# martinruenz/co-fusion

Measured on AMD Instinct MI355X. Metric: frames/sec at 640x480 (N active models) + ICP-reduce achieved HBM GB/s vs peak, higher is better.
Workload: dtype f32

## Files before the change

co_fusion_amd/csrc/cabi_model.hip:

```cpp
#include <math.h>
#include <string.h>

#include <string>
#include <vector>

#include "cf_host.h"

using namespace cf;

struct cf_model {
    cf_ctx* ctx = nullptr;
    uint32_t max_surfels = 0;
    uint32_t count_host = 0;
    bool count_pending = false;
    hipEvent_t count_event = nullptr;
    hipEvent_t count_wait = nullptr;
    bool ratio_valid = false;
    hipEvent_t ratio_event = nullptr;
    float* buf[2] = {nullptr, nullptr};
    int target = 0;
    float* staged = nullptr;
    unsigned* flags = nullptr;
    unsigned* block_sums = nullptr;
    unsigned* d_count = nullptr;
    unsigned* d_nfresh = nullptr;
    unsigned* d_tmp2 = nullptr;
    int ratio_blocks = 0;
    unsigned* h_counts = nullptr;
    float* records = nullptr;
    float* fresh = nullptr;
    unsigned* new_flags = nullptr;
    bool new_flags_clean = true;
    unsigned* owner = nullptr;
    float* fb_rec = nullptr;
    float* fb_raw = nullptr;
    float* fb_filt = nullptr;
    unsigned long long* keys = nullptr;
    unsigned* index = nullptr;
    float *vertConf = nullptr, *colorTime = nullptr, *normRad = nullptr;
    float* clean_rec = nullptr;
    uint8_t* splat_image = nullptr;
    float *splat_vertex = nullptr, *splat_normal = nullptr;
    uint16_t* splat_time = nullptr;
    float *fill_vertex = nullptr, *fill_normal = nullptr;
    uint8_t* fill_image = nullptr;
    float *tcx = nullptr, *tcy = nullptr;
    float* t_inv_dev = nullptr;
    const cf_odom* preindex_od = nullptr;
    int preindex_time = -1;
    float preindex_cutoff = 0.f; int preindex_delta = 0; uint32_t preindex_nb = 0;
    void drop_preindex() { preindex_od = nullptr; preindex_time = -1; }
    float* rays = nullptr;
    float inv_fx = 0, inv_fy = 0;
};

using cf::inv44f;

extern "C" {

int cf_bilateral(cf_ctx* ctx, const float* depth, int cols, int rows, float maxD, float* out)
{
    if (!ctx || !depth || !out) return CF_EINVAL;
    launch_bilateral(ctx->cur(), depth, cols, rows, maxD, out);
    LAUNCHCHK(ctx);
    return CF_OK;
}

int cf_model_create(cf_ctx* ctx, int max_surfels, cf_model** out)
{
    if (!ctx || !out || max_surfels <= 0) return CF_EINVAL;
    cf_model* m = new cf_model();
    m->ctx = ctx; m->max_surfels = (uint32_t)max_surfels;
    *out = m;
    const int W = ctx->cfg.width, H = ctx->cfg.height;
    const size_t N = (size_t)W * H, M = (size_t)max_surfels, Q = N / 4 + 64;
    if (int r = dmalloc(ctx, &m->buf[0], M * 12)) return r;
    if (int r = dmalloc(ctx, &m->buf[1], M * 12)) return r;
    if (int r = dmalloc(ctx, &m->staged, (M + Q) * 12)) return r;
    if (int r = dmalloc(ctx, &m->flags, M + Q)) return r;
    if (int r = dmalloc(ctx, &m->block_sums, (M + Q) / 2048 + N / 2048 + 16)) return r;
    if (int r = dmalloc(ctx, &m->d_count, 1)) return r;
    if (int r = dmalloc(ctx, &m->d_nfresh, 1)) return r;
    if (int r = dmalloc(ctx, &m->d_tmp2, 8)) return r;
    HIPCHK(ctx, hipMemsetAsync(m->d_tmp2, 0, 8 * sizeof(unsigned), ctx->cur()));
    m->ratio_blocks = fill_ratio_sample_blocks(W, H);
    if (int r = dmalloc(ctx, &m->records, N * 12)) return r;
    if (int r = dmalloc(ctx, &m->fresh, Q * 12)) return r;
    if (int r = dmalloc(ctx, &m->new_flags, N)) return r;
    if (int r = dmalloc(ctx, &m->owner, M)) return r;
    HIPCHK(ctx, hipMemsetAsync(m->owner, 0xFF, M * sizeof(unsigned), ctx->cur()));
    if (int r = dmalloc(ctx, &m->fb_rec, N * 12)) return r;
    if (int r = dmalloc(ctx, &m->fb_raw, N * 12)) return r;
    if (int r = dmalloc(ctx, &m->fb_filt, N * 12)) return r;
    if (int r = dmalloc(ctx, &m->keys, N)) return r;
    HIPCHK(ctx, hipMemsetAsync(m->keys, 0xFF, N * sizeof(unsigned long long), ctx->cur()));
    if (int r = dmalloc(ctx, &m->index, N)) return r;
    if (int r = dmalloc(ctx, &m->vertConf, N * 4)) return r;
    if (int r = dmalloc(ctx, &m->colorTime, N * 4)) return r;
    if (int r = dmalloc(ctx, &m->normRad, N * 4)) return r;
    if (int r = dmalloc(ctx, &m->clean_rec, N * 8)) return r;
    if (int r = dmalloc(ctx, &m->splat_image, N * 4)) return r;
    if (int r = dmalloc(ctx, &m->splat_vertex, N * 4)) return r;
    if (int r = dmalloc(ctx, &m->splat_normal, N * 4)) return r;
    if (int r = dmalloc(ctx, &m->splat_time, N)) return r;
    if (int r = dmalloc(ctx, &m->fill_vertex, N * 4)) return r;
    if (int r = dmalloc(ctx, &m->fill_normal, N * 4)) return r;
    if (int r = dmalloc(ctx, &m->fill_image, N * 4)) return r;
    if (int r = dmalloc(ctx, &m->tcx, (size_t)W)) return r;
    if (int r = dmalloc(ctx, &m->tcy, (size_t)H)) return r;
    if (int r = dmalloc(ctx, &m->rays, N * 4)) return r;
    if (int r = dmalloc(ctx, &m->t_inv_dev, 16)) return r;
    launch_splat_rays(ctx->cur(), ctx_cam(ctx), W, H, m->rays);
    HIPCHK(ctx, hipHostMalloc(reinterpret_cast<void**>(&m->h_counts), sizeof(unsigned) * 4, hipHostMallocCoherent));
    HIPCHK(ctx, hipEventCreateWithFlags(&m->count_event, hipEventDisableTiming));
    HIPCHK(ctx, hipEventCreateWithFlags(&m->ratio_event, hipEventDisableTiming));
    std::vector<float> tx(W), ty(H);
    for (int i = 0; i < W; i++) tx[i] = (float)((double)((float)i / (float)W) + 1.0 / (2.0 * (double)(float)W));
    for (int j = 0; j < H; j++) ty[j] = (float)((double)((float)j / (float)H) + 1.0 / (2.0 * (double)(float)H));
    HIPCHK(ctx, hipMemcpyAsync(m->tcx, tx.data(), sizeof(float) * W, hipMemcpyHostToDevice, ctx->cur()));
    HIPCHK(ctx, hipMemcpyAsync(m->tcy, ty.data(), sizeof(float) * H, hipMemcpyHostToDevice, ctx->cur()));
    m->inv_fx = (float)(1.0 / (double)ctx->cfg.fx); m->inv_fy = (float)(1.0 / (double)ctx->cfg.fy);
    HIPCHK(ctx, hipStreamSynchronize(ctx->cur()));
    return CF_OK;
}

void cf_model_destroy(cf_model* m)
{
    if (!m) return;
    (void)hipStreamSynchronize(m->ctx->cur());
    void* ptrs[] = {m->buf[0], m->buf[1], m->staged, m->flags, m->block_sums, m->d_count, m->d_nfresh, m->d_tmp2, m->records,
                    m->fresh, m->new_flags, m->owner, m->fb_rec, m->fb_raw, m->fb_filt, m->keys, m->index, m->vertConf,
                    m->colorTime, m->normRad, m->splat_image, m->splat_vertex, m->splat_normal, m->splat_time, m->fill_vertex,
                    m->fill_normal, m->fill_image, m->tcx, m->tcy, m->rays, m->t_inv_dev, m->clean_rec};
    for (void* p : ptrs) (void)hipFree(p);
    (void)hipHostFree(m->h_counts);
    if (m->count_event) (void)hipEventDestroy(m->count_event);
    if (m->ratio_event) (void)hipEventDestroy(m->ratio_event);
    delete m;
}

static int adopt_count(cf_model* m)
{
    m->count_host = m->h_counts[0];
    m->count_pending = false;
    if (m->count_host > m->max_surfels) { m->ctx->set_error("surfel buffer overflow"); return CF_ENOMEM; }
    return CF_OK;
}
static int sync_count(cf_model* m)
{
    cf_ctx* ctx = m->ctx;
    HIPCHK(ctx, hipMemcpyAsync(m->h_counts, m->d_count, sizeof(unsigned), hipMemcpyDeviceToHost, ctx->cur()));
    HIPCHK(ctx, hipStreamSynchronize(ctx->cur()));
    return adopt_count(m);
}
static int post_count(cf_model* m, uint32_t upper_bound)
{
    cf_ctx* ctx = m->ctx;
    HIPCHK(ctx, hipEventRecord(m->count_event, ctx->cur()));
    m->count_wait = m->count_event;
    m->count_host = upper_bound;
    m->count_pending = true;
    return CF_OK;
}
static int count_bound(cf_model* m, uint32_t* out)
{
    if (m->count_pending) {
        if (!m->count_wait) { if (int r = sync_count(m)) return r; *out = m->count_host; return CF_OK; }
        if (hipEventQuery(m->count_wait) == hipSuccess) { if (int r = adopt_count(m)) return r; }
        else (void)hipGetLastError();
    }
    *out = m->count_host;
    return CF_OK;
}
static int exact_count(cf_model* m, uint32_t* out)
{
    if (m->count_pending) {
        if (!m->count_wait) { if (int r = sync_count(m)) return r; *out = m->count_host; return CF_OK; }
        HIPCHK(m->ctx, hipEventSynchronize(m->count_wait));
        if (int r = adopt_count(m)) return r;
    }
    *out = m->count_host;
    return CF_OK;
}

int cf_model_initialise(cf_model* m, const uint8_t* rgba, const float* depth_raw, const float* depth_filt, int time, float maxDepth)
{
    if (!m || !rgba || !depth_raw || !depth_filt) return CF_EINVAL;
    m->drop_preindex();
    cf_ctx* ctx = m->ctx; hipStream_t s = ctx->cur();
    const int W = ctx->cfg.width, H = ctx->cfg.height; const long long N = (long long)W * H;
    if ((uint32_t)N > m->max_surfels) return CF_ENOMEM;
    const cf_cam cam = ctx_cam(ctx);
    launch_feedback(s, rgba, depth_raw, W, H, cam, m->inv_fx, m->inv_fy, m->tcx, m->tcy, time, maxDepth, m->fb_rec, m->new_flags);
    HIPCHK(ctx, hipMemsetAsync(m->fb_raw, 0, sizeof(float) * 12 * N, s));
    launch_scan_scatter(s, m->fb_rec, m->new_flags, N, m->block_sums, m->d_count, 0, m->fb_raw);
    launch_feedback(s, rgba, depth_filt, W, H, cam, m->inv_fx, m->inv_fy, m->tcx, m->tcy, time, maxDepth, m->fb_rec, m->new_flags);
    HIPCHK(ctx, hipMemsetAsync(m->fb_filt, 0, sizeof(float) * 12 * N, s));
    launch_scan_scatter(s, m->fb_rec, m->new_flags, N, m->block_sums, m->d_tmp2, 0, m->fb_filt);
    m->new_flags_clean = false;
    launch_init(s, m->fb_raw, m->fb_filt, m->d_count, N, m->buf[m->target]);
    LAUNCHCHK(ctx);
    return sync_count(m);
}

int cf_model_count(cf_model* m, uint32_t* count) { if (!m || !count) return CF_EINVAL; return exact_count(m, count); }

int cf_model_predict_indices(cf_model* m, const float pose[16], int time, float maxDepth, int timeDelta)
{
    if (!m || !pose) return CF_EINVAL;
    m->drop_preindex();
    cf_ctx* ctx = m->ctx;
    float t_inv[16];
    inv44f(pose, t_inv);
    uint32_t nb = 0;
    if (int r = count_bound(m, &nb)) return r;
    launch_predict_indices(ctx->cur(), m->buf[m->target], m->d_count, nb, t_inv, ctx_cam(ctx), ctx->cfg.width, ctx->cfg.height,
                           maxDepth, time, timeDelta, m->keys, m->index, m->vertConf, m->colorTime, m->normRad);
    LAUNCHCHK(ctx);
    return CF_OK;
}

int cf_model_index_keys(cf_model* m, const float pose[16], int time, float maxDepth, int timeDelta, uint32_t surfel_begin, uint32_t surfel_end,
                        uint64_t* keys_dev)
{
    if (!m || !pose || !keys_dev || surfel_begin > surfel_end) return CF_EINVAL;
    m->drop_preindex();
    cf_ctx* ctx = m->ctx;
    const int W = ctx->cfg.width, H = ctx->cfg.height;
    float t_inv[16];
    inv44f(pose, t_inv);
    uint32_t nb = 0;
    if (int r = count_bound(m, &nb)) return r;
    HIPCHK(ctx, hipMemsetAsync(keys_dev, 0xFF, sizeof(uint64_t) * (size_t)W * H, ctx->cur()));
    launch_index_keys(ctx->cur(), m->buf[m->target], m->d_count, surfel_begin, surfel_end < nb ? surfel_end : nb, t_inv, ctx_cam(ctx), W, H, maxDepth,
                      time, timeDelta, reinterpret_cast<unsigned long long*>(keys_dev));
    LAUNCHCHK(ctx);
    return CF_OK;
}
int cf_model_index_resolve(cf_model* m, const float pose[16], uint64_t* keys_dev)
{
    if (!m || !pose || !keys_dev) return CF_EINVAL;
    m->drop_preindex();
    cf_ctx* ctx = m->ctx;
    float t_inv[16];
    inv44f(pose, t_inv);
    launch_index_resolve(ctx->cur(), m->buf[m->target], t_inv, ctx->cfg.width, ctx->cfg.height, reinterpret_cast<unsigned long long*>(keys_dev),
                         m->index, m->vertConf, m->colorTime, m->normRad);
    LAUNCHCHK(ctx);
    return CF_OK;
}

int cf_model_predict_indices_sharded(cf_model* m, const float pose[16], int time, float maxDepth, int timeDelta, int shard, int nshards)
{
    if (!m || !pose || nshards < 1 || shard < 0 || shard >= nshards) return CF_EINVAL;
    m->drop_preindex();
    cf_ctx* ctx = m->ctx;
    if (!ctx->collective) { ctx->set_error("cf_model_predict_indices_sharded: no collective registered (cf_set_collective)"); return CF_ESTATE; }
    uint32_t n = 0;
    if (int r = exact_count(m, &n)) return r;
    const uint32_t b = (uint32_t)(((uint64_t)n * (uint64_t)shard) / (uint64_t)nshards), e = (uint32_t)(((uint64_t)n * (uint64_t)(shard + 1)) / (uint64_t)nshards);
    if (int r = cf_model_index_keys(m, pose, time, maxDepth, timeDelta, b, e, reinterpret_cast<uint64_t*>(m->keys))) return r;
    if (ctx->collective(ctx->collective_user, 1, m->keys, (uint64_t)ctx->cfg.width * ctx->cfg.height, (void*)ctx->cur()) != 0) {
        ctx->set_error("cf_model_predict_indices_sharded: the collective failed");
        return CF_ESTATE;
    }
    return cf_model_index_resolve(m, pose, reinterpret_cast<uint64_t*>(m->keys));
}

int cf_model_combined_predict(cf_model* m, const float pose[16], float maxDepth, float confThreshold, int time, int maxTime, int timeDelta)
{
    if (!m || !pose) return CF_EINVAL;
    cf_ctx* ctx = m->ctx;
    float t_inv[16];
    inv44f(pose, t_inv);
    uint32_t nb = 0;
    if (int r = count_bound(m, &nb)) return r;
    launch_combined_predict(ctx->cur(), m->buf[m->target], m->d_count, nb, t_inv, ctx_cam(ctx), ctx->cfg.width, ctx->cfg.height,
                            maxDepth, confThreshold, time, maxTime, timeDelta, m->rays, m->keys, m->splat_image, m->splat_vertex, m->splat_normal,
                            m->splat_time);
    LAUNCHCHK(ctx);
    m->ratio_valid = false;
    return CF_OK;
}

int cf_model_prefetch_fill_ratio(cf_model* m)
{
    if (!m) return CF_EINVAL;
    cf_ctx* ctx = m->ctx;
    launch_fill_ratio(ctx->cur(), m->splat_image, ctx->cfg.width, ctx->cfg.height, m->d_tmp2 + 2, m->h_counts + 2);
    LAUNCHCHK(ctx);
    HIPCHK(ctx, hipEventRecord(m->ratio_event, ctx->cur()));
    m->ratio_valid = true;
    return CF_OK;
}

int cf_model_perform_fill_in(cf_model* m, const uint8_t* rgba, const float* depth_filt, int passthrough_geom, int passthrough_rgb)
{
    if (!m || !rgba || !depth_filt) return CF_EINVAL;
    cf_ctx* ctx = m->ctx;
    launch_fill_in(ctx->cur(), m->splat_vertex, m->splat_normal, m->splat_image, depth_filt, rgba, ctx->cfg.width, ctx->cfg.height, ctx_cam(ctx),
                   m->inv_fx, m->inv_fy, passthrough_geom, passthrough_rgb, m->fill_vertex, m->fill_normal, m->fill_image);
    LAUNCHCHK(ctx);
    return CF_OK;
}

int cf_model_requires_fill_in(cf_model* m, float ratio, int* out)
{
    if (!m || !out) return CF_EINVAL;
    cf_ctx* ctx = m->ctx;
    if (m->ratio_valid) {
        HIPCHK(ctx, hipEventSynchronize(m->ratio_event));
    } else {
        launch_fill_ratio(ctx->cur(), m->splat_image, ctx->cfg.width, ctx->cfg.height, m->d_tmp2 + 2, m->h_counts + 2);
        LAUNCHCHK(ctx);
        HIPCHK(ctx, hipStreamSynchronize(ctx->cur()));
    }
    *out = ((float)m->h_counts[2] / (float)m->h_counts[3] < ratio) ? 1 : 0;
    return CF_OK;
}

int cf_model_fill_ratio_device(cf_model* m, const uint32_t** counts_dev)
{
    if (!m || !counts_dev) return CF_EINVAL;
    *counts_dev = m->ratio_valid ? m->d_tmp2 + 2 : nullptr;
    return CF_OK;
}

int cf_model_fuse(cf_model* m, const float pose[16], int time, const uint8_t* rgba, const uint8_t* mask, const float* depth_raw,
                  const float* depth_filt, float maxDepth, float weighting, int maskID)
{
    if (!m || !pose || !rgba || !mask || !depth_raw || !depth_filt) return CF_EINVAL;
    m->drop_preindex();
    cf_ctx* ctx = m->ctx; hipStream_t s = ctx->cur();
    const int W = ctx->cfg.width, H = ctx->cfg.height; const long long N = (long long)W * H;
    SurfelFuseArgs a;
    a.index = m->index; a.vertConf = m->vertConf; a.normRad = m->normRad; a.rgba = rgba; a.depth_raw = depth_raw; a.depth_filt = depth_filt;
    a.mask = mask; a.tcx = m->tcx; a.tcy = m->tcy; memcpy(a.pose, pose, sizeof(a.pose)); a.cam = ctx_cam(ctx); a.inv_fx = m->inv_fx;
    a.inv_fy = m->inv_fy; a.cols = W; a.rows = H; a.time = time; a.weighting = weighting; a.maskID = maskID; a.maxDepth = maxDepth;
    a.records = m->records; a.new_flags = m->new_flags; a.owner = m->owner; a.flags_clean = m->new_flags_clean ? 1 : 0;
    launch_associate(s, a);
    {
        ScanPassArgs sp{m->records, m->new_flags, N, m->block_sums, m->d_nfresh, 0, m->fresh, nullptr};
        sp.zero_flags = 1;
        launch_scan_scatter_batch(s, &sp, 1);
        m->new_flags_clean = true;
    }
    uint32_t nb = 0;
    if (int r = count_bound(m, &nb)) return r;
    launch_update(s, m->buf[m->target], m->d_count, nb, m->owner, m->records, time, m->buf[1 - m->target]);
    m->target = 1 - m->target;
    LAUNCHCHK(ctx);
    return CF_OK;
}

int cf_model_clean(cf_model* m, const float pose[16], int time, float confThreshold, float outlierCoeff, int timeDelta, const float* depth_filt,
                   const uint8_t* mask, int maskID, uint32_t* count_out)
{
    if (!m || !pose || !depth_filt || !mask) return CF_EINVAL;
    m->drop_preindex();
    cf_ctx* ctx = m->ctx; hipStream_t s = ctx->cur();
    const int W = ctx->cfg.width, H = ctx->cfg.height;
    uint32_t nb = 0;
    if (int r = count_bound(m, &nb)) return r;
    const unsigned bound = nb + (unsigned)((W / 2) * (H / 2));
    if (bound > m->max_surfels + (unsigned)(W * H / 4 + 64)) return CF_ENOMEM;
    SurfelCleanArgs a;
    a.index = m->index; a.vertConf = m->vertConf; a.colorTime = m->colorTime; a.depth_filt = depth_filt; a.mask = mask; a.rec = nullptr;
    inv44f(pose, a.t_inv); a.cam = ctx_cam(ctx); a.cols = W; a.rows = H; a.time = time; a.confThreshold = confThreshold;
    a.outlierCoeff = outlierCoeff; a.timeDelta = timeDelta; a.maskID = maskID;
    launch_clean(s, m->buf[m->target], m->d_count, m->fresh, m->d_nfresh, bound, a, m->staged, m->flags);
    launch_scan_scatter(s, m->staged, m->flags, bound, m->block_sums, m->d_count, 0, m->buf[1 - m->target], m->h_counts);
    m->target = 1 - m->target;
    LAUNCHCHK(ctx);
    const uint32_t upper = bound < m->max_surfels ? bound : m->max_surfels;
    if (int r = post_count(m, upper)) return r;
    if (count_out) return exact_count(m, count_out);
    return CF_OK;
}

int cf_models_preindex(cf_ctx* ctx, const cf_model_preindex* items, int n, float depth_cutoff, int time_delta)
{
    if (!ctx || !items || n <= 0) return CF_EINVAL;
    hipStream_t s = ctx->cur();
    const int W = ctx->cfg.width, H = ctx->cfg.height;
    std::vector<IndexPassArgs> a((size_t)n);
    for (int k = 0; k < n; k++) {
        cf_model* m = items[k].model; const cf_odom* od = items[k].odom;
        if (!m || !od || m->ctx != ctx || od->ctx != ctx) return CF_EINVAL;
        uint32_t nb = 0;
        if (int r = count_bound(m, &nb)) return r;
        const float* pinv = reinterpret_cast<const float*>(reinterpret_cast<const char*>(od->d_state) + offsetof(cf::OdomDev, pose_inv));
        IndexPassArgs& p = a[k];
        p.surfels = m->buf[m->target]; p.count = m->d_count; p.id_begin = 0; p.id_end = nb; p.maxDepth = depth_cutoff; p.time = items[k].time;
        p.timeDelta = time_delta; p.keys = m->keys; p.index = m->index; p.vertConf = m->vertConf; p.colorTime = m->colorTime; p.normRad = m->normRad;
        p.t_inv_dev = pinv;
    }
    launch_index_keys_batch(s, a.data(), n, ctx_cam(ctx), W, H);
    launch_index_resolve_batch(s, a.data(), n, ctx_cam(ctx), W, H);
    LAUNCHCHK(ctx);
    for (int k = 0; k < n; k++) {
        cf_model* m = items[k].model;
        m->preindex_od = items[k].odom; m->preindex_time = items[k].time; m->preindex_cutoff = depth_cutoff; m->preindex_delta = time_delta; m->preindex_nb = a[k].id_end;
    }
    return CF_OK;
}
static bool preindexed_with(const cf_model* m, const float pose[16], int time, float depth_cutoff, int time_delta, uint32_t nb)
{
    if (!m->preindex_od || m->preindex_time != time) return false;
    if (m->preindex_cutoff != depth_cutoff || m->preindex_delta != time_delta || m->preindex_nb != nb) return false;
    const cf::OdomDev* h = m->preindex_od->h_state;
    for (int r = 0; r < 3; r++) {
        if (memcmp(&pose[r * 4], &h->Rcurr[r * 3], 12) != 0 || memcmp(&pose[r * 4 + 3], &h->tcurr[r], 4) != 0) return false;
    }
    return pose[12] == 0 && pose[13] == 0 && pose[14] == 0 && pose[15] == 1;
}

int cf_models_frame_passes(cf_ctx* ctx, const cf_model_pass* items, int n, float depth_cutoff, float outlier_coeff, int time_delta)
{
    if (!ctx || !items || n <= 0) return CF_EINVAL;
    hipStream_t s = ctx->cur();
    const int W = ctx->cfg.width, H = ctx->cfg.height; const long long N = (long long)W * H;
    const cf_cam cam = ctx_cam(ctx);
    std::vector<int> fusing;
    for (int k = 0; k < n; k++) {
        const cf_model_pass& it = items[k];
        if (!it.model || it.model->ctx != ctx || !it.pose || !it.rgba || !it.depth_filtered) return CF_EINVAL;
        if (it.do_fuse) { if (!it.mask || !it.depth_raw) return CF_EINVAL; fusing.push_back(k); }
    }
    for (int k : fusing) {
        cf_model* m = items[k].model;
        uint32_t nb = 0;
        if (int r = count_bound(m, &nb)) return r;
        if (nb + (unsigned)((W / 2) * (H / 2)) > m->max_surfels + (unsigned)(W * H / 4 + 64)) {
            ctx->set_error("cf_models_frame_passes: a model's surfel buffer cannot hold the clean stage's staging area (max_surfels too small)");
            return CF_ENOMEM;
        }
    }
    for (int k = 0; k < n; k++) { uint32_t nb = 0; if (int r = count_bound(items[k].model, &nb)) return r; }
    int surf_ev = -1;
    if (ctx->prof.enabled > 0 && (ctx->surf_calls_seen++ % (unsigned)ctx->prof.enabled) == 0 && ctx->surf_used + 2 <= cf_ctx::kSurfEvents) {
        for (int e = ctx->surf_used; e < ctx->surf_used + 2; e++)
            if (!ctx->surf_events[e]) HIPCHK(ctx, hipEventCreate(&ctx->surf_events[e]));
        surf_ev = ctx->surf_used; ctx->surf_used += 2;
        HIPCHK(ctx, hipEventRecord(ctx->surf_events[surf_ev], s));
        for (int k = 0; k < n; k++) ctx->surf_bytes += (uint64_t)items[k].model->count_host * 48u * (items[k].do_fuse ? 8u : 2u);
        ctx->surf_calls++;
    }
    static const bool clean_rec_on = getenv("CF_NO_CLEAN_REC") == nullptr;
    auto index_args_of = [&](const std::vector<int>& which, bool feeds_clean, std::vector<IndexPassArgs>& a) -> int {
        a.assign(which.size(), IndexPassArgs{});
        for (size_t q = 0; q < which.size(); q++) {
            const cf_model_pass& it = items[which[q]]; cf_model* m = it.model;
            uint32_t nb = 0;
            if (int r = count_bound(m, &nb)) return r;
            IndexPassArgs& p = a[q];
            p.surfels = m->buf[m->target]; p.count = m->d_count; p.id_begin = 0; p.id_end = nb; inv44f(it.pose, p.t_inv); p.maxDepth = depth_cutoff;
            p.time = it.time; p.timeDelta = time_delta; p.keys = m->keys; p.index = m->index; p.vertConf = m->vertConf; p.colorTime = m->colorTime;
            p.normRad = m->normRad;
            if (feeds_clean && clean_rec_on) { p.clean_rec = m->clean_rec; p.clean_depth = it.depth_filtered; }
        }
        return CF_OK;
    };
    auto index_pass = [&](const std::vector<int>& which) -> int {
        std::vector<IndexPassArgs> a;
        if (int r = index_args_of(which, false, a)) return r;
        launch_index_keys_batch(s, a.data(), (int)a.size(), cam, W, H);
        launch_index_resolve_batch(s, a.data(), (int)a.size(), cam, W, H);
        return CF_OK;
    };
    if (!fusing.empty()) {
        const int nf = (int)fusing.size();
        {
            std::vector<int> todo;
            for (int k : fusing) {
                uint32_t nb = 0;
                if (int r = count_bound(items[k].model, &nb)) return r;
                if (!preindexed_with(items[k].model, items[k].pose, items[k].time, depth_cutoff, time_delta, nb)) todo.push_back(k);
            }
            if (!todo.empty()) { if (int r = index_pass(todo)) return r; }
        }
        std::vector<SurfelFuseArgs> fa(nf);
        std::vector<ScanPassArgs> sa(nf);
        std::vector<UpdatePassArgs> ua(nf);
        for (int q = 0; q < nf; q++) {
            const cf_model_pass& it = items[fusing[q]]; cf_model* m = it.model;
            SurfelFuseArgs& a = fa[q];
            a.index = m->index; a.vertConf = m->vertConf; a.normRad = m->normRad; a.rgba = it.rgba; a.depth_raw = it.depth_raw; a.depth_filt = it.depth_filtered;
            a.mask = it.mask; a.tcx = m->tcx; a.tcy = m->tcy; memcpy(a.pose, it.pose, sizeof(a.pose)); a.cam = cam; a.inv_fx = m->inv_fx;
            a.inv_fy = m->inv_fy; a.cols = W; a.rows = H; a.time = it.time; a.weighting = it.weighting; a.maskID = it.mask_id; a.maxDepth = it.fuse_max_depth;
            a.records = m->records; a.new_flags = m->new_flags; a.owner = m->owner; a.flags_clean = m->new_flags_clean ? 1 : 0;
            sa[q] = ScanPassArgs{m->records, m->new_flags, N, m->block_sums, m->d_nfresh, 0, m->fresh, nullptr};
            sa[q].zero_flags = 1;
            m->new_flags_clean = true;
            uint32_t nb = 0;
            if (int r = count_bound(m, &nb)) return r;
            ua[q] = UpdatePassArgs{m->buf[m->target], m->d_count, nb, m->owner, m->records, it.time, m->buf[1 - m->target]};
        }
        launch_associate_batch(s, fa.data(), nf);
        for (int q = 0; q < nf; q++) items[fusing[q]].model->target = 1 - items[fusing[q]].model->target;
        {
            std::vector<IndexPassArgs> ia;
            if (int r = index_args_of(fusing, true, ia)) return r;
            static const bool side_by_side = getenv("CF_NO_SIDE_BY_SIDE") == nullptr;
            if (!(side_by_side && launch_update_compaction_index_keys(s, ua.data(), sa.data(), ia.data(), nf, cam, W, H))) {
                launch_scan_scatter_batch(s, sa.data(), nf);
                launch_update_batch(s, ua.data(), nf);
                launch_index_keys_batch(s, ia.data(), nf, cam, W, H);
            }
            launch_index_resolve_batch(s, ia.data(), nf, cam, W, H);
        }
        std::vector<CleanPassArgs> ca(nf);
        std::vector<uint32_t> upper(nf);
        for (int q = 0; q < nf; q++) {
            const cf_model_pass& it = items[fusing[q]]; cf_model* m = it.model;
            uint32_t nb = 0;
            if (int r = count_bound(m, &nb)) return r;
            const unsigned bound = nb + (unsigned)((W / 2) * (H / 2));
            if (bound > m->max_surfels + (unsigned)(W * H / 4 + 64)) return CF_ENOMEM;
            CleanPassArgs& c = ca[q];
            c.h.index = m->index; c.h.vertConf = m->vertConf; c.h.colorTime = m->colorTime; c.h.depth_filt = it.depth_filtered; c.h.mask = it.mask;
            c.h.rec = clean_rec_on ? m->clean_rec : nullptr;
            inv44f(it.pose, c.h.t_inv); c.h.cam = cam; c.h.cols = W; c.h.rows = H; c.h.time = it.time; c.h.confThreshold = it.conf_threshold;
            c.h.outlierCoeff = outlier_coeff; c.h.timeDelta = time_delta; c.h.maskID = it.mask_id;
            c.surfels = m->buf[m->target]; c.count = m->d_count; c.fresh = m->fresh; c.n_fresh = m->d_nfresh; c.total_bound = bound; c.staged = m->staged;
            c.flags = m->flags;
            sa[q] = ScanPassArgs{m->staged, m->flags, (long long)bound, m->block_sums, m->d_count, 0, m->buf[1 - m->target], m->h_counts};
            upper[q] = bound < m->max_surfels ? bound : m->max_surfels;
        }
        launch_clean_batch(s, ca.data(), nf);
        launch_scan_scatter_batch(s, sa.data(), nf);
        if (!ctx->batch_event) HIPCHK(ctx, hipEventCreateWithFlags(&ctx->batch_event, hipEventDisableTiming));
        for (int q = 0; q < nf; q++) {
            cf_model* m = items[fusing[q]].model;
            m->target = 1 - m->target;
            m->count_host = upper[q]; m->count_pending = true; m->count_wait = nullptr;
        }
    }
    std::vector<SplatPassArgs> pa(n);
    for (int k = 0; k < n; k++) {
        const cf_model_pass& it = items[k]; cf_model* m = it.model;
        uint32_t nb = m->count_host;
        if (!(m->count_pending && !m->count_wait)) { if (int r = count_bound(m, &nb)) return r; }
        SplatPassArgs& p = pa[k];
        p.surfels = m->buf[m->target]; p.count = m->d_count; p.count_bound = nb; inv44f(it.pose, p.t_inv); p.maxDepth = depth_cutoff;
        p.confThreshold = it.conf_threshold; p.time = it.time; p.maxTime = it.time; p.timeDelta = time_delta; p.rays = m->rays; p.keys = m->keys;
        p.image = m->splat_image; p.vertexConf = m->splat_vertex; p.normalRad = m->splat_normal; p.time16 = m->splat_time;
        m->ratio_valid = false;
        if (it.fill_in)
            p.fill = SplatFillArgs{it.depth_filtered, it.rgba, m->inv_fx, m->inv_fy, it.passthrough_geom ? 1 : 0, it.passthrough_rgb ? 1 : 0,
                                   m->fill_vertex, m->fill_normal, m->fill_image, reinterpret_cast<unsigned long long*>(m->d_tmp2 + 4),
                                   m->d_tmp2 + 2, m->h_counts + 2, m->ratio_blocks};
    }
    launch_combined_predict_batch(s, pa.data(), n, cam, W, H);
    LAUNCHCHK(ctx);
    for (int k = 0; k < n; k++)
        if (items[k].fill_in) {
            HIPCHK(ctx, hipEventRecord(items[k].model->ratio_event, s));
            items[k].model->ratio_valid = true;
        }
    if (surf_ev >= 0) HIPCHK(ctx, hipEventRecord(ctx->surf_events[surf_ev + 1], s));
    if (!fusing.empty()) {
        HIPCHK(ctx, hipEventRecord(ctx->batch_event, s));
        for (int k : fusing) items[k].model->count_wait = ctx->batch_event;
    }
    for (int k = 0; k < n; k++) items[k].model->drop_preindex();
    return CF_OK;
}

int cf_model_download_map(cf_model* m, float* host_surfels, uint32_t capacity, uint32_t* count)
{
    if (!m || !count) return CF_EINVAL;
    cf_ctx* ctx = m->ctx;
    if (int r = exact_count(m, count)) return r;
    if (host_surfels) {
        const uint32_t n = m->count_host < capacity ? m->count_host : capacity;
        HIPCHK(ctx, hipMemcpyAsync(host_surfels, m->buf[m->target], (size_t)n * 48, hipMemcpyDeviceToHost, ctx->cur()));
        HIPCHK(ctx, hipStreamSynchronize(ctx->cur()));
    }
    return CF_OK;
}

int cf_model_upload_map(cf_model* m, const float* host_surfels, uint32_t count)
{
    if (!m || (!host_surfels && count) || count > m->max_surfels) return CF_EINVAL;
    m->drop_preindex();
    cf_ctx* ctx = m->ctx;
    if (count) HIPCHK(ctx, hipMemcpyAsync(m->buf[m->target], host_surfels, (size_t)count * 48, hipMemcpyHostToDevice, ctx->cur()));
    launch_set_count(ctx->cur(), m->d_count, count);
    HIPCHK(ctx, hipStreamSynchronize(ctx->cur()));
    m->count_host = count; m->count_pending = false;
    return CF_OK;
}

int cf_model_buffer(cf_model* m, int which, void** dptr, uint64_t* bytes)
{
    if (!m || !dptr) return CF_EINVAL;
    const size_t N = (size_t)m->ctx->cfg.width * m->ctx->cfg.height;
    void* p = nullptr; size_t b = 0;
    switch (which) {
        case 0: p = m->index; b = N * 4; break;
        case 1: p = m->vertConf; b = N * 16; break;
        case 2: p = m->colorTime; b = N * 16; break;
        case 3: p = m->normRad; b = N * 16; break;
        case 4: p = m->splat_image; b = N * 4; break;
        case 5: p = m->splat_vertex; b = N * 16; break;
        case 6: p = m->splat_normal; b = N * 16; break;
        case 7: p = m->splat_time; b = N * 2; break;
        case 8: p = m->fill_vertex; b = N * 16; break;
        case 9: p = m->fill_normal; b = N * 16; break;
        case 10: p = m->fill_image; b = N * 4; break;
        case 11: { uint32_t c = 0; if (int r = exact_count(m, &c)) return r; p = m->buf[m->target]; b = (size_t)c * 48; break; }
        case 12: {
            unsigned nf = 0;
            HIPCHK(m->ctx, hipMemcpyAsync(&nf, m->d_nfresh, sizeof(unsigned), hipMemcpyDeviceToHost, m->ctx->cur()));
            HIPCHK(m->ctx, hipStreamSynchronize(m->ctx->cur()));
            if (nf > N / 4 + 64) { m->ctx->set_error("cf_model_buffer: the new-surfel count exceeds its buffer"); return CF_ESTATE; }
            p = m->fresh; b = (size_t)nf * 48; break;
        }
        case 13: p = m->clean_rec; b = N * 32; break;
        default: return CF_EINVAL;
    }
    *dptr = p; if (bytes) *bytes = b;
    return CF_OK;
}

int cf_redetect_score(cf_ctx* ctx, const cf_redetect_candidate* cands, int n, const cf_redetect_frame* f, cf_redetect_counts* counts, uint32_t* label_pixels)
{
    if (!ctx || !cands || !f || !counts || n <= 0 || n > kRedetectBatch) return CF_EINVAL;
    if (!f->depth || !f->label || f->cols <= 0 || f->rows <= 0 || (long long)f->cols * f->rows > 0x7fffffffLL) return CF_EINVAL;
    hipStream_t s = ctx->cur();
    const unsigned words = (unsigned)(((long long)f->cols * f->rows + 31) / 32);
    const size_t n_counts = (size_t)kRedetectBatch * kRedetectWords + 1;
    if (!ctx->d_redetect_counts) {
        if (int r = dmalloc(ctx, &ctx->d_redetect_counts, n_counts)) return r;
        HIPCHK(ctx, hipHostMalloc(reinterpret_cast<void**>(&ctx->h_redetect_counts), n_counts * sizeof(unsigned)));
    }
    if (words > ctx->redetect_words) {
        HIPCHK(ctx, hipStreamSynchronize(s));
        if (ctx->d_redetect_bits) (void)hipFree(ctx->d_redetect_bits);
        ctx->d_redetect_bits = nullptr; ctx->redetect_words = 0;
        if (int r = dmalloc(ctx, &ctx->d_redetect_bits, (size_t)kRedetectBatch * words)) return r;
        ctx->redetect_words = words;
    }
    RedetectCand rc[kRedetectBatch];
    for (int k = 0; k < n; k++) {
        cf_model* m = cands[k].model;
        if (!m || m->ctx != ctx) return CF_EINVAL;
        uint32_t nb = 0;
        if (int r = count_bound(m, &nb)) return r;
        rc[k].surfels = m->buf[m->target]; rc[k].count = m->d_count; rc[k].count_bound = nb; rc[k].theta = cands[k].conf_threshold;
        inv44f(cands[k].pose, rc[k].t_inv);
    }
    RedetectFrame rf{f->depth, f->label, f->cols, f->rows, f->cam, f->new_label, f->depth_cutoff, f->depth_tol};
    if (ctx->redetect_timing) HIPCHK(ctx, hipEventRecord(ctx->redetect_ev[0], s));
    HIPCHK(ctx, hipMemsetAsync(ctx->d_redetect_counts, 0, n_counts * sizeof(unsigned), s));
    launch_redetect_score(s, rc, n, rf, ctx->d_redetect_bits, words, ctx->d_redetect_counts);
    LAUNCHCHK(ctx);
    if (ctx->redetect_timing) HIPCHK(ctx, hipEventRecord(ctx->redetect_ev[1], s));
    HIPCHK(ctx, hipMemcpyAsync(ctx->h_redetect_counts, ctx->d_redetect_counts, n_counts * sizeof(unsigned), hipMemcpyDeviceToHost, s));
    HIPCHK(ctx, hipStreamSynchronize(s));
    if (ctx->redetect_timing) HIPCHK(ctx, hipEventElapsedTime(&ctx->redetect_last_ms, ctx->redetect_ev[0], ctx->redetect_ev[1]));
    for (int k = 0; k < n; k++) {
        const unsigned* w = ctx->h_redetect_counts + (size_t)k * kRedetectWords;
        counts[k] = cf_redetect_counts{w[0], w[1], w[2], w[3], w[4], w[5]};
    }
    if (label_pixels) *label_pixels = ctx->h_redetect_counts[(size_t)kRedetectBatch * kRedetectWords];
    return CF_OK;
}

int cf_redetect_timing(cf_ctx* ctx, int on, float* last_ms)
{
    if (!ctx) return CF_EINVAL;
    if (on) for (hipEvent_t& e : ctx->redetect_ev) if (!e) HIPCHK(ctx, hipEventCreate(&e));
    ctx->redetect_timing = on != 0;
    if (last_ms) *last_ms = ctx->redetect_last_ms;
    return CF_OK;
}

int cf_relabel(cf_ctx* ctx, uint8_t* label_dev, uint64_t n, int from, int to)
{
    if (!ctx || !label_dev || from < 0 || from > 255 || to < 0 || to > 255 || (reinterpret_cast<uintptr_t>(label_dev) & 15u)) return CF_EINVAL;
    if (from == to || n == 0) return CF_OK;
    launch_relabel(ctx->cur(), label_dev, n, (unsigned)from, (unsigned)to);
    LAUNCHCHK(ctx);
    return CF_OK;
}

float cf_fusion_weight(const float pose[16], const float lastPose[16], float weightMultiplier)
{
    float pinv[16], diff[16];
    inv44f(pose, pinv);
    for (int i = 0; i < 4; i++)
        for (int j = 0; j < 4; j++) {
            float s = 0;
            for (int k = 0; k < 4; k++) s += pinv[i * 4 + k] * lastPose[k * 4 + j];
            diff[i * 4 + j] = s;
        }
    const float tn = sqrtf(diff[3] * diff[3] + diff[7] * diff[7] + diff[11] * diff[11]);
    const float* R = diff;
    double rx = R[2 * 4 + 1] - R[1 * 4 + 2], ry = R[0 * 4 + 2] - R[2 * 4 + 0], rz = R[1 * 4 + 0] - R[0 * 4 + 1];
    const double s = sqrt((rx * rx + ry * ry + rz * rz) * 0.25);
    double c = (double)((R[0] + R[5] + R[10]) - 1.0f) * 0.5;
    c = c > 1. ? 1. : c < -1. ? -1. : c;
    double theta = acos(c);
    if (s < 1e-5) {
        double t;
        if (c > 0) rx = ry = rz = 0;
        else {
            t = (R[0] + 1) * 0.5; rx = sqrt(t > 0.0 ? t : 0.0);
            t = (R[5] + 1) * 0.5; ry = sqrt(t > 0.0 ? t : 0.0) * (R[0 * 4 + 1] < 0 ? -1.0 : 1.0);
            t = (R[10] + 1) * 0.5; rz = sqrt(t > 0.0 ? t : 0.0) * (R[0 * 4 + 2] < 0 ? -1.0 : 1.0);
            if (fabs(rx) < fabs(ry) && fabs(rx) < fabs(rz) && (R[1 * 4 + 2] > 0) != (ry * rz > 0)) rz = -rz;
            theta /= sqrt(rx * rx + ry * ry + rz * rz);
            rx *= theta; ry *= theta; rz *= theta;
        }
    } else {
        double vth = 1 / (2 * s);
        vth *= theta;
        rx *= vth; ry *= vth; rz *= vth;
    }
    const float rv[3] = {(float)rx, (float)ry, (float)rz};
    const float rn = sqrtf(rv[0] * rv[0] + rv[1] * rv[1] + rv[2] * rv[2]);
    float weighting = tn > rn ? tn : rn;
    const float largest = 0.01f, minWeight = 0.5f;
    if (weighting > largest) weighting = largest;
    const float w = 1.0f - (weighting / largest);
    weighting = (w > minWeight ? w : minWeight) * weightMultiplier;
    return weighting;
}

}
```

co_fusion_amd/csrc/cf_host.h:

```cpp
#pragma once

#include <string.h>

#include <mutex>
#include <string>

#include "cf_kernels.h"

struct cf_ctx;
struct cf_thread_binding { const cf_ctx* ctx = nullptr; hipStream_t stream = nullptr; };
extern thread_local cf_thread_binding cf_tls_binding;

struct cf_ctx {
    cf_config cfg{};
    hipStream_t stream = nullptr;
    hipStream_t cur() const { return cf_tls_binding.ctx == this ? cf_tls_binding.stream : stream; }
    hipStream_t own_stream = nullptr;
    std::string last_error;
    std::mutex error_mutex;
    cf::IcpLaunch icp_launch{256, 0};
    int icp_arith = 0;
    float* d_ref = nullptr;
    float* h_ref = nullptr;
    unsigned long long* d_acc_a = nullptr;
    unsigned long long* d_acc_b = nullptr;
    unsigned long long* d_out = nullptr;
    unsigned long long* h_out = nullptr;
    cf::OdomDev* d_scratch_state = nullptr;
    cf::OdomDev* h_scratch_state = nullptr;
    uint8_t* d_cand_scratch = nullptr;
    cf::So3Sync* d_so3_sync = nullptr;
    unsigned gn_mode_epoch = 0;
    int xcd_round_robin = -1;
    int gn_mode = 1;
    static constexpr int kStateSlots = 256;
    cf::OdomDev* d_state_pool = nullptr;
    cf::OdomDev* h_state_pool = nullptr;
    bool slot_used[kStateSlots]{};
    hipEvent_t batch_event = nullptr;
    static constexpr int kLanes = 8;
    hipStream_t lanes[kLanes]{};
    hipEvent_t lane_done[kLanes]{};
    hipEvent_t fork_point = nullptr;
    static constexpr int kMarks = 64;
    hipEvent_t marks[kMarks]{};
    bool mark_set[kMarks]{};
    hipStream_t forked_from = nullptr;
    bool forked = false;
    unsigned lanes_used = 0;
    int (*collective)(void* user, int op, void* dev_buf, uint64_t words, void* stream) = nullptr;
    void* collective_user = nullptr;
    void* rccl = nullptr;
    unsigned prof_calls = 0;
    cf::ProfSink prof{};
    double prof_ms_accum = 0;
    static constexpr int kSurfEvents = 64;
    hipEvent_t surf_events[kSurfEvents]{};
    int surf_used = 0; unsigned surf_calls_seen = 0;
    double surf_ms_accum = 0; uint64_t surf_calls = 0, surf_bytes = 0;
    unsigned* d_redetect_bits = nullptr; unsigned redetect_words = 0;
    unsigned* d_redetect_counts = nullptr; unsigned* h_redetect_counts = nullptr;
    bool redetect_timing = false; hipEvent_t redetect_ev[2]{}; float redetect_last_ms = 0.f;
    void set_error(const std::string& m);
};
inline cf_cam ctx_cam(const cf_ctx* ctx) { return cf_cam{ctx->cfg.fx, ctx->cfg.fy, ctx->cfg.cx, ctx->cfg.cy}; }
extern "C" int cf_wait_stream(cf_ctx* ctx);
#define HIPCHK(ctx, call)                                                                      \
    do {                                                                                       \
        hipError_t e_ = (call);                                                                \
        if (e_ != hipSuccess) {                                                                \
            (ctx)->set_error(std::string(#call) + ": " + hipGetErrorString(e_));               \
            return CF_EHIP;                                                                    \
        }                                                                                      \
    } while (0)
#define LAUNCHCHK(ctx) HIPCHK(ctx, hipGetLastError())
template <typename T>
inline int dmalloc(cf_ctx* ctx, T** p, size_t count)
{
    HIPCHK(ctx, hipMalloc(reinterpret_cast<void**>(p), count * sizeof(T)));
    HIPCHK(ctx, hipMemsetAsync(*p, 0, count * sizeof(T), ctx->cur()));
    return CF_OK;
}
inline int clear_acc(cf_ctx* ctx, unsigned long long* acc)
{
    HIPCHK(ctx, hipMemsetAsync(acc, 0, sizeof(unsigned long long) * cf::kGroups * 32, ctx->stream));
    return CF_OK;
}
struct cf_odom;
namespace cf {
int ref_track(cf_ctx* ctx, cf_odom* od, const float pose[16], const cf_track_opts* opts, float* err_surface);
int ref_icp_step(cf_ctx* ctx, const float Rcurr[9], const float tcurr[3], const float* vc, const float* nc, const float Rprev_inv[9], const float tprev[3],
                 cf_cam intr, const float* vp, const float* np, float dist_thres, float angle_thres, int cols, int rows, float* err, float out29[29]);
int ref_rgb_step(cf_ctx* ctx, const cf_dataterm* corres, float sigma, const float* cloud3, float fx, float fy, const int16_t* dIdx, const int16_t* dIdy,
                 float sobel_scale, int cols, int rows, float out29[29]);
int ref_so3_step(cf_ctx* ctx, const uint8_t* last_image, const uint8_t* next_image, const float basis[9], const float kinv[9], const float krlr[9],
                 int cols, int rows, float out11[11]);
inline void pose_split(const float pose[16], float R[9], float t[3])
{
    for (int i = 0; i < 3; i++) { R[3 * i] = pose[4 * i]; R[3 * i + 1] = pose[4 * i + 1]; R[3 * i + 2] = pose[4 * i + 2]; t[i] = pose[4 * i + 3]; }
}
struct TrackTerms { bool icp, rgb; };
inline TrackTerms track_terms(const cf_track_opts* o) { return TrackTerms{!o->rgb_only && o->icp_weight > 0, o->rgb_only || o->icp_weight < 100}; }
}

struct cf_odom {
    cf_ctx* ctx = nullptr;
    float* vmaps_tmp = nullptr;
    float* nmaps_tmp = nullptr;
    float* vmap_g_prev[3]{};
    float* nmap_g_prev[3]{};
    float* vmap_curr[3]{};
    float* nmap_curr[3]{};
    const float* ext_vmap_curr[3]{};
    const float* ext_nmap_curr[3]{};
    float2* zrange[3]{};
    bool zrange_valid = false;
    const float2* ext_zrange[3]{};
    const float* cur_vmap(int l) const { return ext_vmap_curr[l] ? ext_vmap_curr[l] : vmap_curr[l]; }
    const float* cur_nmap(int l) const { return ext_nmap_curr[l] ? ext_nmap_curr[l] : nmap_curr[l]; }
    const float2* cur_zrange(int l) const { return ext_vmap_curr[l] ? ext_zrange[l] : (zrange_valid ? zrange[l] : nullptr); }
    float* lastDepth[3]{};
    float* nextDepth[3]{};
    bool next_depth_is_last = false;
    float* next_depth(int i) const { return next_depth_is_last ? lastDepth[i] : nextDepth[i]; }
    uint8_t* lastImage[3]{};
    uint8_t* nextImage[3]{};
    uint8_t* lastNextImage[3]{};
    int16_t* dIdx[3]{};
    int16_t* dIdy[3]{};
    float* cloud[3]{};
    cf_dataterm* corres[3]{};
    uint8_t* cand[3]{};
    unsigned char* occ = nullptr;
    bool occ_valid = false;
    bool use_occ = false;
    unsigned* aabb = nullptr;
    float map_pose[12]{};
    int box_hint[4] = {0x7fffffff, 0, 0, 0};
    unsigned* res_range = nullptr;
    int res_hint[3] = {-1, -1, -1};
    bool box_valid = false;
    int band_begin = 0, band_end = 0;
    bool band_counts = true;
    unsigned long long* icp_acc = nullptr;
    unsigned long long* rgb_acc = nullptr;
    cf::OdomDev* d_state = nullptr;
    cf::OdomDev* h_state = nullptr;
    int slot = -1;
    float distThres = 0, angleThres = 0, sobelScale = 0, maxDepthDeltaRGB = 0, maxDepthRGB = 0;
    float angleSqLt = 0, distSqLe = 0;
    float minGrad[3]{};
    bool pending_so3_swap = false;
    size_t rgb_acc_words = 0;
    unsigned gn_epoch_seen = 0;
    bool result_pending = false;
    int expected_solves = -1;
    cf::LaunchShape launch_shape{};
};
```

co_fusion_amd/csrc/cf_kernels.h:

```cpp
#pragma once

#include <hip/hip_runtime.h>
#include <hip/hip_ext.h>
#include <stdint.h>

#include "../../include/cofusion_hip.h"

namespace cf {

__host__ __device__ __forceinline__ cf_cam cam_level(cf_cam c, int level)
{
    const int div = 1 << level;
    return cf_cam{c.fx / div, c.fy / div, c.cx / div, c.cy / div};
}

constexpr int kGroups = 64;

struct alignas(64) GnHot {
    int icp, level_done; float cull_z[2];
    float Rcurr[9], tcurr[3];
    float Rprev_inv[9], tprev[3];
    int cull_box[4];
    int rgb, rgbOnly, level_done2, pad;
    float krkInv[9], kt[3];
// ... 109 lines not shown
void launch_frame_maps(hipStream_t s, FrameMapsArgs a, int W, int H);
void launch_rgbd_pyramids(hipStream_t s, const RgbdBatch& b, int n_chains, int W, int H, float cutoff);
void launch_model_maps_and_pyramids(hipStream_t s, const ModelMapsBatch& mb, int n, const RgbdBatch& rb, int n_chains, int W, int H, float cutoff);
void launch_rgb_prep(hipStream_t s, RgbPrepBatch b, int n, int W, int H);

struct IDiv { unsigned M, s; };
inline IDiv make_idiv(int d)
{
    if (d < 2) return IDiv{0x80000000u, 0u};
    unsigned l = 0;
    while ((1u << l) < (unsigned)d) l++;
    return IDiv{(unsigned)((((unsigned long long)1 << (31 + l)) + (unsigned)d - 1) / (unsigned)d), l - 1};
}
constexpr int kGramBits[8] = {20, 20, 20, 17, 17, 17, 22, 0};
struct LaunchShape { int icp[3]; int res[3]; int icp_err; };
struct IcpLaunch { int threads; int ppt; int gram;
                   LaunchShape* const* shape = nullptr; };

constexpr int kMaxBatch = 16;
struct IcpModelArgs {
    const float* vc; const float* nc;
    const float* vp; const float* np;
    const OdomDev* st;
    unsigned long long* acc;
    float* err;
    const unsigned char* occ;
    int row_begin, row_end;
    int cull;
    const float2* zr;
    int box_blocks;
};
constexpr int kNoBoxHint = 0x7fffffff;
struct CullRuns { int x0, y0, nrx, total; };
__host__ __device__ inline CullRuns cull_runs(const int box[4], int L, int cols, int rows)
{
    int bx0 = (box[0] >> L) - 1, by0 = (box[1] >> L) - 1, bx1 = (box[2] >> L) + 1, by1 = (box[3] >> L) + 1;
    bx0 = bx0 < 0 ? 0 : bx0; by0 = by0 < 0 ? 0 : by0; bx1 = bx1 > cols - 1 ? cols - 1 : bx1; by1 = by1 > rows - 1 ? rows - 1 : by1;
    if (bx0 > bx1 || by0 > by1) return CullRuns{0, 0, 0, 0};
    if ((cols & 63) == 0) { const int nrx = (bx1 >> 6) - (bx0 >> 6) + 1; return CullRuns{bx0 >> 6, by0, nrx, nrx * (by1 - by0 + 1)}; }
    const int q0 = (by0 * cols) >> 6, q1 = ((by1 + 1) * cols - 1) >> 6;
    return CullRuns{0, q0, 0, q1 - q0 + 1};
}
inline int box_blocks_for(const int box_hint[4], int L, int cols, int rows, int threads)
{
    if (box_hint[0] == kNoBoxHint) return 0;
    const CullRuns cr = cull_runs(box_hint, L, cols, rows);
    const int wpb = threads / 64;
    const int runs = cr.total + cr.total / 4 + 2 * (cr.nrx > 0 ? cr.nrx : (cols + 63) / 64);
    int want = (((runs + 2 * wpb - 1) / (2 * wpb) + 7) / 8) * 8;
    return want < 8 ? 8 : want;
}
inline int residual_blocks_for(int seen) { return seen < 0 ? 0 : seen + seen / 4 + 2; }
struct GnArgs {
    OdomDev* od[kMaxBatch];
    unsigned long long* icp_acc[kMaxBatch];
    unsigned long long* rgb_acc[kMaxBatch];
    OdomDev* od_host[kMaxBatch];
    int slot_px;
    int icp_gram;
};
struct RgbModelArgs {
    OdomDev* st;
    const uint8_t* cand; const float* nextDepth; const float* lastDepth;
    const uint8_t* lastImage; const uint8_t* nextImage;
    cf_dataterm* corres; const float* cloud; const int16_t* dIdx; const int16_t* dIdy;
    unsigned long long* icp_acc; unsigned long long* rgb_acc;
    int no_counts;
    uint2* recs;
    unsigned* slot_counts;
    const unsigned* res_range;
    int res_blocks;
};
struct RgbArgs {
    RgbModelArgs m[kMaxBatch];
    int cols, rows;
    cf_cam il;
    float sobelScale, maxDepthDelta;
    int compact;
    int slot_px;
    IDiv cdiv;
};
inline RgbModelArgs rgb_model_args(const OdomDev* h , OdomDev* d_state, int level)
{
    return RgbModelArgs{d_state, h->cand[level], h->nextDepth[level], h->lastDepth[level], h->lastImage[level], h->nextImage[level],
                        h->corres[level], h->cloud[level], h->dIdx[level], h->dIdy[level], h->icp_acc, h->rgb_acc, 0,
                        reinterpret_cast<uint2*>(h->corres[level]),
                        reinterpret_cast<unsigned*>(reinterpret_cast<uint2*>(h->corres[level]) + (size_t)(h->width >> level) * (h->height >> level)),
                        h->res_range ? h->res_range + 2 * level : nullptr, 0};
}
constexpr int kMaxSlots = 2 * kMaxBatch;
struct IcpArgs {
    IcpModelArgs m[kMaxBatch];
    int cols, rows;
    cf_cam intr;
    float distThres, angleThres;
    float angleSqLt, distSqLe;
    int occ_w, occ_shift;
    int flags;
    int row_begin, row_end;
    IDiv cdiv;
    int slot_end[kMaxSlots];
    unsigned char slot_desc[kMaxSlots];
    int slots_used;
};
constexpr unsigned char kResidualSlot = 0x80;
void launch_icp_level(hipStream_t s, IcpLaunch cfg, const IcpArgs& args, int n, int level, hipEvent_t ev0 = nullptr, hipEvent_t ev1 = nullptr);
void launch_rgb_residual(hipStream_t s, const RgbArgs& ra, int n);
void launch_rgb_step(hipStream_t s, const RgbArgs& ra, int n);
constexpr uint64_t kRgbResidualBytes = 27;
constexpr uint64_t kRgbResidualBytesCompact = 11;
void launch_acc_total(hipStream_t s, const unsigned long long* acc, unsigned long long* out);
void launch_rgb_cand(hipStream_t s, const int16_t* dIdx, const int16_t* dIdy, const float* next_depth,
                     const uint8_t* next_image, float min_scale, int cols, int rows, uint8_t* cand);
void launch_so3_step(hipStream_t s, const uint8_t* last_image, const uint8_t* next_image, const float basis[9],
                     const float kinv[9], const float krlr[9], int cols, int rows, unsigned long long* out16);
void launch_gn_solve(hipStream_t s, const GnArgs& gn, int n, int next_level, int last_of_level);

struct ProfSink {
    hipEvent_t* events; int capacity; int used; uint64_t bytes; uint64_t launches; int enabled;
};

constexpr int kSo3Blocks = 16;
constexpr int kStepSubs = 16;
struct So3Sync { unsigned long long acc[10][16]; unsigned arrive, depart;
                 unsigned step_top, pad;
                 unsigned step_sub[kStepSubs][32]; };
struct GnHook { int (*fn)(void* user, int op, void* dev_buf, uint64_t words, void* stream); void* user; int split[kMaxBatch]; };
struct TrackerStates { OdomDev* dev[kMaxBatch]; const OdomDev* host[kMaxBatch]; };
bool launch_gn_track(hipStream_t s, IcpLaunch cfg, const TrackerStates& states, So3Sync* so3_syncs ,
                     const GnHook* hook, const IcpArgs icp_args[3], const RgbArgs rgb_args[3], int n, int width, int height, bool so3,
                     bool pyramid, bool fast_odom, bool rgb, bool icp, int mode, ProfSink* prof,
                     OdomDev* const* h_states = nullptr ,
                     const RgbPrepBatch* prep = nullptr );
void rgb_prep_levels(RgbPrepBatch& b, int n, int W, int H);
float replay_icp_level0(hipStream_t s, IcpLaunch cfg, const IcpArgs& a0, const RgbArgs& r0, int n, int slots, int ablate, int reps, hipEvent_t e0, hipEvent_t e1);
#ifdef CF_ABLATE
void trace_so3_dump(hipStream_t s);
void trace_solve_begin();
void trace_solve_end(hipStream_t s, const char* path);
void trace_step_solve(hipStream_t s, IcpLaunch cfg, const IcpArgs& a0, const RgbArgs& r0, So3Sync* syncs, int n, const char* path);
void trace_icp_level0(hipStream_t s, IcpLaunch cfg, const IcpArgs& a0, const RgbArgs& r0, int n, int slots, const char* path);
#endif
bool probe_xcd_round_robin(hipStream_t s);
float sqrt_gate_lt(float T);
float sqrt_gate_le(float T);

constexpr int kSurfBatch = 16;
struct IndexPassArgs {
    const float* surfels; const unsigned* count; unsigned id_begin, id_end; float t_inv[16]; float maxDepth; int time, timeDelta;
    unsigned long long* keys; unsigned* index; float* vertConf; float* colorTime; float* normRad;
    const float* t_inv_dev;
    float* clean_rec;
    const float* clean_depth;
};
__host__ __device__ inline void inv44f(const float a[16], float o[16])
{
    const float c00 = a[5] * a[10] - a[6] * a[9];
    const float c01 = a[6] * a[8] - a[4] * a[10];
    const float c02 = a[4] * a[9] - a[5] * a[8];
    const float det = a[0] * c00 + a[1] * c01 + a[2] * c02;
    const float id = 1.0f / det;
    float Li[9];
    Li[0] = c00 * id; Li[1] = (a[2] * a[9] - a[1] * a[10]) * id; Li[2] = (a[1] * a[6] - a[2] * a[5]) * id;
    Li[3] = c01 * id; Li[4] = (a[0] * a[10] - a[2] * a[8]) * id; Li[5] = (a[2] * a[4] - a[0] * a[6]) * id;
    Li[6] = c02 * id; Li[7] = (a[1] * a[8] - a[0] * a[9]) * id; Li[8] = (a[0] * a[5] - a[1] * a[4]) * id;
    for (int i = 0; i < 3; i++) {
        o[i * 4 + 0] = Li[i * 3 + 0]; o[i * 4 + 1] = Li[i * 3 + 1]; o[i * 4 + 2] = Li[i * 3 + 2];
        o[i * 4 + 3] = -(Li[i * 3 + 0] * a[3] + Li[i * 3 + 1] * a[7] + Li[i * 3 + 2] * a[11]);
    }
    o[12] = 0; o[13] = 0; o[14] = 0; o[15] = 1;
}
struct SplatFillArgs {
    const float* depth_filt; const uint8_t* rgba;
    float inv_fx, inv_fy; int pass_geom, pass_rgb;
    float* fill_vertex; float* fill_normal; uint8_t* fill_image;
    unsigned long long* acc;
    unsigned* out2; unsigned* out2_host;
    int sample_blocks;
};
int fill_ratio_sample_blocks(int cols, int rows);
struct SplatPassArgs {
    const float* surfels; const unsigned* count; unsigned count_bound; float t_inv[16]; float maxDepth, confThreshold; int time, maxTime, timeDelta;
    const float* rays; unsigned long long* keys; uint8_t* image; float* vertexConf; float* normalRad; uint16_t* time16;
    SplatFillArgs fill;
};
struct UpdatePassArgs { const float* in; const unsigned* count; unsigned count_bound; unsigned* owner; const float* records; int time; float* out; };
struct SurfelFuseArgs {
    const unsigned* index; const float* vertConf; const float* normRad;
    const uint8_t* rgba; const float* depth_raw; const float* depth_filt; const uint8_t* mask;
    const float* tcx; const float* tcy;
    float pose[16]; cf_cam cam; float inv_fx, inv_fy;
    int cols, rows, time; float weighting; int maskID; float maxDepth;
    float* records; unsigned* new_flags; unsigned* owner;
    int flags_clean = 0;
};
struct SurfelCleanArgs {
    const unsigned* index; const float* vertConf; const float* colorTime;
    const float* depth_filt; const uint8_t* mask;
    const float* rec;
    float t_inv[16]; cf_cam cam; int cols, rows, time; float confThreshold, outlierCoeff; int timeDelta, maskID;
};
struct CleanPassArgs {
    SurfelCleanArgs h; const float* surfels; const unsigned* count; const float* fresh; const unsigned* n_fresh; unsigned total_bound;
    float* staged; unsigned* flags;
};
struct ScanPassArgs {
    const float* rec; const unsigned* flags; long long n; unsigned* block_sums; unsigned* total; unsigned add_to_total; float* out; unsigned* total_host;
    int zero_flags = 0;
};
void launch_index_keys_batch(hipStream_t s, const IndexPassArgs* items, int n, cf_cam cam, int cols, int rows);
bool launch_update_compaction_index_keys(hipStream_t s, const UpdatePassArgs* up, const ScanPassArgs* sc, const IndexPassArgs* ix, int n, cf_cam cam, int cols,
                                         int rows);
void launch_index_resolve_batch(hipStream_t s, const IndexPassArgs* items, int n, cf_cam cam, int cols, int rows);
void launch_combined_predict_batch(hipStream_t s, const SplatPassArgs* items, int n, cf_cam cam, int cols, int rows);
void launch_associate_batch(hipStream_t s, const SurfelFuseArgs* items, int n);
void launch_update_batch(hipStream_t s, const UpdatePassArgs* items, int n);
void launch_clean_batch(hipStream_t s, const CleanPassArgs* items, int n);
void launch_scan_scatter_batch(hipStream_t s, const ScanPassArgs* items, int n);
void launch_bilateral(hipStream_t s, const float* depth, int cols, int rows, float maxD, float* out);
void launch_scan_scatter(hipStream_t s, const float* rec, const unsigned* flags, long long n, unsigned* block_sums, unsigned* total,
                         unsigned add_to_total, float* out, unsigned* total_host = nullptr );
void launch_feedback(hipStream_t s, const uint8_t* rgba, const float* depth, int cols, int rows, cf_cam cam, float inv_fx, float inv_fy,
                     const float* tcx, const float* tcy, int time, float maxDepth, float* rec, unsigned* flags);
void launch_init(hipStream_t s, const float* raw, const float* filt, const unsigned* raw_count, long long max_n, float* out);
void launch_index_keys(hipStream_t s, const float* surfels, const unsigned* count, unsigned id_begin, unsigned id_end, const float t_inv[16],
                       cf_cam cam, int cols, int rows, float maxDepth, int time, int timeDelta, unsigned long long* keys);
void launch_index_resolve(hipStream_t s, const float* surfels, const float t_inv[16], int cols, int rows, unsigned long long* keys,
                          unsigned* index, float* vertConf, float* colorTime, float* normRad);
void launch_predict_indices(hipStream_t s, const float* surfels, const unsigned* count, unsigned count_bound, const float t_inv[16], cf_cam cam,
                            int cols, int rows, float maxDepth, int time, int timeDelta, unsigned long long* keys, unsigned* index,
                            float* vertConf, float* colorTime, float* normRad);
void launch_splat_rays(hipStream_t s, cf_cam cam, int cols, int rows, float* rays );
void launch_combined_predict(hipStream_t s, const float* surfels, const unsigned* count, unsigned count_bound, const float t_inv[16], cf_cam cam,
                             int cols, int rows, float maxDepth, float confThreshold, int time, int maxTime, int timeDelta,
                             const float* rays, unsigned long long* keys, uint8_t* image, float* vertexConf, float* normalRad, uint16_t* time16);
void launch_fill_in(hipStream_t s, const float* pv, const float* pn, const uint8_t* pimg, const float* depth, const uint8_t* rgba, int cols,
                    int rows, cf_cam cam, float inv_fx, float inv_fy, int pass_geom, int pass_rgb, float* ov, float* on, uint8_t* oi);
void launch_fill_ratio(hipStream_t s, const uint8_t* pimg, int cols, int rows, unsigned* out2, unsigned* out2_host = nullptr );
void launch_associate(hipStream_t s, const SurfelFuseArgs& h);
void launch_update(hipStream_t s, const float* in, const unsigned* count, unsigned count_bound, unsigned* owner, const float* records, int time,
                   float* out);
void launch_clean(hipStream_t s, const float* surfels, const unsigned* count, const float* fresh, const unsigned* n_fresh, unsigned total_bound,
                  const SurfelCleanArgs& h, float* staged, unsigned* flags);
void launch_set_count(hipStream_t s, unsigned* out, unsigned v);

constexpr int kRedetectBatch = 16;
constexpr int kRedetectWords = 8;
struct RedetectCand {
    const float* surfels; const unsigned* count; unsigned count_bound;
    float theta;
    float t_inv[16];
};
struct RedetectFrame {
    const float* depth; const uint8_t* label; int cols, rows; cf_cam cam; int new_label; float cutoff, tol;
};
void launch_redetect_score(hipStream_t s, const RedetectCand* cands, int n, const RedetectFrame& f, unsigned* bits, unsigned words, unsigned* counts);
void launch_relabel(hipStream_t s, uint8_t* label , unsigned long long n, unsigned from, unsigned to);

}
```

co_fusion_amd/csrc/surfel.hip:

```cpp
#include "cf_surfel_device.h"
#include "cf_kernels.h"

namespace cf {

static constexpr int kB = 256;
static inline int gridFor(long long n) { return (int)((n + kB - 1) / kB); }
static inline int gridXcd(long long n, int chunk = 1) { const int q = 8 * (chunk > 1 ? chunk : 1); return (gridFor(n) + q - 1) / q * q; }
#ifdef CF_ABLATE
static int xcd_env(const char* name, int dflt) { const char* e = getenv(name); return e ? atoi(e) : dflt; }
#else
static constexpr int xcd_env(const char*, int dflt) { return dflt; }
#endif
struct BatchHdr { int n; int blk_end[kSurfBatch]; };
template <class A> struct Batch { BatchHdr h; A m[kSurfBatch]; };
struct VBlock { int model, bid, nblk; };
__device__ __forceinline__ VBlock batch_decode_at(const BatchHdr& h, int b)
{
    int slot = 0;
#pragma unroll
    for (int k = 0; k < kSurfBatch - 1; k++) slot += (b >= h.blk_end[k]) ? 1 : 0;
    const int start = slot ? h.blk_end[slot - 1] : 0;
    return VBlock{slot, b - start, h.blk_end[slot] - start};
}
__device__ __forceinline__ VBlock batch_decode(const BatchHdr& h) { return batch_decode_at(h, (int)blockIdx.x); }
template <class A>
static int batch_layout(Batch<A>& B, const int* blocks, int n)
{
    int total = 0;
    B.h.n = n;
    for (int k = 0; k < kSurfBatch; k++) {
        if (k < n) total += (blocks[k] + 7) / 8 * 8;
        B.h.blk_end[k] = k < n ? total : 0x7fffffff;
    }
    return total;
}

__device__ __forceinline__ int xcd_block(int chunk, int b, int nblk)
{
    if (chunk == 0) return b;
    const int per = nblk >> 3, x = b & 7, r = b >> 3;
    if (chunk < 0) return x * per + r;
    const int lb = ((r / chunk) * 8 + x) * chunk + (r % chunk);
    return lb;
}

__device__ __forceinline__ unsigned sortable_bits(float z)
{
    const unsigned b = __float_as_uint(z);
    return (b & 0x80000000u) ? ~b : (b | 0x80000000u);
}
__device__ __forceinline__ unsigned long long zkey(float z, unsigned id) { return ((unsigned long long)sortable_bits(z) << 32) | id; }
constexpr unsigned long long kEmptyKey = ~0ull;

__global__ void __launch_bounds__(kB) bilateral_kernel(const float* __restrict__ depth, int cols, int rows, float maxD,
                                                       float* __restrict__ out)
{
    const int i = blockIdx.x * kB + threadIdx.x;
    if (i >= cols * rows) return;
    const int y = i / cols, x = i - y * cols;
    const float value = depth[i];
    if (value > maxD || value < 0.3f) { out[i] = 0; return; }
    float sum1 = 0, sum2 = 0;
#pragma unroll
    for (int dy = -6; dy <= 6; ++dy) {
        const int cy = y + dy;
        if (cy < 0 || cy >= rows) continue;
        const float* __restrict__ rowp = depth + cy * cols + x;
#pragma unroll
        for (int dx = -6; dx <= 6; ++dx) {
            const int cx = x + dx;
            if (cx < 0 || cx >= cols) continue;
            const float tmp = rowp[dx];
            const float space2 = (float)(dx * dx + dy * dy);
            const float color2 = (value - tmp) * (value - tmp);
            const float weight = det_expf(-(space2 * 0.024691358f + color2 * 555.556f));
            sum1 += tmp * weight;
            sum2 += weight;
        }
    }
    out[i] = sum1 / sum2;
}

static constexpr int kScanItems = 2048;
struct ScanArgs {
    const float4* rec; const unsigned* flags; long long n; unsigned* block_sums; unsigned* total; unsigned add_to_total; float4* out;
    unsigned* total_host; int zero_flags;
};
__device__ __forceinline__ void scan_load_flags(const unsigned* __restrict__ flags, long long i0, long long n, unsigned (&f)[8])
{
    if (i0 + 8 <= n) {
        const uint4 a = *reinterpret_cast<const uint4*>(flags + i0), c = *reinterpret_cast<const uint4*>(flags + i0 + 4);
        f[0] = a.x; f[1] = a.y; f[2] = a.z; f[3] = a.w; f[4] = c.x; f[5] = c.y; f[6] = c.z; f[7] = c.w;
    } else {
        unsigned t[8];
#pragma unroll
        for (int e = 0; e < 8; e++) t[e] = flags[i0 + e < n ? i0 + e : n - 1];
#pragma unroll
        for (int e = 0; e < 8; e++) f[e] = (i0 + e < n) ? t[e] : 0u;
    }
}
__device__ __forceinline__ void scan_block_sums_body(const Batch<ScanArgs>& B, int blk)
{
    const VBlock vb = batch_decode_at(B.h, blk);
    const ScanArgs& a = B.m[vb.model];
    const unsigned* __restrict__ flags = a.flags; const long long n = a.n; unsigned* __restrict__ block_sums = a.block_sums;
    if ((long long)vb.bid * kScanItems >= n) return;
    unsigned f[8];
    scan_load_flags(flags, (long long)vb.bid * kScanItems + (long long)threadIdx.x * 8, n, f);
    unsigned s = 0;
#pragma unroll
    for (int e = 0; e < 8; e++) s += f[e];
    for (int o = 32; o > 0; o >>= 1) s += __shfl_xor((int)s, o, 64);
    __shared__ unsigned w[4];
    if ((threadIdx.x & 63) == 0) w[threadIdx.x >> 6] = s;
    __syncthreads();
    if (threadIdx.x == 0) block_sums[vb.bid] = w[0] + w[1] + w[2] + w[3];
}
__global__ void __launch_bounds__(256) scan_block_sums_kernel(const Batch<ScanArgs> B) { scan_block_sums_body(B, (int)blockIdx.x); }
__global__ void set_count_kernel(unsigned* out, unsigned v);
__global__ void set_count2_kernel(unsigned* out, unsigned* out_host, unsigned v);
__device__ __forceinline__ void scan_scatter_body(const Batch<ScanArgs>& B, int blk)
{
    const VBlock vb = batch_decode_at(B.h, blk);
    const ScanArgs& a = B.m[vb.model];
    const float4* __restrict__ rec = a.rec; const unsigned* __restrict__ flags = a.flags; const long long n = a.n;
    const unsigned* __restrict__ block_sums = a.block_sums; unsigned* __restrict__ total = a.total; const unsigned add_to_total = a.add_to_total;
    float4* __restrict__ out = a.out; unsigned* __restrict__ total_host = a.total_host;
    const int nb = (int)((n + kScanItems - 1) / kScanItems);
    if (vb.bid >= nb) return;
    __shared__ unsigned wsum[4], s_base;
    __shared__ unsigned short s_src[kScanItems];
    const int tid = threadIdx.x, lane = tid & 63, wave = tid >> 6;
    const long long i0 = (long long)vb.bid * kScanItems + (long long)tid * 8;
    unsigned f[8];
    scan_load_flags(flags, i0, n, f);
    if (a.zero_flags) {
        unsigned* fz = const_cast<unsigned*>(flags);
        if (i0 + 8 <= n) { *reinterpret_cast<uint4*>(fz + i0) = make_uint4(0, 0, 0, 0); *reinterpret_cast<uint4*>(fz + i0 + 4) = make_uint4(0, 0, 0, 0); }
        else
            for (int e = 0; e < 8; e++) if (i0 + e < n) fz[i0 + e] = 0;
    }
    unsigned b = 0;
    for (int k = tid; k < vb.bid; k += 256) b += block_sums[k];
    for (int o = 32; o > 0; o >>= 1) b += __shfl_xor((int)b, o, 64);
    if (lane == 0) wsum[wave] = b;
    __syncthreads();
    if (tid == 0) s_base = wsum[0] + wsum[1] + wsum[2] + wsum[3];
    unsigned mine = 0;
#pragma unroll
    for (int e = 0; e < 8; e++) mine += f[e];
    unsigned incl = mine;
    for (int o = 1; o < 64; o <<= 1) { const unsigned t = __shfl_up((int)incl, o, 64); if (lane >= o) incl += t; }
    __syncthreads();
    if (lane == 63) wsum[wave] = incl;
    __syncthreads();
    unsigned rel = incl - mine;
    for (int w = 0; w < wave; w++) rel += wsum[w];
#pragma unroll
    for (int e = 0; e < 8; e++)
        if (f[e]) s_src[rel++] = (unsigned short)(tid * 8 + e);
    const unsigned count = wsum[0] + wsum[1] + wsum[2] + wsum[3];
    const unsigned base = s_base;
    __syncthreads();
    const float4* __restrict__ in0 = rec + (size_t)vb.bid * kScanItems * 3;
    float4* __restrict__ out0 = out + (size_t)base * 3;
    const unsigned words = count * 3;
#ifndef CF_SCAN_FLY
#define CF_SCAN_FLY 4
#endif
    constexpr int kFly = CF_SCAN_FLY;
    for (unsigned m0 = tid; m0 < words; m0 += kFly * 256) {
        float4 v[kFly];
#pragma unroll
        for (int u = 0; u < kFly; u++) {
            const unsigned m = m0 + u * 256;
            const unsigned mc = m < words ? m : words - 1;
            const unsigned j = mc / 3u;
            v[u] = in0[(size_t)s_src[j] * 3 + (mc - 3u * j)];
        }
#pragma unroll
        for (int u = 0; u < kFly; u++) { const unsigned m = m0 + u * 256; if (m < words) out0[m] = v[u]; }
    }
    if (vb.bid == nb - 1 && tid == 255) {
        *total = base + count + add_to_total;
        if (total_host) *total_host = base + count + add_to_total;
    }
}
__global__ void __launch_bounds__(256) scan_scatter_kernel(const Batch<ScanArgs> B) { scan_scatter_body(B, (int)blockIdx.x); }

void launch_scan_scatter_batch(hipStream_t s, const ScanPassArgs* items, int n_items)
{
    for (int base = 0; base < n_items; base += kSurfBatch) {
        const int nb = n_items - base < kSurfBatch ? n_items - base : kSurfBatch;
        Batch<ScanArgs> B;
        int blocks[kSurfBatch], any = 0;
        for (int k = 0; k < nb; k++) {
            const ScanPassArgs& h = items[base + k];
            B.m[k] = ScanArgs{reinterpret_cast<const float4*>(h.rec), h.flags, h.n, h.block_sums, h.total, h.add_to_total, reinterpret_cast<float4*>(h.out), h.total_host, h.zero_flags};
            blocks[k] = (int)((B.m[k].n + kScanItems - 1) / kScanItems);
            any += blocks[k];
            if (blocks[k] == 0) set_count2_kernel<<<1, 1, 0, s>>>(B.m[k].total, B.m[k].total_host, B.m[k].add_to_total);
        }
        if (!any) continue;
        const int grid = batch_layout(B, blocks, nb);
        scan_block_sums_kernel<<<grid, 256, 0, s>>>(B);
        scan_scatter_kernel<<<grid, 256, 0, s>>>(B);
    }
}
void launch_scan_scatter(hipStream_t s, const float* rec, const unsigned* flags, long long n, unsigned* block_sums, unsigned* total,
                         unsigned add_to_total, float* out, unsigned* total_host)
{
    const ScanPassArgs a{rec, flags, n, block_sums, total, add_to_total, out, total_host};
    launch_scan_scatter_batch(s, &a, 1);
}

__global__ void __launch_bounds__(kB) feedback_kernel(const uchar4* __restrict__ rgba, const float* __restrict__ depth, int cols, int rows,
                                                      float cx, float cy, float inv_fx, float inv_fy, const float* __restrict__ tcx,
                                                      const float* __restrict__ tcy, int time, float maxDepth,
                                                      float4* __restrict__ rec , unsigned* __restrict__ flags)
{
    const int q = blockIdx.x * kB + threadIdx.x;
    if (q >= cols * rows) return;
    const int j = q / cols, i = q - j * cols;
    const int rank = i * rows + j;
    const float x = tcx[i] * (float)cols, y = tcy[j] * (float)rows;
    const f3 p = get_vertex(depth, cols, rows, i, j, x, y, cx, cy, inv_fx, inv_fy);
    if (p.z <= 0 || p.z > maxDepth) { flags[rank] = 0; return; }
    const f3 n = get_normal_central(p, depth, cols, rows, i, j, x, y, cx, cy, inv_fx, inv_fy);
    const uchar4 c = rgba[q];
    flags[rank] = 1;
    rec[rank * 3 + 0] = make_float4(p.x, p.y, p.z, confidence(x, y, cx, cy, 1.0f));
    rec[rank * 3 + 1] = make_float4(encode_color((float)c.x / 255.0f, (float)c.y / 255.0f, (float)c.z / 255.0f), 0.f, (float)c.z / 255.0f, (float)time);
    rec[rank * 3 + 2] = make_float4(n.x, n.y, n.z, get_radius(p.z, n.z, inv_fx, inv_fy));
}


__global__ void __launch_bounds__(kB) init_kernel(const float4* __restrict__ raw, const float4* __restrict__ filt,
                                                  const unsigned* __restrict__ raw_count, float4* __restrict__ out)
{
    const unsigned k = blockIdx.x * kB + threadIdx.x;
    if (k >= *raw_count) return;
    const float4 c = raw[k * 3 + 1];
    out[k * 3] = raw[k * 3];
    out[k * 3 + 1] = make_float4(c.x, 0.f, 1.f, c.w);
    out[k * 3 + 2] = filt[k * 3 + 2];
}

__device__ __forceinline__ bool index_project(const float4 pc, const float4 ct, const Mat4& t_inv, cf_cam cam, int cols, int rows,
                                              float maxDepth, int time, int timeDelta, f3& ph, int& q)
{
    if ((float)time - ct.w > (float)timeDelta) return false;
    return surfel_project(pc, t_inv, cam, cols, rows, maxDepth, ph, q);
}

struct IndexArgs {
    const float4* surfels; const unsigned* count; Mat4 t_inv; float maxDepth; int time, timeDelta; unsigned id_begin, id_end;
    unsigned long long* keys; unsigned* index; float4* vertConf; float4* colorTime; float4* normRad;
    const float* t_inv_dev;
    float4* clean_rec; const float* clean_depth;
};
__device__ __forceinline__ Mat4 index_matrix(const IndexArgs& a)
{
    if (!a.t_inv_dev) return a.t_inv;
    Mat4 m;
#pragma unroll
    for (int k = 0; k < 16; k++) m.m[k] = a.t_inv_dev[k];
    return m;
}
struct FrameGeom { cf_cam cam; int cols, rows; };

__device__ __forceinline__ void index_splat_body(const Batch<IndexArgs>& B, const FrameGeom& g, int blk)
{
    const VBlock vb = batch_decode_at(B.h, blk);
    const IndexArgs& a = B.m[vb.model];
    const float4* __restrict__ surfels = a.surfels;
    const unsigned id = a.id_begin + vb.bid * kB + threadIdx.x;
    if (id >= *a.count || id >= a.id_end) return;
    f3 ph; int q;
    const Mat4 T = index_matrix(a);
    if (!index_project(surfels[id * 3], surfels[id * 3 + 1], T, g.cam, g.cols, g.rows, a.maxDepth, a.time, a.timeDelta, ph, q)) return;
    atomicMin(&a.keys[q], zkey(ph.z, id));
}
__global__ void __launch_bounds__(kB) index_splat_kernel(const Batch<IndexArgs> B, const FrameGeom g) { index_splat_body(B, g, (int)blockIdx.x); }

__global__ void __launch_bounds__(kB) index_resolve_kernel(const Batch<IndexArgs> B, const FrameGeom g)
{
    const VBlock vb = batch_decode(B.h);
    const IndexArgs& a = B.m[vb.model];
    const float4* __restrict__ surfels = a.surfels; unsigned long long* __restrict__ keys = a.keys; unsigned* __restrict__ index = a.index;
    float4* __restrict__ vertConf = a.vertConf; float4* __restrict__ colorTime = a.colorTime; float4* __restrict__ normRad = a.normRad;
    const int q = vb.bid * kB + threadIdx.x;
    if (q >= g.cols * g.rows) return;
    const unsigned long long k = keys[q];
    keys[q] = kEmptyKey;
    float4* __restrict__ const rec = a.clean_rec;
    const float dflt = rec ? a.clean_depth[q] : 0.f;
    if (k == kEmptyKey) {
        index[q] = 0;
        vertConf[q] = colorTime[q] = normRad[q] = make_float4(0, 0, 0, 0);
        if (rec) { rec[2 * q] = make_float4(0, 0, 0, 0); rec[2 * q + 1] = make_float4(0, 0, __uint_as_float(0u), dflt); }
        return;
    }
    const unsigned id = (unsigned)k;
    const float4 pc = surfels[id * 3], ct = surfels[id * 3 + 1], nr = surfels[id * 3 + 2];
    const Mat4 T = index_matrix(a);
    const f3 ph = xform_point(T, f3{pc.x, pc.y, pc.z});
    const f3 n = normalized(xform_dir(T, f3{nr.x, nr.y, nr.z}));
    index[q] = id;
    vertConf[q] = make_float4(ph.x, ph.y, ph.z, pc.w);
    colorTime[q] = ct;
    normRad[q] = make_float4(n.x, n.y, n.z, nr.w);
    if (rec) { rec[2 * q] = make_float4(ph.x, ph.y, ph.z, pc.w); rec[2 * q + 1] = make_float4(ct.z, ct.w, __uint_as_float(id), dflt); }
}

struct SplatSetup { f3 ph, n; float rad, pn; int x_lo, x_hi, y_lo, y_hi; };

__device__ __forceinline__ bool splat_setup(const float4 pc, const float4 ct, const float4 nr, const Mat4& t_inv, cf_cam cam, int cols,
                                            int rows, float maxDepth, float confThreshold, int time, int maxTime, int timeDelta,
                                            SplatSetup& s)
{
    s.ph = xform_point(t_inv, f3{pc.x, pc.y, pc.z});
    if (s.ph.z > maxDepth || s.ph.z < 0 || pc.w < confThreshold || (float)time - ct.w > (float)timeDelta || ct.w > (float)maxTime) return false;
    s.n = normalized(xform_dir(t_inv, f3{nr.x, nr.y, nr.z}));
    s.rad = nr.w;
    const f3 x1n = normalized(f3{s.n.y - s.n.z, -s.n.x, s.n.x});
    const f3 x1 = {x1n.x * s.rad * 1.41421356f, x1n.y * s.rad * 1.41421356f, x1n.z * s.rad * 1.41421356f};
    const f3 y1 = cross(s.n, x1);
    const f3 c[4] = {s.ph + x1, s.ph + y1, s.ph - y1, s.ph - x1};
    float px_[4], py_[4];
#pragma unroll
    for (int k = 0; k < 4; k++) { px_[k] = ((cam.fx * c[k].x) / c[k].z) + cam.cx; py_[k] = ((cam.fy * c[k].y) / c[k].z) + cam.cy; }
    const float xmin = fminf(px_[0], fminf(px_[1], fminf(px_[2], px_[3]))), xmax = fmaxf(px_[0], fmaxf(px_[1], fmaxf(px_[2], px_[3])));
    const float ymin = fminf(py_[0], fminf(py_[1], fminf(py_[2], py_[3]))), ymax = fmaxf(py_[0], fmaxf(py_[1], fmaxf(py_[2], py_[3])));
    const float size = fmaxf(0.0f, fmaxf(fabsf(xmax - xmin), fabsf(ymax - ymin)));
    if (!(size > 0.0f) || !(size <= 4096.0f)) return false;
    const float u = ((cam.fx * s.ph.x) / s.ph.z) + cam.cx, v = ((cam.fy * s.ph.y) / s.ph.z) + cam.cy;
    if (!(u >= 0.0f && v >= 0.0f && u <= (float)cols && v <= (float)rows)) return false;
    const float half = size * 0.5f;
    s.x_lo = max((int)ceilf(u - half - 0.5f), 0); s.x_hi = min((int)ceilf(u + half - 0.5f) - 1, cols - 1);
    s.y_lo = max((int)ceilf(v - half - 0.5f), 0); s.y_hi = min((int)ceilf(v + half - 0.5f) - 1, rows - 1);
    s.pn = dot(s.ph, s.n);
    return true;
}

__device__ __forceinline__ bool splat_fragment(const SplatSetup& s, const float4* __restrict__ rays, int cols, int px, int py, float maxDepth,
                                               float& z)
{
    const float4 lr = rays[py * cols + px];
    const f3 l = {lr.x, lr.y, lr.z};
    const float k = s.pn / dot(l, s.n);
    const f3 cp = {k * l.x, k * l.y, k * l.z};
    const f3 diff = cp - s.ph;
    if (!(dot(diff, diff) <= s.rad * s.rad)) return false;
    if (!(cp.z < maxDepth)) return false;
    z = cp.z;
    return true;
}

__global__ void __launch_bounds__(kB) splat_rays_kernel(cf_cam cam, int cols, int rows, float4* __restrict__ rays)
{
    const int q = blockIdx.x * kB + threadIdx.x;
    if (q >= cols * rows) return;
    const int py = q / cols, px = q - py * cols;
    const float fx_ = (float)px + 0.5f, fy_ = (float)py + 0.5f;
    const f3 l = normalized(f3{(fx_ - cam.cx) / cam.fx, (fy_ - cam.cy) / cam.fy, 1.0f});
    rays[q] = make_float4(l.x, l.y, l.z, 0.f);
}

struct SplatArgs {
    const float4* surfels; const unsigned* count; Mat4 t_inv; float maxDepth, confThreshold; int time, maxTime, timeDelta;
    const float4* rays; unsigned long long* keys; uchar4* image; float4* vertexConf; float4* normalRad; unsigned short* time16;
    SplatFillArgs fill;
};

__global__ void __launch_bounds__(kB) splat_raster_kernel(const Batch<SplatArgs> B, const FrameGeom g)
{
    const VBlock vb = batch_decode(B.h);
    const SplatArgs& a = B.m[vb.model];
    const float4* __restrict__ surfels = a.surfels; const float4* __restrict__ rays = a.rays; unsigned long long* __restrict__ keys = a.keys;
    const int cols = g.cols, rows = g.rows;
    const unsigned gt = vb.bid * kB + threadIdx.x;
    const unsigned id = gt >> 2;
    const int sub = (int)(gt & 3u);
    if (id >= *a.count) return;
    SplatSetup s;
    if (!splat_setup(surfels[id * 3], surfels[id * 3 + 1], surfels[id * 3 + 2], a.t_inv, g.cam, cols, rows, a.maxDepth, a.confThreshold, a.time,
                     a.maxTime, a.timeDelta, s))
        return;
    const int w = s.x_hi - s.x_lo + 1, h = s.y_hi - s.y_lo + 1;
    if (w <= 0 || h <= 0) return;
    int fx = sub, fy = 0;
    while (fx >= w) { fx -= w; fy++; }
    while (fy < h) {
        const int px = s.x_lo + fx, py = s.y_lo + fy;
        float z;
        if (splat_fragment(s, rays, cols, px, py, a.maxDepth, z)) {
            atomicMin(&keys[py * cols + px], zkey(z, id));
        }
        fx += 4;
        while (fx >= w) { fx -= w; fy++; }
    }
}

__device__ __forceinline__ void fill_in_px(float4 v, float4 n, uchar4 e, const float* __restrict__ depth, const uchar4* __restrict__ rgba, int cols,
                                           int rows, int x, int y, int q, float cx, float cy, float inv_fx, float inv_fy, int pass_geom, int pass_rgb,
                                           float4* __restrict__ ov, float4* __restrict__ on, uchar4* __restrict__ oi)
{
    const float z = depth[q];
    const f3 p = {((float)x - cx) * z * inv_fx, ((float)y - cy) * z * inv_fy, z};
    ov[q] = (v.z == 0 || pass_geom) ? make_float4(p.x, p.y, p.z, 1.f) : v;
    if (n.z == 0 || pass_geom) {
        const float zx = depth[y * cols + min(x + 1, cols - 1)], zy = depth[min(y + 1, rows - 1) * cols + x];
        const f3 vx = {((float)(x + 1) - cx) * zx * inv_fx, ((float)y - cy) * zx * inv_fy, zx};
        const f3 vy = {((float)x - cx) * zy * inv_fx, ((float)(y + 1) - cy) * zy * inv_fy, zy};
        const f3 nn = normalized(cross(vx - p, vy - p));
        on[q] = make_float4(nn.x, nn.y, nn.z, 1.f);
    } else
        on[q] = n;
    oi[q] = (((int)e.x + (int)e.y + (int)e.z) == 0 || pass_rgb) ? rgba[q] : e;
}
__global__ void __launch_bounds__(kB) fill_in_kernel(const float4* __restrict__ pv, const float4* __restrict__ pn, const uchar4* __restrict__ pimg,
                                                     const float* __restrict__ depth, const uchar4* __restrict__ rgba, int cols, int rows,
                                                     float cx, float cy, float inv_fx, float inv_fy, int pass_geom, int pass_rgb,
                                                     float4* __restrict__ ov, float4* __restrict__ on, uchar4* __restrict__ oi)
{
    const int q = blockIdx.x * kB + threadIdx.x;
    if (q >= cols * rows) return;
    const int y = q / cols, x = q - y * cols;
    fill_in_px(pv[q], pn[q], pimg[q], depth, rgba, cols, rows, x, y, q, cx, cy, inv_fx, inv_fy, pass_geom, pass_rgb, ov, on, oi);
}
__device__ __forceinline__ bool fill_ratio_sample(int p, int dn, int size)
{
    const int i0 = p * dn / size;
    bool hit = false;
    for (int i = max(i0 - 1, 0); i <= min(i0 + 1, dn - 1); i++) hit = hit || nearest_texel(((float)i + 0.5f) / (float)dn, size) == p;
    return hit;
}

int fill_ratio_sample_blocks(int cols, int rows)
{
    const int dw = cols / 20, dh = rows / 20;
    int blocks = 0, last = -1;
    for (int j = 0; j < dh; j++)
        for (int i = 0; i < dw; i++) {
// ... 325 lines not shown
    f3 localPos{0, 0, 0}, localNorm{0, 0, 0};
    float x = 0, y = 0, x_n = 0, y_n = 0;
    const float stepX = 1.0f / (float)cols, stepY = 1.0f / (float)rows;
    const float indexXStep = stepX * 0.5f / scale, indexYStep = stepY * 0.5f / scale;
    const float windowMultiplier = 2;
    bool window = false;
    if (exists) {
        const float4* src = (k < n_old) ? surfels + (size_t)k * 3 : fresh + (size_t)(k - n_old) * 3;
        pc = src[0]; ct = src[1]; nr = src[2];
        localPos = xform_point(a.t_inv, f3{pc.x, pc.y, pc.z});
        x = ((a.cam.fx * localPos.x) / localPos.z) + a.cam.cx; y = ((a.cam.fy * localPos.y) / localPos.z) + a.cam.cy;
        localNorm = normalized(xform_dir(a.t_inv, f3{nr.x, nr.y, nr.z}));
        x_n = x / (float)cols; y_n = y / (float)rows;
        window = (float)a.time - ct.w < (float)a.timeDelta && localPos.z > 0 && x > 0 && y > 0 && x < (float)cols && y < (float)rows;
    }
    const float iBeg = x_n - (scale * indexXStep * windowMultiplier), jBeg = y_n - (scale * indexYStep * windowMultiplier);
    const int X0 = (int)floorf(iBeg * (float)cols - 0.5f), Y0 = (int)floorf(jBeg * (float)rows - 0.5f);
#ifdef CF_ABLATE
    const int abl = a.abl;
#else
    constexpr int abl = 0;
#endif
    if (window && rec && !(abl & 1)) {
        const int half = sub & 1;
#pragma unroll
        for (int q = 0; q < 8; q++) {
            const int row = q >> 1, tex = (sub >> 1) + 2 * (q & 1), t = row * 4 + tex;
            const int g = iclamp(Y0 + row, 0, rows - 1) * cols + iclamp(X0 + tex, 0, cols - 1);
            const float4 v = rec[2 * g + half];
            float* const o = P + half * 64 + t;
            o[0] = v.x; o[16] = v.y; o[32] = v.z; o[48] = v.w;
        }
    } else
    if (window && !(abl & 1)) {
#pragma unroll
        for (int c = 0; c < 4; c++) {
            const int t = sub * 4 + c;
            const int g = iclamp(Y0 + sub, 0, rows - 1) * cols + iclamp(X0 + c, 0, cols - 1);
            const float4 vcf = a.vertConf[g];
            const float4 ctm = a.colorTime[g];
            const unsigned idx = a.index[g];
            P[0 * 16 + t] = vcf.x; P[1 * 16 + t] = vcf.y; P[2 * 16 + t] = vcf.z; P[3 * 16 + t] = vcf.w;
            P[4 * 16 + t] = ctm.z; P[5 * 16 + t] = ctm.w;
            P[6 * 16 + t] = __uint_as_float(idx);
        }
    }
    __syncthreads();
    if (!exists) return;
    int test = 1;
    int cnt = 0, zCount = 0, violationCount = 0;
    float avgViolation = 0;
    if (window && !(abl & 2)) {
        float i = iBeg;
        for (int s4 = 0; s4 < sub; s4++) i += indexXStep;
        for (; i < x_n + (scale * indexXStep * windowMultiplier); i += indexXStep, i += indexXStep, i += indexXStep, i += indexXStep) {
            for (float j = jBeg; j < y_n + (scale * indexYStep * windowMultiplier); j += indexYStep) {
                const int nlx = (int)floorf(i * (float)cols) - X0, nly = (int)floorf(j * (float)rows) - Y0;
                const unsigned current = ((unsigned)nlx < 4u && (unsigned)nly < 4u)
                                             ? __float_as_uint(P[6 * 16 + nly * 4 + nlx])
                                             : a.index[nearest_texel(j, rows) * cols + nearest_texel(i, cols)];
                if (current > 0U) {
                    float4 vertConf, colorTime;
                    const float fu = i * (float)cols - 0.5f, fv = j * (float)rows - 0.5f;
                    const float x0f = floorf(fu), y0f = floorf(fv);
                    const int lx = (int)x0f - X0, ly = (int)y0f - Y0;
                    if ((unsigned)lx < 3u && (unsigned)ly < 3u) {
                        const float wx = fu - x0f, wy = fv - y0f;
                        const float* q = P + (ly * 4 + lx);
                        vertConf.x = bilerp(q[0 * 16], q[0 * 16 + 1], q[0 * 16 + 4], q[0 * 16 + 5], wx, wy);
                        vertConf.y = bilerp(q[1 * 16], q[1 * 16 + 1], q[1 * 16 + 4], q[1 * 16 + 5], wx, wy);
                        vertConf.z = bilerp(q[2 * 16], q[2 * 16 + 1], q[2 * 16 + 4], q[2 * 16 + 5], wx, wy);
                        vertConf.w = bilerp(q[3 * 16], q[3 * 16 + 1], q[3 * 16 + 4], q[3 * 16 + 5], wx, wy);
                        colorTime.z = bilerp(q[4 * 16], q[4 * 16 + 1], q[4 * 16 + 4], q[4 * 16 + 5], wx, wy);
                        colorTime.w = bilerp(q[5 * 16], q[5 * 16 + 1], q[5 * 16 + 4], q[5 * 16 + 5], wx, wy);
                    } else {
                        vertConf = tex4_linear(a.vertConf, cols, rows, i, j);
                        colorTime = tex4_linear(a.colorTime, cols, rows, i, j);
                    }
                    const float dx = vertConf.x - localPos.x, dy = vertConf.y - localPos.y;
                    if (colorTime.z < ct.z && vertConf.w > a.confThreshold && vertConf.z > localPos.z && vertConf.z - localPos.z < 0.01f &&
                        sqrtf(dx * dx + dy * dy) < nr.w * 1.4f)
                        cnt++;
                    if (colorTime.w == (float)a.time && vertConf.w > a.confThreshold && vertConf.z > localPos.z &&
                        vertConf.z - localPos.z > 0.01f && fabsf(localNorm.z) > 0.85f)
                        zCount++;
                }
            }
        }
    }
    if (window && !(abl & 4)) {
        for (float i = x_n - stepX; i <= x_n + stepX; i += stepX)
            for (float j = y_n - stepY; j <= y_n + stepY; j += stepY) {
                const int tx = nearest_texel(i, cols), ty = nearest_texel(j, rows);
                const int lx = tx - X0, ly = ty - Y0;
                const float dv = (rec && (unsigned)lx < 4u && (unsigned)ly < 4u) ? P[7 * 16 + ly * 4 + lx] : a.depth_filt[ty * cols + tx];
                const float d = dv - localPos.z;
                if (d > 0.03f) { violationCount++; avgViolation += d; }
            }
    }
    cnt += __shfl_xor(cnt, 1, 4); cnt += __shfl_xor(cnt, 2, 4);
    zCount += __shfl_xor(zCount, 1, 4); zCount += __shfl_xor(zCount, 2, 4);
    if (sub != 0) return;
    if (cnt > 8 || zCount > 4) test = 0;
    if (ct.w == -2) ct.w = (float)a.time;
    if ((ct.w == -1 || (((float)a.time - ct.w) > 20 && pc.w < a.confThreshold))) test = 0;
    if (ct.w > 0 && (float)a.time - ct.w > (float)a.timeDelta) test = 1;
    if (violationCount > 0) {
        avgViolation /= (float)violationCount;
        pc.w *= 1.0f / (1 + a.outlierCoeff * avgViolation);
        const int mx = nearest_texel(x_n, cols), my = nearest_texel(y_n, rows);
        const int maskValue = a.mask[my * cols + mx];
        const float wDepth = a.depth_filt[my * cols + mx];
        if (maskValue != a.maskID && (wDepth > localPos.z - 0.05f && wDepth < localPos.z + 0.05f))
            pc.w *= (0.5f + 0.5f * (1 - a.outlierCoeff / 10.0f));
    }
    flags[k] = (unsigned)test;
    staged[(size_t)k * 3] = pc; staged[(size_t)k * 3 + 1] = ct; staged[(size_t)k * 3 + 2] = nr;
}

struct FillArgs { uint4* p; long long n16; };
__global__ void __launch_bounds__(kB) fill_zero_kernel(const Batch<FillArgs> B)
{
    const VBlock vb = batch_decode(B.h);
    const FillArgs& a = B.m[vb.model];
    const long long i = (long long)vb.bid * kB + threadIdx.x;
    if (i < a.n16) a.p[i] = make_uint4(0, 0, 0, 0);
}
__global__ void set_count_kernel(unsigned* out, unsigned v) { *out = v; }
__global__ void set_count2_kernel(unsigned* out, unsigned* out_host, unsigned v) { *out = v; if (out_host) *out_host = v; }

void launch_bilateral(hipStream_t s, const float* depth, int cols, int rows, float maxD, float* out)
{
    bilateral_kernel<<<gridFor((long long)cols * rows), kB, 0, s>>>(depth, cols, rows, maxD, out);
}

static Mat4 mat4_from(const float m[16]) { Mat4 r; for (int i = 0; i < 16; i++) r.m[i] = m[i]; return r; }

void launch_feedback(hipStream_t s, const uint8_t* rgba, const float* depth, int cols, int rows, cf_cam cam, float inv_fx, float inv_fy,
                     const float* tcx, const float* tcy, int time, float maxDepth, float* rec, unsigned* flags)
{
    feedback_kernel<<<gridFor((long long)cols * rows), kB, 0, s>>>(reinterpret_cast<const uchar4*>(rgba), depth, cols, rows, cam.cx, cam.cy, inv_fx,
                                                                   inv_fy, tcx, tcy, time, maxDepth, reinterpret_cast<float4*>(rec), flags);
}
void launch_init(hipStream_t s, const float* raw, const float* filt, const unsigned* raw_count, long long max_n, float* out)
{
    init_kernel<<<gridFor(max_n), kB, 0, s>>>(reinterpret_cast<const float4*>(raw), reinterpret_cast<const float4*>(filt), raw_count,
                                              reinterpret_cast<float4*>(out));
}
static_assert(sizeof(Batch<FuseArgs>) + 16 <= 4096 && sizeof(Batch<CleanArgs>) + 16 <= 4096 && sizeof(Batch<IndexArgs>) + sizeof(FrameGeom) <= 4096 &&
              sizeof(Batch<SplatArgs>) + sizeof(FrameGeom) <= 4096 && sizeof(Batch<ScanArgs>) <= 4096, "lower kSurfBatch");
static IndexArgs index_args(const IndexPassArgs& h)
{
    return IndexArgs{reinterpret_cast<const float4*>(h.surfels), h.count, mat4_from(h.t_inv), h.maxDepth, h.time, h.timeDelta, h.id_begin, h.id_end,
                     h.keys, h.index, reinterpret_cast<float4*>(h.vertConf), reinterpret_cast<float4*>(h.colorTime), reinterpret_cast<float4*>(h.normRad),
                     h.t_inv_dev, reinterpret_cast<float4*>(h.clean_rec), h.clean_depth};
}
void launch_index_keys_batch(hipStream_t s, const IndexPassArgs* items, int n_items, cf_cam cam, int cols, int rows)
{
    const FrameGeom g{cam, cols, rows};
    for (int base = 0; base < n_items; base += kSurfBatch) {
        const int nb = n_items - base < kSurfBatch ? n_items - base : kSurfBatch;
        Batch<IndexArgs> B;
        int blocks[kSurfBatch], any = 0;
        for (int k = 0; k < nb; k++) {
            B.m[k] = index_args(items[base + k]);
            blocks[k] = B.m[k].id_end > B.m[k].id_begin ? gridFor(B.m[k].id_end - B.m[k].id_begin) : 0;
            any += blocks[k];
        }
        if (any) index_splat_kernel<<<batch_layout(B, blocks, nb), kB, 0, s>>>(B, g);
    }
}
void launch_index_resolve_batch(hipStream_t s, const IndexPassArgs* items, int n_items, cf_cam cam, int cols, int rows)
{
    const FrameGeom g{cam, cols, rows};
    for (int base = 0; base < n_items; base += kSurfBatch) {
        const int nb = n_items - base < kSurfBatch ? n_items - base : kSurfBatch;
        Batch<IndexArgs> B;
        int blocks[kSurfBatch];
        for (int k = 0; k < nb; k++) { B.m[k] = index_args(items[base + k]); blocks[k] = gridFor((long long)cols * rows); }
        index_resolve_kernel<<<batch_layout(B, blocks, nb), kB, 0, s>>>(B, g);
    }
}
void launch_index_keys(hipStream_t s, const float* surfels, const unsigned* count, unsigned id_begin, unsigned id_end, const float t_inv[16],
                       cf_cam cam, int cols, int rows, float maxDepth, int time, int timeDelta, unsigned long long* keys)
{
    IndexPassArgs a{};
    a.surfels = surfels; a.count = count; a.id_begin = id_begin; a.id_end = id_end; for (int q = 0; q < 16; q++) a.t_inv[q] = t_inv[q];
    a.maxDepth = maxDepth; a.time = time; a.timeDelta = timeDelta; a.keys = keys;
    launch_index_keys_batch(s, &a, 1, cam, cols, rows);
}
void launch_index_resolve(hipStream_t s, const float* surfels, const float t_inv[16], int cols, int rows, unsigned long long* keys,
                          unsigned* index, float* vertConf, float* colorTime, float* normRad)
{
    IndexPassArgs a{};
    a.surfels = surfels; for (int q = 0; q < 16; q++) a.t_inv[q] = t_inv[q]; a.keys = keys; a.index = index; a.vertConf = vertConf; a.colorTime = colorTime;
    a.normRad = normRad;
    launch_index_resolve_batch(s, &a, 1, cf_cam{}, cols, rows);
}
void launch_predict_indices(hipStream_t s, const float* surfels, const unsigned* count, unsigned count_bound, const float t_inv[16], cf_cam cam,
                            int cols, int rows, float maxDepth, int time, int timeDelta, unsigned long long* keys, unsigned* index,
                            float* vertConf, float* colorTime, float* normRad)
{
    launch_index_keys(s, surfels, count, 0, count_bound, t_inv, cam, cols, rows, maxDepth, time, timeDelta, keys);
    launch_index_resolve(s, surfels, t_inv, cols, rows, keys, index, vertConf, colorTime, normRad);
}
void launch_combined_predict_batch(hipStream_t s, const SplatPassArgs* items, int n_items, cf_cam cam, int cols, int rows)
{
    const FrameGeom g{cam, cols, rows};
    for (int base = 0; base < n_items; base += kSurfBatch) {
        const int nb = n_items - base < kSurfBatch ? n_items - base : kSurfBatch;
        Batch<SplatArgs> B;
        int blocks[kSurfBatch], any = 0;
        for (int k = 0; k < nb; k++) {
            const SplatPassArgs& h = items[base + k];
            B.m[k] = SplatArgs{reinterpret_cast<const float4*>(h.surfels), h.count, mat4_from(h.t_inv), h.maxDepth, h.confThreshold, h.time, h.maxTime,
                               h.timeDelta, reinterpret_cast<const float4*>(h.rays), h.keys, reinterpret_cast<uchar4*>(h.image),
                               reinterpret_cast<float4*>(h.vertexConf), reinterpret_cast<float4*>(h.normalRad), h.time16, h.fill};
            blocks[k] = h.count_bound > 0 ? gridFor(4ll * h.count_bound) : 0;
            any += blocks[k];
        }
        if (any) splat_raster_kernel<<<batch_layout(B, blocks, nb), kB, 0, s>>>(B, g);
        for (int k = 0; k < nb; k++) blocks[k] = gridFor((long long)cols * rows);
        splat_resolve_kernel<<<batch_layout(B, blocks, nb), kB, 0, s>>>(B, g);
    }
}
void launch_combined_predict(hipStream_t s, const float* surfels, const unsigned* count, unsigned count_bound, const float t_inv[16], cf_cam cam,
                             int cols, int rows, float maxDepth, float confThreshold, int time, int maxTime, int timeDelta,
                             const float* rays, unsigned long long* keys, uint8_t* image, float* vertexConf, float* normalRad,
                             uint16_t* time16)
{
    SplatPassArgs a{};
    a.surfels = surfels; a.count = count; a.count_bound = count_bound; for (int q = 0; q < 16; q++) a.t_inv[q] = t_inv[q]; a.maxDepth = maxDepth;
    a.confThreshold = confThreshold; a.time = time; a.maxTime = maxTime; a.timeDelta = timeDelta; a.rays = rays; a.keys = keys; a.image = image;
    a.vertexConf = vertexConf; a.normalRad = normalRad; a.time16 = time16;
    launch_combined_predict_batch(s, &a, 1, cam, cols, rows);
}
void launch_splat_rays(hipStream_t s, cf_cam cam, int cols, int rows, float* rays)
{
    splat_rays_kernel<<<gridFor((long long)cols * rows), kB, 0, s>>>(cam, cols, rows, reinterpret_cast<float4*>(rays));
}
void launch_fill_in(hipStream_t s, const float* pv, const float* pn, const uint8_t* pimg, const float* depth, const uint8_t* rgba, int cols,
                    int rows, cf_cam cam, float inv_fx, float inv_fy, int pass_geom, int pass_rgb, float* ov, float* on, uint8_t* oi)
{
    fill_in_kernel<<<gridFor((long long)cols * rows), kB, 0, s>>>(
        reinterpret_cast<const float4*>(pv), reinterpret_cast<const float4*>(pn), reinterpret_cast<const uchar4*>(pimg), depth,
        reinterpret_cast<const uchar4*>(rgba), cols, rows, cam.cx, cam.cy, inv_fx, inv_fy, pass_geom, pass_rgb, reinterpret_cast<float4*>(ov),
        reinterpret_cast<float4*>(on), reinterpret_cast<uchar4*>(oi));
}
void launch_fill_ratio(hipStream_t s, const uint8_t* pimg, int cols, int rows, unsigned* out2, unsigned* out2_host)
{
    fill_ratio_kernel<<<1, 1024, 0, s>>>(reinterpret_cast<const uchar4*>(pimg), cols, rows, out2, out2_host);
}
void launch_associate_batch(hipStream_t s, const SurfelFuseArgs* items, int n_items)
{
    const int chunk = xcd_env("CF_XCD_ASSOC", 0);
    for (int base = 0; base < n_items; base += kSurfBatch) {
        const int nb = n_items - base < kSurfBatch ? n_items - base : kSurfBatch;
        Batch<FuseArgs> B;
        Batch<FillArgs> Z;
        int blocks[kSurfBatch], zblocks[kSurfBatch], zany = 0;
        for (int k = 0; k < nb; k++) {
            const SurfelFuseArgs& h = items[base + k];
            FuseArgs& a = B.m[k];
            a.index = h.index; a.vertConf = reinterpret_cast<const float4*>(h.vertConf); a.normRad = reinterpret_cast<const float4*>(h.normRad);
            a.rgba = reinterpret_cast<const uchar4*>(h.rgba); a.depth_raw = h.depth_raw; a.depth_filt = h.depth_filt; a.mask = h.mask;
            a.tcx = h.tcx; a.tcy = h.tcy; a.pose = mat4_from(h.pose); a.cam = h.cam; a.inv_fx = h.inv_fx; a.inv_fy = h.inv_fy;
            a.cols = h.cols; a.rows = h.rows; a.time = h.time; a.weighting = h.weighting; a.maskID = h.maskID; a.maxDepth = h.maxDepth;
            a.records = reinterpret_cast<float4*>(h.records); a.new_flags = h.new_flags; a.owner = h.owner;
            const int par = h.time % 2;
            const long long n = (long long)((h.cols - par + 1) / 2) * ((h.rows - par + 1) / 2);
            blocks[k] = gridXcd(4 * n, chunk);
            const long long n16 = ((long long)h.cols * h.rows + 3) / 4;
            Z.m[k] = FillArgs{reinterpret_cast<uint4*>(h.new_flags), n16};
            zblocks[k] = h.flags_clean ? 0 : gridFor(n16);
            zany += zblocks[k];
        }
        if (zany) fill_zero_kernel<<<batch_layout(Z, zblocks, nb), kB, 0, s>>>(Z);
        associate_kernel<<<batch_layout(B, blocks, nb), kB, 0, s>>>(B, chunk);
    }
}
void launch_associate(hipStream_t s, const SurfelFuseArgs& h) { launch_associate_batch(s, &h, 1); }
void launch_update_batch(hipStream_t s, const UpdatePassArgs* items, int n_items)
{
    for (int base = 0; base < n_items; base += kSurfBatch) {
        const int nb = n_items - base < kSurfBatch ? n_items - base : kSurfBatch;
        Batch<UpdateArgs> B;
        int blocks[kSurfBatch], any = 0;
        for (int k = 0; k < nb; k++) {
            const UpdatePassArgs& h = items[base + k];
            B.m[k] = UpdateArgs{reinterpret_cast<const float4*>(h.in), h.count, h.owner, reinterpret_cast<const float4*>(h.records), h.time,
                                reinterpret_cast<float4*>(h.out)};
            blocks[k] = h.count_bound > 0 ? gridFor(h.count_bound) : 0;
            any += blocks[k];
        }
        if (any) update_kernel<<<batch_layout(B, blocks, nb), kB, 0, s>>>(B);
    }
}
void launch_update(hipStream_t s, const float* in, const unsigned* count, unsigned count_bound, unsigned* owner, const float* records, int time,
                   float* out)
{
    const UpdatePassArgs a{in, count, count_bound, owner, records, time, out};
    launch_update_batch(s, &a, 1);
}
bool launch_update_compaction_index_keys(hipStream_t s, const UpdatePassArgs* up, const ScanPassArgs* sc, const IndexPassArgs* ix, int n, cf_cam cam, int cols,
                                         int rows)
{
    if (n <= 0 || n > kSurfBatch) return false;
    Batch<UpdateArgs> U; Batch<ScanArgs> S; Batch<IndexArgs> I;
    int ub[kSurfBatch], sb[kSurfBatch], ib[kSurfBatch];
    for (int k = 0; k < n; k++) {
        U.m[k] = UpdateArgs{reinterpret_cast<const float4*>(up[k].in), up[k].count, up[k].owner, reinterpret_cast<const float4*>(up[k].records), up[k].time,
                            reinterpret_cast<float4*>(up[k].out)};
        ub[k] = up[k].count_bound > 0 ? gridFor(up[k].count_bound) : 0;
        const ScanPassArgs& h = sc[k];
        S.m[k] = ScanArgs{reinterpret_cast<const float4*>(h.rec), h.flags, h.n, h.block_sums, h.total, h.add_to_total, reinterpret_cast<float4*>(h.out), h.total_host, h.zero_flags};
        sb[k] = (int)((h.n + kScanItems - 1) / kScanItems);
        if (sb[k] == 0) return false;
        I.m[k] = index_args(ix[k]);
        ib[k] = I.m[k].id_end > I.m[k].id_begin ? gridFor(I.m[k].id_end - I.m[k].id_begin) : 0;
    }
    const int ug = batch_layout(U, ub, n), sg = batch_layout(S, sb, n), ig = batch_layout(I, ib, n);
    const FrameGeom g{cam, cols, rows};
    update_blocksums_kernel<<<ug + sg, kB, 0, s>>>(U, S, ug);
    indexsplat_scatter_kernel<<<ig + sg, kB, 0, s>>>(I, g, S, ig);
    return true;
}
void launch_clean_batch(hipStream_t s, const CleanPassArgs* items, int n_items)
{
    const int chunk = xcd_env("CF_XCD_CLEAN", 64);
    for (int base = 0; base < n_items; base += kSurfBatch) {
        const int nb = n_items - base < kSurfBatch ? n_items - base : kSurfBatch;
        Batch<CleanArgs> B;
        int blocks[kSurfBatch], any = 0;
        for (int k = 0; k < nb; k++) {
            const CleanPassArgs& p = items[base + k];
            const SurfelCleanArgs& h = p.h;
            CleanArgs& a = B.m[k];
            a.index = h.index; a.vertConf = reinterpret_cast<const float4*>(h.vertConf); a.colorTime = reinterpret_cast<const float4*>(h.colorTime);
            a.rec = reinterpret_cast<const float4*>(h.rec);
            a.depth_filt = h.depth_filt; a.mask = h.mask; a.t_inv = mat4_from(h.t_inv); a.cam = h.cam; a.cols = h.cols; a.rows = h.rows; a.time = h.time;
            a.confThreshold = h.confThreshold; a.outlierCoeff = h.outlierCoeff; a.timeDelta = h.timeDelta; a.maskID = h.maskID;
            a.surfels = reinterpret_cast<const float4*>(p.surfels); a.count = p.count; a.fresh = reinterpret_cast<const float4*>(p.fresh);
            a.n_fresh = p.n_fresh; a.total_bound = p.total_bound; a.staged = reinterpret_cast<float4*>(p.staged); a.flags = p.flags;
            const int cchunk = chunk * (kB / kCleanB);
            const long long cgrid = (4ll * p.total_bound + kCleanB - 1) / kCleanB;
            a.xcd = cgrid >= 4ll * 8 * cchunk ? cchunk : 0;
#ifdef CF_ABLATE
            static const int clean_abl = getenv("CF_CLEAN_ABLATE") ? atoi(getenv("CF_CLEAN_ABLATE")) : 0;
            a.abl = clean_abl;
#endif
            { const int q = 8 * (a.xcd > 1 ? a.xcd : 1); blocks[k] = p.total_bound > 0 ? (int)((cgrid + q - 1) / q * q) : 0; }
            any += blocks[k];
        }
        if (any) clean_kernel<<<batch_layout(B, blocks, nb), kCleanB, 0, s>>>(B);
    }
}
void launch_clean(hipStream_t s, const float* surfels, const unsigned* count, const float* fresh, const unsigned* n_fresh, unsigned total_bound,
                  const SurfelCleanArgs& h, float* staged, unsigned* flags)
{
    const CleanPassArgs a{h, surfels, count, fresh, n_fresh, total_bound, staged, flags};
    launch_clean_batch(s, &a, 1);
}
void launch_set_count(hipStream_t s, unsigned* out, unsigned v) { set_count_kernel<<<1, 1, 0, s>>>(out, v); }

}
```

co_fusion_amd/facade.py:

```python
from __future__ import annotations

import ctypes as C
import os

import numpy as np
import torch

from . import lib as _libmod
from .api import Profile


class Config(C.Structure):
    _fields_ = [("width", C.c_int), ("height", C.c_int), ("fx", C.c_float), ("fy", C.c_float), ("cx", C.c_float), ("cy", C.c_float),
                ("device", C.c_int), ("max_surfels", C.c_int), ("max_models", C.c_int), ("conf_global_init", C.c_float),
                ("conf_object_init", C.c_float), ("depth_cutoff", C.c_float), ("icp_weight", C.c_float),
                ("outlier_coefficient", C.c_float), ("fast_odom", C.c_int), ("so3", C.c_int), ("frame_to_frame_rgb", C.c_int),
                ("pyramid", C.c_int), ("rgb_only", C.c_int), ("model_spawn_offset", C.c_uint), ("enable_multiple_models", C.c_int),
                ("enable_pose_logging", C.c_int), ("rank", C.c_int), ("world", C.c_int), ("device_frames_complete", C.c_int),
                ("mid_frame_predict", C.c_int), ("shard_background", C.c_int), ("enqueue_threads", C.c_int),
                ("colocate_background", C.c_int), ("reloc", C.c_int), ("early_index_maps", C.c_int), ("time_delta", C.c_int)]


class RedetectCandidate(C.Structure):
    _fields_ = [("id", C.c_uint), ("projected", C.c_uint32), ("occluded", C.c_uint32), ("seen_through", C.c_uint32), ("agree", C.c_uint32),
# ... 228 lines not shown

    def __del__(self):
        try:
            self.close()
        except Exception:
            pass

    def set_crf(self, unary_weight_error=75.0, unary_k_error=0.0375, threshold_new=5.5, weight_appearance=7.0, weight_smoothness=2.0,
                sigma_rgb=10.0, sigma_depth=0.9, sigma_pos=1.8, min_rel_size_new=0.015, max_rel_size_new=0.4, iterations=10):
        f = C.c_float
        self._check(self.lib.cofusion_set_crf(self.h, f(unary_weight_error), f(unary_k_error), f(threshold_new), f(weight_appearance),
                                              f(weight_smoothness), f(sigma_rgb), f(sigma_depth), f(sigma_pos), f(min_rel_size_new),
                                              f(max_rel_size_new), C.c_uint(iterations)))

    def set_seg_early(self, on=True):
        self._check(self.lib.cofusion_set_seg_early(self.h, 1 if on else 0))

    def process_frame(self, depth, rgb, mask=None, in_pose=None, timestamp=0):
        d = np.ascontiguousarray(depth, np.float32); c = np.ascontiguousarray(rgb, np.uint8)
        m = None if mask is None else np.ascontiguousarray(mask, np.uint8)
        p = None if in_pose is None else np.ascontiguousarray(in_pose, np.float32).reshape(16)
        self._check(self.lib.cofusion_process_frame(self.h, C.c_int64(timestamp), c.ctypes.data_as(C.c_void_p), d.ctypes.data_as(C.c_void_p),
                                                    None if m is None else m.ctypes.data_as(C.c_void_p),
                                                    None if p is None else p.ctypes.data_as(C.c_void_p)))

    def process_frame_device(self, depth_t, rgba_t, in_pose=None, timestamp=0, mask=None):
        p = None if in_pose is None else np.ascontiguousarray(in_pose, np.float32).reshape(16)
        if mask is not None:
            _check_mask_tensor(mask, depth_t)
            self._check(self.lib.cofusion_process_frame_device_masked(self.h, C.c_int64(timestamp), C.c_void_p(depth_t.data_ptr()),
                                                                      C.c_void_p(rgba_t.data_ptr()), C.c_void_p(mask.data_ptr()),
                                                                      None if p is None else p.ctypes.data_as(C.c_void_p)))
            return
        self._check(self.lib.cofusion_process_frame_device(self.h, C.c_int64(timestamp), C.c_void_p(depth_t.data_ptr()),
                                                           C.c_void_p(rgba_t.data_ptr()),
                                                           None if p is None else p.ctypes.data_as(C.c_void_p)))

    def process_frame_device_ptr(self, depth_ptr, rgba_ptr, mask_ptr=None, in_pose=None, timestamp=0):
        p = None if in_pose is None else np.ascontiguousarray(in_pose, np.float32).reshape(16)
        self._check(self.lib.cofusion_process_frame_device_masked(self.h, C.c_int64(timestamp), C.c_void_p(depth_ptr), C.c_void_p(rgba_ptr),
                                                                  C.c_void_p(mask_ptr) if mask_ptr else None,
                                                                  None if p is None else p.ctypes.data_as(C.c_void_p)))

    @property
    def num_models(self):
        return self.lib.cofusion_num_models(self.h)

    @property
    def tick(self):
        return self.lib.cofusion_tick(self.h)

    @property
    def lost(self):
        return bool(self.lib.cofusion_is_lost(self.h))

    def set_relocalisation(self, on=True, n_ferns=500, fern_threshold=0.3095, photo_threshold=115.0, min_age=300, seed=0, capacity=1024):
        self._check(self.lib.cofusion_set_relocalisation(self.h, int(bool(on)), int(n_ferns), C.c_float(fern_threshold), C.c_float(photo_threshold),
                                                         int(min_age), C.c_uint64(seed), int(capacity)))

    def reloc_stats(self):
        k = C.c_int(); c = C.c_int(); r = C.c_int(); f = C.c_int()
        self._check(self.lib.cofusion_reloc_stats(self.h, C.byref(k), C.byref(c), C.byref(r), C.byref(f)))
        return dict(keyframes=k.value, last_closest=c.value, recoveries=r.value, database_full=bool(f.value))

    def deform_background(self, src, dst, src_time, dst_time=None, pin=False, sample_rate=25000):
        from . import deform as _deform
        s = np.ascontiguousarray(src, np.float32).reshape(-1, 3); d = np.ascontiguousarray(dst, np.float32).reshape(-1, 3)
        ts = np.ascontiguousarray(src_time, np.float32).reshape(-1)
        td = None if dst_time is None else np.ascontiguousarray(dst_time, np.float32).reshape(-1)
        assert len(s) == len(d) == len(ts) and (td is None or len(td) == len(s))
        res = _deform.Result(); nodes = C.c_int()
        vp = lambda a: None if a is None else a.ctypes.data_as(C.c_void_p)
        self._check(self.lib.cofusion_deform_background(self.h, vp(s), vp(d), vp(ts), vp(td), len(s), int(bool(pin)), int(sample_rate), C.byref(res),
                                                        C.byref(nodes)))
        out = {k: getattr(res, k) for k in _deform.RESULT_FIELDS}
        for k in ("optimised", "accepted", "failed"):
            out[k] = bool(out[k])
        out["nodes"] = nodes.value
        return out

    def set_loop_closure(self, on=True, sample_rate=25000):
        self._check(self.lib.cofusion_set_loop_closure(self.h, int(bool(on)), int(sample_rate)))

    def loop_stats(self):
        from . import deform as _deform

        class _Stats(C.Structure):
            _fields_ = [(k, C.c_int32) for k in ("gated", "candidates", "fern_accepts", "optimised", "accepted", "failed", "last_keyframe",
                                                "last_keyframe_time", "last_nodes", "last_tick")] + [("last", _deform.Result)]
        s = _Stats()
        self._check(self.lib.cofusion_loop_stats(self.h, C.byref(s)))
        out = {k: getattr(s, k) for k, _ in _Stats._fields_[:-1]}
        last = {k: getattr(s.last, k) for k in _deform.RESULT_FIELDS}
        for k in ("optimised", "accepted", "failed"):
            last[k] = bool(last[k])
        out["last"] = last
        return out

    def set_redetection(self, on=True, min_fit=0.5, min_cover=0.044, depth_tol=0.10, max_candidates=8, keep_min_surfels=4000,
                        keep_conf_threshold=0.3):
        f = C.c_float
        self._check(self.lib.cofusion_set_redetection(self.h, int(bool(on)), f(min_fit), f(min_cover), f(depth_tol), int(max_candidates),
                                                      int(keep_min_surfels), f(keep_conf_threshold)))

    def redetect_stats(self):
        a = C.c_int(); r = C.c_int(); i = C.c_int()
        self._check(self.lib.cofusion_redetect_stats(self.h, C.byref(a), C.byref(r), C.byref(i)))
        return dict(attempts=a.value, reactivations=r.value, last_id=i.value)

    def redetect_last(self):
        cap = 16
        out = (RedetectCandidate * cap)()
        n = C.c_int(); px = C.c_uint32(); w = C.c_int()
        self._check(self.lib.cofusion_redetect_last(self.h, out, cap, C.byref(n), C.byref(px), C.byref(w)))
        cands = [{k: getattr(out[q], k) for k, _ in RedetectCandidate._fields_} for q in range(min(n.value, cap))]
        for c in cands:
            c["eligible"] = bool(c["eligible"])
        return dict(label_pixels=px.value, winner=w.value, candidates=cands)

    @property
    def num_inactive_models(self):
        return self.lib.cofusion_num_inactive_models(self.h)

    def model_info(self, index):
        mid = C.c_uint(); cnt = C.c_uint(); conf = C.c_float(); pose = (C.c_float * 16)()
        self._check(self.lib.cofusion_model_info(self.h, index, C.byref(mid), C.byref(cnt), pose, C.byref(conf)))
        return dict(id=mid.value, count=cnt.value, pose=np.array(pose, np.float32).reshape(4, 4), conf_threshold=conf.value)

    def model_cull_box(self, index):
        b = (C.c_int * 4)()
        self._check(self.lib.cofusion_model_cull_box(self.h, index, b))
        return list(b)

    def model_level0_visited(self, index):
        a = C.c_uint64(); b = C.c_uint64()
        self._check(self.lib.cofusion_model_level0_visited(self.h, index, C.byref(a), C.byref(b)))
        return int(a.value), int(b.value)

    def model_icp_stats(self, index):
        e = C.c_float(); c = C.c_float()
        self._check(self.lib.cofusion_model_icp_stats(self.h, index, C.byref(e), C.byref(c)))
        return e.value, c.value

    def model_tracking_inputs(self, index):
        H, W = self.height, self.width
        v = np.empty((H, W, 4), np.float32); n = np.empty((H, W, 4), np.float32); img = np.empty((H, W, 4), np.uint8)
        self._check(self.lib.cofusion_model_tracking_inputs(self.h, index, v.ctypes.data_as(C.c_void_p), n.ctypes.data_as(C.c_void_p),
                                                            img.ctypes.data_as(C.c_void_p)))
        return v, n, img

    def set_gn_mode(self, mode):
        assert self.abi.cf_set_gn_mode(self._ctx(), int(mode)) == 0

    def model_download(self, index):
        n = self.model_info(index)["count"]
        out = np.zeros((max(n, 1), 12), np.float32)
        c = C.c_uint32()
        self._check(self.lib.cofusion_model_download(self.h, index, out.ctypes.data_as(C.c_void_p), n, C.byref(c)))
        return out[:n]

    def mask(self):
        ptr = self.lib.cofusion_mask_device(self.h)
        host = np.empty(self.width * self.height, np.uint8)
        ctx = C.c_void_p(self.lib.cofusion_context(self.h))
        rc = self.abi.cf_memcpy_d2h(ctx, host.ctypes.data_as(C.c_void_p), C.c_void_p(ptr), C.c_uint64(host.size))
        if rc != 0:
            raise CoFusionError("mask readback failed")
        return host.reshape(self.height, self.width)

    def _ctx(self):
        return C.c_void_p(self.lib.cofusion_context(self.h))

    def set_icp_launch(self, threads, ppt):
        assert self.abi.cf_set_icp_launch(self._ctx(), threads, ppt) == 0

    def set_icp_arith(self, mode):
        assert self.abi.cf_set_icp_arith(self._ctx(), {"product": 0, "gram": 1, "reference": 2}.get(mode, mode)) == 0

    def profile_enable(self, on=True):
        assert self.abi.cf_profile_enable(self._ctx(), int(on)) == 0

    def profile_read(self, reset=True):
        p = Profile()
        assert self.abi.cf_profile_read(self._ctx(), C.byref(p), int(reset)) == 0
        return p


class CoFusionGroup:

    def __init__(self, n_sequences, width=640, height=480, fx=528.0, fy=528.0, cx=320.0, cy=240.0, device=0, **kw):
        if not torch.cuda.is_available():
            raise CoFusionError("no GPU visible: the Co-Fusion hot path has no CPU fallback")
        self.lib = _libmod.load_host()
        cfg = _make_config(self.lib, width, height, fx, fy, cx, cy, device, kw)
        self.device = torch.device("cuda", device)
        torch.cuda.set_device(self.device)
        self.n = int(n_sequences)
        self.g = C.c_void_p()
        if self.lib.cofusion_group_create(C.byref(cfg), self.n, C.byref(self.g)) != 0:
            raise CoFusionError(f"cofusion_group_create: {self.lib.cofusion_last_error().decode()}")
        self._check(self.lib.cofusion_group_set_stream(self.g, C.c_void_p(torch.cuda.current_stream(self.device).cuda_stream)))
        self.sequences = [CoFusion(width, height, fx, fy, cx, cy, device, _borrowed=self.lib.cofusion_group_sequence(self.g, s), **kw)
                          for s in range(self.n)]

    def _check(self, rc):
        if rc != 0:
            raise CoFusionError(f"cofusion error {rc}: {self.lib.cofusion_last_error().decode()}")

    def set_stream(self, stream):
        ptr = stream.cuda_stream if hasattr(stream, "cuda_stream") else int(stream)
        self._check(self.lib.cofusion_group_set_stream(self.g, C.c_void_p(ptr)))

    def process_frames(self, depths, rgbs, masks=None, timestamp=0):
        keep = [np.ascontiguousarray(d, np.float32) for d in depths] + [np.ascontiguousarray(r, np.uint8) for r in rgbs]
        mk = [None if (masks is None or m is None) else np.ascontiguousarray(m, np.uint8) for m in (masks or [None] * self.n)]
        P = C.c_void_p * self.n
        ts = (C.c_int64 * self.n)(*([timestamp] * self.n))
        self._check(self.lib.cofusion_group_process_frames(
            self.g, ts, P(*[r.ctypes.data for r in keep[self.n:]]), P(*[d.ctypes.data for d in keep[:self.n]]),
            P(*[None if m is None else m.ctypes.data for m in mk]) if masks is not None else None))

    def process_frames_device(self, depth_ts, rgba_ts, timestamp=0, masks=None):
        P = C.c_void_p * self.n
        ts = (C.c_int64 * self.n)(*([timestamp] * self.n))
        if masks is not None:
            for m, d in zip(masks, depth_ts):
                if m is not None:
                    _check_mask_tensor(m, d)
            self._check(self.lib.cofusion_group_process_frames_device_masked(
                self.g, ts, P(*[t.data_ptr() for t in depth_ts]), P(*[t.data_ptr() for t in rgba_ts]),
                P(*[None if m is None else m.data_ptr() for m in masks])))
            return
        self._check(self.lib.cofusion_group_process_frames_device(self.g, ts, P(*[t.data_ptr() for t in depth_ts]),
                                                                  P(*[t.data_ptr() for t in rgba_ts])))

    def close(self):
        if getattr(self, "g", None):
            for s in self.sequences:
                s.h = None
            self.lib.cofusion_group_destroy(self.g)
            self.g = None

    def __del__(self):
        try:
            self.close()
        except Exception:
            pass
```

co_fusion_amd/host/CoFusion.cpp:

```cpp
#include "CoFusion.h"
#include "ExportWriter.h"

#include <algorithm>
#include <chrono>

#include <cmath>
#include <cstdio>
#include <cstdlib>
#include <cstring>
#include <condition_variable>
#include <exception>
#include <functional>
#include <mutex>
#include <stdexcept>
#include <thread>

namespace cofusion {

PhaseTimes& phaseTimes() { static thread_local PhaseTimes t; return t; }
namespace {
struct PhaseTimer {
    int id; std::chrono::steady_clock::time_point t0 = std::chrono::steady_clock::now();
    explicit PhaseTimer(int i) : id(i) {}
    ~PhaseTimer() { phaseTimes().ms[id] += std::chrono::duration<double, std::milli>(std::chrono::steady_clock::now() - t0).count(); }
// ... 1111 lines not shown
            q[j] = (p.m[j * 4 + i] + p.m[i * 4 + j]) * t;
            q[k] = (p.m[k * 4 + i] + p.m[i * 4 + k]) * t;
            qx = q[0]; qy = q[1]; qz = q[2];
        }
        item.p[3] = qx; item.p[4] = qy; item.p[5] = qz; item.p[6] = qw;
        model->poseLog.push_back(item);
        first = false;
    }
}

bool CoFusion::processFrame(const FrameData& frame, const Mat4f* inPose, float weightMultiplier, bool bootstrap)
{
    const int frameTick = tick;
    frameBegin(frame, inPose, weightMultiplier, bootstrap);
    if (st.willTrack) { PhaseTimer t(PhaseTimes::Track); trackModels(st.pyr); }
    frameSegment(nullptr, nullptr);
    framePreIndex();
    frameCollect();
    frameFuse(true, 0);
    if (ferns) fernsAfterPredict();
    frameEnd();
    if (exportViewsWhich) exportViews(frameTick);
    return false;
}

void CoFusion::setRelocalisation(bool on, int nFerns, float fernThresh, float photoThresh, int minAge, uint64_t seed, int capacity)
{
    if (on && !cfg.reloc) throw std::runtime_error("setRelocalisation: needs Config::reloc (the failure detection that declares the camera lost)");
    if (on && dist.world > 1) throw std::runtime_error("setRelocalisation: a single-GPU option, like reloc");
    if (on && !ownsCtx) throw std::runtime_error("setRelocalisation: not available for a sequence of a lock-step group");
    if (ferns) { cf_ferns_destroy(ferns); ferns = nullptr; }
    lastFrameRecovery = false; fernLastClosest = -1; recoveries = 0;
    closeLoops = false; fernFirstAdd = -1; fernCount = 0; loopSt = LoopStats{};
    if (!on) return;
    cf_ferns_config fc{};
    fc.n_ferns = nFerns; fc.capacity = capacity; fc.max_depth_mm = (int)(cfg.depthCutoff * 1000.0f); fc.photo_threshold = photoThresh;
    check(ctx, cf_ferns_create(ctx, &fc, nullptr, seed, &ferns), "cf_ferns_create");
    fernThreshold = fernThresh; fernMinAge = minAge; fernCount = nFerns;
}

void CoFusion::setLoopClosure(bool on, int sampleRate)
{
    if (on && dist.world > 1) throw std::runtime_error("setLoopClosure: a single-GPU option, like reloc");
    if (on && !ownsCtx) throw std::runtime_error("setLoopClosure: not available for a sequence of a lock-step group");
    if (on && !ferns) throw std::runtime_error("setLoopClosure: needs setRelocalisation on (the keyframe database)");
    if (on && sampleRate < 1) throw std::runtime_error("setLoopClosure: sampleRate >= 1");
    if (on) {
        const int step = fernCount / 50;
        if (fernCount < 50 || (fernCount + step - 1) / step > CF_FERNS_MAX_SAMPLES)
            throw std::runtime_error("setLoopClosure: the fern count must be at least 50 and give at most 64 samples of stride n / 50");
        if (!deform) check(ctx, cf_deform_create(ctx, &deform), "cf_deform_create");
    }
    closeLoops = on;
    if (on) loopSampleRate = sampleRate;
    loopSt = LoopStats{};
}

void CoFusion::relocStats(int* keyframes, int* lastClosest, int* recoveriesOut, int* databaseFull)
{
    int count = 0, full = 0;
    if (ferns) check(ctx, cf_ferns_count(ferns, &count, &full), "cf_ferns_count");
    if (keyframes) *keyframes = count;
    if (lastClosest) *lastClosest = fernLastClosest;
    if (recoveriesOut) *recoveriesOut = recoveries;
    if (databaseFull) *databaseFull = full;
}

void CoFusion::fernsAfterPredict()
{
    Model& g = *globalModel;
    const float* v = static_cast<const float*>(mbuf(ctx, g.handle(), 8));
    const float* n = static_cast<const float*>(mbuf(ctx, g.handle(), 9));
    const uint8_t* img = static_cast<const uint8_t*>(mbuf(ctx, g.handle(), 10));
    if (!lost) {
        const bool gate = closeLoops && fernFirstAdd >= 0 && tick - fernFirstAdd > fernMinAge;
        if (fernFirstAdd < 0) fernFirstAdd = tick;
        if (!gate) {
            check(ctx, cf_ferns_add_async(ferns, v, n, img, g.getPose().m, tick, fernThreshold), "cf_ferns_add_async");
            return;
        }
        cf_ferns_gate rec{};
        check(ctx, cf_ferns_encode(ferns, v, n, img), "cf_ferns_encode");
        check(ctx, cf_ferns_search(ferns, tick, fernMinAge), "cf_ferns_search");
        check(ctx, cf_ferns_gate_async(ferns), "cf_ferns_gate_async");
        check(ctx, cf_ferns_gate_wait(ferns, &rec), "cf_ferns_gate_wait");
        loopSt.gated++;
        fernLastClosest = -1;
        if (rec.match_id >= 0 && rec.overlap > 0.3f) {
            loopSt.candidates++;
            if (closeLoop(rec)) return;
        }
        check(ctx, cf_ferns_append(ferns, g.getPose().m, tick, fernThreshold), "cf_ferns_append");
        return;
    }
    lastFrameRecovery = false;
    cf_ferns_result res{};
    check(ctx, cf_ferns_encode(ferns, v, n, img), "cf_ferns_encode");
    check(ctx, cf_ferns_relocalise(ferns, g.getPose().m, tick, fernMinAge, 1, &res), "cf_ferns_relocalise");
    fernLastClosest = res.accepted ? res.keyframe : -1;
    if (!res.accepted) return;
    Mat4f p;
    for (int i = 0; i < 16; i++) p.m[i] = res.pose[i];
    g.overridePose(p);
    lastFrameRecovery = true;
    fuseAndPredict(false, st.weightMultiplier, lost, true, 0);
}

int CoFusion::deformBackground(const float* src, const float* dst, const float* srcTime, const float* dstTime, int n, bool pin, int sampleRate,
                               cf_deform_result* result)
{
    if (dist.world > 1) throw std::runtime_error("deformBackground: a single-GPU option, like reloc");
    if (!ownsCtx) throw std::runtime_error("deformBackground: not available for a sequence of a lock-step group");
    if (!src || !dst || !srcTime || (pin && !dstTime) || n < 1 || n * (pin ? 2 : 1) > CF_DEFORM_MAX_CONSTRAINTS)
        throw std::runtime_error("deformBackground: 1..128 constraints (pins included), with their times");
    if (!curRgba || !depthFiltered_dev) throw std::runtime_error("deformBackground: no frame has been processed yet");
    if (!deform) check(ctx, cf_deform_create(ctx, &deform), "cf_deform_create");
    std::vector<float> s, d, t;
    for (int i = 0; i < n; i++) {
        s.insert(s.end(), src + 3 * i, src + 3 * i + 3); d.insert(d.end(), dst + 3 * i, dst + 3 * i + 3); t.push_back(srcTime[i]);
        if (pin) { s.insert(s.end(), dst + 3 * i, dst + 3 * i + 3); d.insert(d.end(), dst + 3 * i, dst + 3 * i + 3); t.push_back(dstTime[i]); }
    }
    cf_deform_result res{};
    const int nodes = deformMap(sampleRate > 0 ? sampleRate : 25000, [&] { return cf_deform_weights(deform, s.data(), d.data(), t.data(), (int)t.size()); },
                                lost ? 0 : 1, nullptr, 0, &res);
    if (result) *result = res;
    if (res.accepted) check(ctx, cf_synchronize(ctx), "cf_synchronize");
    return nodes;
}

int CoFusion::deformMap(int sampleRate, const std::function<int()>& weigh, int clockAhead, const Mat4f* correctedPose, int keyframes,
                        cf_deform_result* result)
{
    Model& g = *globalModel;
    uint32_t count = 0;
    check(ctx, cf_model_count(g.handle(), &count), "cf_model_count");
    float* map = static_cast<float*>(const_cast<void*>(mbuf(ctx, g.handle(), 11)));
    int nodes = 0, stride = 0, monotone = 0;
    check(ctx, cf_deform_sample(deform, map, count, sampleRate, &nodes, &stride, &monotone), "cf_deform_sample");
    cf_deform_result res{};
    if (result) *result = res;
    if (nodes < 5 || !monotone) return nodes;
    check(ctx, weigh(), "cf_deform_weights");
    check(ctx, cf_deform_optimise(deform, nullptr, &res), "cf_deform_optimise");
    if (result) *result = res;
    if (!res.accepted) return nodes;
    if (correctedPose) g.overridePose(*correctedPose);
    cf_deform_reactivate re{};
    for (int i = 0; i < 16; i++) re.pose[i] = g.getPose().m[i];
    re.cam = cf_cam{cfg.fx, cfg.fy, cfg.cx, cfg.cy}; re.cols = cfg.width; re.rows = cfg.height; re.max_depth = maxDepthProcessed;
    tick -= clockAhead;
    re.depth = depthFiltered_dev; re.conf_threshold = g.getConfidenceThreshold(); re.tick = tick;
    struct Restore { int& t; int a; ~Restore() { t += a; } } restore{tick, clockAhead};
    check(ctx, cf_deform_apply(deform, map, count, &re), "cf_deform_apply");
    if (keyframes > 0) {
        float* poses = nullptr; int32_t* times = nullptr;
        check(ctx, cf_ferns_keyframe_buffers(ferns, &poses, &times), "cf_ferns_keyframe_buffers");
        check(ctx, cf_deform_apply_poses(deform, poses, times, keyframes), "cf_deform_apply_poses");
    }
    fuseAndPredict(false, st.weightMultiplier, lost, true, 0);
    return nodes;
}

bool CoFusion::closeLoop(const cf_ferns_gate& gate)
{
    Model& g = *globalModel;
    cf_ferns_result res{};
    cf_ferns_closure cl{};
    check(ctx, cf_ferns_find_frame(ferns, g.getPose().m, tick, fernMinAge, 0, &res, &cl), "cf_ferns_find_frame");
    if (!res.accepted || cl.n_constraints < 1) return false;
    loopSt.fernAccepts++;
    loopSt.lastKeyframe = fernLastClosest = res.keyframe;
    loopSt.lastKeyframeTime = cl.keyframe_time;
    loopSt.lastTick = tick;
    float *src = nullptr, *dst = nullptr, *time = nullptr;
    check(ctx, cf_ferns_constraint_buffers(ferns, &src, &dst, &time), "cf_ferns_constraint_buffers");
    Mat4f est;
    for (int i = 0; i < 16; i++) est.m[i] = res.pose[i];
    cf_deform_result dr{};
    loopSt.lastNodes = deformMap(loopSampleRate, [&] { return cf_deform_weights_device(deform, src, dst, time, cl.n_constraints); }, 0, &est,
                                 gate.keyframes, &dr);
    loopSt.last = dr;
    loopSt.optimised += dr.optimised; loopSt.accepted += dr.accepted; loopSt.failed += dr.failed;
    if (!dr.accepted) return false;
    check(ctx, cf_ferns_add_async(ferns, static_cast<const float*>(mbuf(ctx, g.handle(), 8)), static_cast<const float*>(mbuf(ctx, g.handle(), 9)),
                                  static_cast<const uint8_t*>(mbuf(ctx, g.handle(), 10)), g.getPose().m, tick, fernThreshold), "cf_ferns_add_async");
    return true;
}

void CoFusion::framePreIndex()
{
    if (!cfg.earlyIndexMaps || !passesBatched() || trackPending.empty() || cfg.rgbOnly || lost) return;
    std::vector<cf_model_preindex> items;
    for (Model* m : trackPending) items.push_back(cf_model_preindex{m->model, m->odom, (int)tick});
    check(ctx, cf_models_preindex(ctx, items.data(), (int)items.size(), maxDepthProcessed, cfg.timeDelta), "cf_models_preindex");
}

CoFusionGroup::CoFusionGroup(const CoFusion::Config& c, int sequences) : cfg(c)
{
    if (sequences < 1 || sequences > 16) throw std::runtime_error("CoFusionGroup: 1..16 sequences");
    if (c.world > 1) throw std::runtime_error("CoFusionGroup: a group lives on one GPU (world == 1)");
    CoFusion::Config shared = c;
    shared.maxModels = c.maxModels * sequences;
    ctx = make_ctx(shared);
    try {
        for (int s = 0; s < sequences; s++) seqs.emplace_back(new CoFusion(c, ctx, s));
    } catch (...) { seqs.clear(); cf_destroy(ctx); throw; }
}

CoFusionGroup::~CoFusionGroup()
{
    seqs.clear();
    cf_destroy(ctx);
}

void CoFusionGroup::processFrames(const FrameData* frames, const Mat4f* const* inPoses)
{
    if (failed) throw std::runtime_error("CoFusionGroup: a previous processFrames failed part-way; the sequences are out of step (destroy the group)");
    try { stepAll(frames, inPoses); }
    catch (...) {
        failed = true;
        (void)cf_join(ctx);
        throw;
    }
}

void CoFusionGroup::stepAll(const FrameData* frames, const Mat4f* const* inPoses)
{
    const int S = (int)seqs.size();
    for (int s = 0; s < S; s++) seqs[s]->frameBegin(frames[s], inPoses ? inPoses[s] : nullptr, 1.f, false);
    {
        PhaseTimer t(PhaseTimes::Track);
        CoFusion::TrackBatch batch;
        for (int s = 0; s < S; s++) if (seqs[s]->frameTracks()) seqs[s]->trackCollect(batch);
        CoFusion::trackLaunch(ctx, batch, cfg);
    }
    {
        std::vector<cf_seg_job> jobs;
        std::vector<cf_seg_mask_job> maskJobs;
        std::vector<int> owner;
        jobs.reserve((size_t)S); maskJobs.reserve((size_t)S);
        for (int s = 0; s < S; s++) {
            const size_t before = jobs.size();
            seqs[s]->frameSegment(&jobs, &maskJobs);
            if (jobs.size() > before) owner.push_back(s);
        }
        if (!maskJobs.empty()) {
            check(ctx, cf_fork_after(ctx, 7, -1), "cf_fork_after");
            Segmentation::runMaskBatch(ctx, maskJobs);
            check(ctx, cf_join_lane(ctx, 7), "cf_join_lane");
        }
        std::vector<char> done(jobs.size(), 0);
        for (size_t a = 0; a < jobs.size(); a++) {
            if (done[a]) continue;
            const cf_seg_params Pa = seqs[owner[a]]->segmentation().deviceParams();
            std::vector<cf_seg_job> chain;
            for (size_t b = a; b < jobs.size(); b++) {
                if (done[b]) continue;
                const cf_seg_params Pb = seqs[owner[b]]->segmentation().deviceParams();
                if (memcmp(&Pa, &Pb, sizeof(Pa)) == 0) { chain.push_back(jobs[b]); done[b] = 1; }
            }
            Segmentation::runBatch(ctx, seqs[owner[a]]->segmentation(), chain);
        }
    }
    for (int s = 0; s < S; s++) seqs[s]->frameCollect();
    {
        PhaseTimer t(PhaseTimes::Fuse);
        std::vector<cf_model_pass> items;
        for (int s = 0; s < S; s++) seqs[s]->frameFuseCollect(items);
        check(ctx, cf_models_frame_passes(ctx, items.data(), (int)items.size(), seqs[0]->depthLimit(), cfg.outlierCoefficient, cfg.timeDelta),
              "cf_models_frame_passes");
        for (int s = 0; s < S; s++) seqs[s]->frameFuseFinish();
    }
    for (int s = 0; s < S; s++) seqs[s]->frameEnd();
}

}
```

co_fusion_amd/lib.py:

```python
from __future__ import annotations

import ctypes as C
import os
import subprocess

_HERE = os.path.dirname(os.path.abspath(__file__))
_LIB_DIR = os.environ.get("CF_LIB_DIR") or os.path.join(_HERE, "lib")
LIB_PATH = os.environ.get("CF_HIP_LIB") or os.path.join(_LIB_DIR, "libcofusion_hip.so")

SYMBOLS = [
    "cf_create", "cf_destroy", "cf_last_error", "cf_set_stream", "cf_use_own_stream", "cf_get_stream", "cf_synchronize", "cf_fork", "cf_main", "cf_join", "cf_join_lane", "cf_thread_lane", "cf_mark", "cf_event_wait_host", "cf_fork_after", "cf_malloc",
    "cf_free", "cf_memcpy_h2d", "cf_memcpy_d2h", "cf_malloc_host", "cf_free_host", "cf_memcpy_h2d_async", "cf_memcpy_d2h_async", "cf_memcpy_d2d_async", "cf_rgb_to_rgba", "cf_create_vmap", "cf_create_nmap", "cf_copy_maps", "cf_resize_map",
    "cf_transform_maps", "cf_vertices_to_depth", "cf_pyrdown_gauss_f32", "cf_pyrdown_gauss_u8",
    "cf_rgba_to_intensity", "cf_sobel", "cf_project_cloud", "cf_icp_step", "cf_icp_step_band", "cf_rgb_residual", "cf_rgb_step",
    "cf_so3_step", "cf_gn_solve_step", "cf_odom_create", "cf_odom_destroy", "cf_odom_init_icp_model", "cf_odom_init_rgb_model",
    "cf_odom_init_rgb", "cf_odom_init_models_batch", "cf_odom_init_models_batch_frames", "cf_odom_init_models_batch_select", "cf_model_fill_ratio_device", "cf_odom_init_first_rgb", "cf_odom_init_icp", "cf_odom_get_incremental_transformation",
    "cf_odom_track_batch_async", "cf_odom_fetch_result", "cf_odom_get_covariance", "cf_odom_bind_frame_maps", "cf_odom_share_frame_maps", "cf_odom_set_culling", "cf_odom_set_band", "cf_set_collective", "cf_model_predict_indices_sharded", "cf_odom_buffer",
    "cf_bilateral", "cf_model_create", "cf_model_destroy", "cf_model_initialise", "cf_model_count",
    "cf_model_predict_indices", "cf_model_index_keys", "cf_model_index_resolve", "cf_model_combined_predict", "cf_model_prefetch_fill_ratio", "cf_model_perform_fill_in", "cf_model_requires_fill_in",
    "cf_model_fuse", "cf_model_clean", "cf_models_frame_passes", "cf_models_preindex", "cf_model_download_map", "cf_model_upload_map", "cf_model_buffer",
    "cf_redetect_score", "cf_redetect_timing", "cf_relabel",
    "cf_fusion_weight", "cf_seg_create", "cf_seg_destroy", "cf_seg_slic", "cf_seg_crf", "cf_seg_sums", "cf_seg_infer", "cf_seg_early", "cf_seg_run_batch", "cf_seg_fetch", "cf_seg_publish_poses", "cf_seg_fetch_poses",
    "cf_seg_labels", "cf_seg_buffer", "cf_seg_create_masks", "cf_seg_masks", "cf_seg_masks_batch", "cf_seg_new_mask_value",
    "cf_depth_pyramid", "cf_set_icp_launch", "cf_set_icp_arith", "cf_get_icp_arith", "cf_set_gn_mode", "cf_profile_enable", "cf_profile_read", "cf_odom_bench_icp", "cf_odom_level0_visited", "cf_odom_last_launch_shape",
    "cf_rccl_unique_id", "cf_rccl_init", "cf_rccl_allreduce", "cf_rccl_broadcast", "cf_rccl_info", "cf_rccl_destroy",
    "cf_render_create", "cf_render_destroy", "cf_render", "cf_render_palette",
    "cf_ferns_table", "cf_ferns_create", "cf_ferns_destroy", "cf_ferns_get_table", "cf_ferns_encode", "cf_ferns_search", "cf_ferns_append", "cf_ferns_add_async",
    "cf_ferns_relocalise", "cf_ferns_count", "cf_ferns_download", "cf_ferns_last_search",
    "cf_frame_decoder_create", "cf_frame_decoder_destroy", "cf_frame_decoder_slot", "cf_frame_decoder_submit", "cf_frame_decoder_acquire", "cf_frame_decoder_timing",
    "cf_frame_decoder_enable_images", "cf_frame_decoder_image_slot", "cf_frame_decoder_submit_images", "cf_frame_decoder_acquire_mask", "cf_frame_decoder_image_timing",
    "cf_png_encoder_create", "cf_png_encoder_destroy", "cf_png_encoder_submit", "cf_png_encoder_acquire", "cf_png_encoder_timing",
    "cf_deform_create", "cf_deform_destroy", "cf_deform_default_thresholds", "cf_deform_sample", "cf_deform_set_nodes", "cf_deform_weights", "cf_deform_assemble",
    "cf_deform_iterate", "cf_deform_optimise", "cf_deform_apply", "cf_deform_apply_poses", "cf_deform_download", "cf_deform_weights_device",
    "cf_ferns_gate_async", "cf_ferns_gate_wait", "cf_ferns_constraints", "cf_ferns_find_frame", "cf_ferns_constraint_buffers", "cf_ferns_keyframe_buffers",
]


def build(verbose: bool = False) -> str:
    cmd = ["make", "-C", os.path.join(_HERE, "csrc"), "-j8"]
    if not verbose:
        cmd.insert(1, "-s")
    subprocess.check_call(cmd)
    cmd = ["make", "-C", os.path.join(_HERE, "host")]
    if not verbose:
        cmd.insert(1, "-s")
    subprocess.check_call(cmd)
    return LIB_PATH


HOST_LIB_PATH = os.path.join(_LIB_DIR, "libcofusion.so")
HOST_SYMBOLS = [
    "cofusion_default_config", "cofusion_create", "cofusion_destroy", "cofusion_last_error", "cofusion_set_stream",
    "cofusion_process_frame", "cofusion_process_frame_device", "cofusion_process_frame_device_masked", "cofusion_group_process_frames_device_masked", "cofusion_num_models", "cofusion_tick", "cofusion_model_info",
    "cofusion_model_download", "cofusion_model_icp_stats", "cofusion_model_cull_box", "cofusion_model_level0_visited", "cofusion_model_tracking_inputs", "cofusion_mask_device", "cofusion_context", "cofusion_set_crf", "cofusion_set_seg_early",
    "cofusion_save_ply", "cofusion_export_poses", "cofusion_set_export_segmentation", "cofusion_klg_open", "cofusion_klg_next", "cofusion_klg_set_reference_compatible", "cofusion_klg_close",
    "cofusion_klg_create", "cofusion_klg_write", "cofusion_klg_finish", "cofusion_debug_phase_ms", "cofusion_set_allreduce", "cofusion_set_allreduce_device", "cofusion_group_create", "cofusion_group_destroy", "cofusion_group_size", "cofusion_group_sequence", "cofusion_group_set_stream", "cofusion_group_process_frames", "cofusion_group_process_frames_device", "cofusion_rccl_unique_id", "cofusion_init_rccl", "cofusion_broadcast", "cofusion_model_owned", "cofusion_is_lost",
    "cofusion_render", "cofusion_render_device", "cofusion_set_export_views", "cofusion_set_export_async", "cofusion_export_flush", "cofusion_export_stats", "cofusion_set_relocalisation", "cofusion_reloc_stats", "cofusion_deform_background", "cofusion_set_loop_closure", "cofusion_loop_stats",
    "cofusion_set_redetection", "cofusion_redetect_stats", "cofusion_redetect_last", "cofusion_num_inactive_models",
    "cofusion_klg_player_open", "cofusion_klg_player_next", "cofusion_klg_player_process", "cofusion_klg_player_rewind", "cofusion_klg_player_set_limits", "cofusion_klg_player_close",
    "cofusion_jpeg_front", "cofusion_jpeg_finish_host", "cofusion_klg_prefetch_open", "cofusion_klg_prefetch_next", "cofusion_klg_prefetch_rewind", "cofusion_klg_prefetch_close",
    "cofusion_image_reader_open", "cofusion_image_reader_next", "cofusion_image_reader_rewind", "cofusion_image_reader_close",
    "cofusion_image_player_open", "cofusion_image_player_next", "cofusion_image_player_process", "cofusion_image_player_rewind", "cofusion_image_player_set_limits",
    "cofusion_image_player_times", "cofusion_image_player_close",
    "cofusion_image_prefetch_open", "cofusion_image_prefetch_next", "cofusion_image_prefetch_rewind", "cofusion_image_prefetch_close",
    "cofusion_png_decode", "cofusion_png_finish_host", "cofusion_exr_decode", "cofusion_exr_finish_host", "cofusion_ppm_decode",
]
_host = None


def load_host() -> C.CDLL:
    global _host
    if _host is None:
        load()
        if not os.path.exists(HOST_LIB_PATH):
            raise RuntimeError(f"{HOST_LIB_PATH} is missing: run __graft_entry__.build()")
        _host = C.CDLL(HOST_LIB_PATH)
        _host.cofusion_last_error.restype = C.c_char_p
        _host.cofusion_mask_device.restype = C.c_void_p
        _host.cofusion_context.restype = C.c_void_p
        _host.cofusion_group_sequence.restype = C.c_void_p
    return _host


_lib = None


def load() -> C.CDLL:
    global _lib
    if _lib is None:
        if not os.path.exists(LIB_PATH):
            raise RuntimeError(
                f"{LIB_PATH} is missing: build it with `python -c 'import __graft_entry__ as g; g.build()'` "
                "(there is no CPU fallback for the product path)")
        import torch
        _lib = C.CDLL(LIB_PATH)
        _lib.cf_last_error.restype = C.c_char_p
        _lib.cf_get_stream.restype = C.c_void_p
        pp = C.POINTER(C.c_void_p)
        _lib.cf_odom_init_models_batch_select.restype = C.c_int
        _lib.cf_odom_init_models_batch_select.argtypes = [C.c_void_p, pp, C.c_int, pp, pp, pp, pp, pp, pp, pp, C.c_float,
                                                          C.POINTER(C.POINTER(C.c_float)), pp]
        _lib.cf_models_frame_passes.restype = C.c_int
        _lib.cf_models_frame_passes.argtypes = [C.c_void_p, C.c_void_p, C.c_int, C.c_float, C.c_float, C.c_int]
        _lib.cf_models_preindex.restype = C.c_int
        _lib.cf_models_preindex.argtypes = [C.c_void_p, C.c_void_p, C.c_int, C.c_float, C.c_int]
    return _lib
```

co_fusion_amd/model.py:

```python
from __future__ import annotations

import ctypes as C

import numpy as np
import torch

from .api import Context, Odometry, _f, _p

SURFEL = 12
TIME_DELTA = 2 ** 31 // 2 - 1

class ModelPass(C.Structure):
    _fields_ = [("model", C.c_void_p), ("pose", C.POINTER(C.c_float)), ("rgba", C.c_void_p), ("mask", C.c_void_p), ("depth_raw", C.c_void_p),
                ("depth_filtered", C.c_void_p), ("do_fuse", C.c_int), ("time", C.c_int), ("fuse_max_depth", C.c_float), ("weighting", C.c_float),
                ("mask_id", C.c_int), ("conf_threshold", C.c_float), ("fill_in", C.c_int), ("passthrough_geom", C.c_int),
                ("passthrough_rgb", C.c_int)]


class ModelPreindex(C.Structure):
    _fields_ = [("model", C.c_void_p), ("odom", C.c_void_p), ("time", C.c_int)]


def frame_passes(ctx: Context, items, depth_cutoff, outlier_coeff, time_delta=None):
    n = len(items)
    arr = (ModelPass * n)()
    keep = []
    for a, it in zip(arr, items):
        pose = _f(np.asarray(it["pose"], np.float32).reshape(16))
        keep.append(pose)
        a.model = it["model"].h
        a.pose = C.cast(pose, C.POINTER(C.c_float))
        a.rgba, a.mask = _p(it["rgba"]), _p(it.get("mask"))
        a.depth_raw, a.depth_filtered = _p(it.get("depth_raw")), _p(it["depth_filt"])
        a.do_fuse = int(it.get("do_fuse", 1))
        a.time = int(it["time"])
        a.fuse_max_depth = float(it.get("fuse_max_depth", depth_cutoff))
        a.weighting = float(it.get("weighting", 1.0))
        a.mask_id = int(it.get("mask_id", 0))
        a.conf_threshold = float(it["conf_threshold"])
        a.fill_in, a.passthrough_geom, a.passthrough_rgb = int(it.get("fill_in", 0)), int(it.get("passthrough_geom", 0)), int(it.get("passthrough_rgb", 0))
    ctx._check(ctx.lib.cf_models_frame_passes(ctx.h, arr, n, C.c_float(depth_cutoff), C.c_float(outlier_coeff),
                                              int(TIME_DELTA if time_delta is None else time_delta)))


def preindex(ctx: Context, items, depth_cutoff, time_delta=None):
    n = len(items)
    arr = (ModelPreindex * n)()
    for a, (m, od, time) in zip(arr, items):
        a.model, a.odom, a.time = m.h, od.h, int(time)
    ctx._check(ctx.lib.cf_models_preindex(ctx.h, arr, n, C.c_float(depth_cutoff), int(TIME_DELTA if time_delta is None else time_delta)))


_BUF = {0: (np.uint32, 1), 1: (np.float32, 4), 2: (np.float32, 4), 3: (np.float32, 4), 4: (np.uint8, 4), 5: (np.float32, 4),
        6: (np.float32, 4), 7: (np.uint16, 1), 8: (np.float32, 4), 9: (np.float32, 4), 10: (np.uint8, 4)}


def bilateral(ctx: Context, depth, max_d):
    rows, cols = depth.shape
    out = ctx.empty((rows, cols))
    ctx._check(ctx.lib.cf_bilateral(ctx.h, _p(depth), cols, rows, C.c_float(max_d), _p(out)))
    return out


def fusion_weight(ctx: Context, pose, last_pose, mult):
    ctx.lib.cf_fusion_weight.restype = C.c_float
    return float(ctx.lib.cf_fusion_weight(_f(np.asarray(pose, np.float32).reshape(16)), _f(np.asarray(last_pose, np.float32).reshape(16)),
                                          C.c_float(mult)))


class Model:
    def __init__(self, ctx: Context, max_surfels=1 << 20):
        self.ctx = ctx
        self.h = C.c_void_p()
        ctx._check(ctx.lib.cf_model_create(ctx.h, int(max_surfels), C.byref(self.h)))

    def close(self):
        if getattr(self, "h", None) and self.ctx.h:
            self.ctx.lib.cf_model_destroy(self.h)
        self.h = None

    def __del__(self):
        try:
            self.close()
        except Exception:
            pass

    def _pose(self, pose):
        return _f(np.asarray(pose, np.float32).reshape(16))

    def initialise(self, rgba, depth_raw, depth_filt, time, max_depth):
        self.ctx._check(self.ctx.lib.cf_model_initialise(self.h, _p(rgba), _p(depth_raw), _p(depth_filt), time, C.c_float(max_depth)))

    def count(self):
        c = C.c_uint32()
        self.ctx._check(self.ctx.lib.cf_model_count(self.h, C.byref(c)))
        return c.value

    def predict_indices(self, pose, time, max_depth, time_delta=TIME_DELTA):
        self.ctx._check(self.ctx.lib.cf_model_predict_indices(self.h, self._pose(pose), time, C.c_float(max_depth), time_delta))

    def index_keys(self, pose, time, max_depth, surfel_begin, surfel_end, time_delta=TIME_DELTA):
        keys = torch.empty((self.ctx.height, self.ctx.width), dtype=torch.int64, device=self.ctx.device)
        self.ctx._check(self.ctx.lib.cf_model_index_keys(self.h, self._pose(pose), time, C.c_float(max_depth), time_delta,
                                                         int(surfel_begin), int(surfel_end), C.c_void_p(keys.data_ptr())))
        return keys

    def index_resolve(self, pose, keys):
        self.ctx._check(self.ctx.lib.cf_model_index_resolve(self.h, self._pose(pose), C.c_void_p(keys.data_ptr())))

    def combined_predict(self, pose, max_depth, conf_threshold, time, max_time, time_delta=TIME_DELTA):
        self.ctx._check(self.ctx.lib.cf_model_combined_predict(self.h, self._pose(pose), C.c_float(max_depth), C.c_float(conf_threshold),
                                                               time, max_time, time_delta))

    def perform_fill_in(self, rgba, depth_filt, pass_geom=False, pass_rgb=False):
        self.ctx._check(self.ctx.lib.cf_model_perform_fill_in(self.h, _p(rgba), _p(depth_filt), int(pass_geom), int(pass_rgb)))

    def prefetch_fill_ratio(self):
        self.ctx._check(self.ctx.lib.cf_model_prefetch_fill_ratio(self.h))

    def fill_counts_device(self):
        ptr = C.c_void_p()
        self.ctx._check(self.ctx.lib.cf_model_fill_ratio_device(self.h, C.byref(ptr)))
        if not ptr.value:
            return None
        host = np.empty(2, np.uint32)
        self.ctx._check(self.ctx.lib.cf_memcpy_d2h(self.ctx.h, host.ctypes.data_as(C.c_void_p), ptr, C.c_uint64(8)))
        return host

    def requires_fill_in(self, ratio=0.75):
        out = C.c_int()
        self.ctx._check(self.ctx.lib.cf_model_requires_fill_in(self.h, C.c_float(ratio), C.byref(out)))
        return bool(out.value)

    def fuse(self, pose, time, rgba, mask, depth_raw, depth_filt, max_depth, weighting, mask_id):
        self.ctx._check(self.ctx.lib.cf_model_fuse(self.h, self._pose(pose), time, _p(rgba), _p(mask), _p(depth_raw), _p(depth_filt),
                                                   C.c_float(max_depth), C.c_float(weighting), mask_id))

    def clean(self, pose, time, conf_threshold, outlier_coeff, depth_filt, mask, mask_id, time_delta=TIME_DELTA):
        c = C.c_uint32()
        self.ctx._check(self.ctx.lib.cf_model_clean(self.h, self._pose(pose), time, C.c_float(conf_threshold), C.c_float(outlier_coeff),
                                                    time_delta, _p(depth_filt), _p(mask), mask_id, C.byref(c)))
        return c.value

    def download_map(self):
        n = self.count()
        out = np.zeros((max(n, 1), SURFEL), np.float32)
        c = C.c_uint32()
        self.ctx._check(self.ctx.lib.cf_model_download_map(self.h, out.ctypes.data_as(C.c_void_p), n, C.byref(c)))
        return out[:n]

    def upload_map(self, surfels):
        s = np.ascontiguousarray(surfels, np.float32).reshape(-1, SURFEL)
        self.ctx._check(self.ctx.lib.cf_model_upload_map(self.h, s.ctypes.data_as(C.c_void_p), s.shape[0]))

    def tensor(self, which):
        ptr = C.c_void_p(); nbytes = C.c_uint64()
        self.ctx._check(self.ctx.lib.cf_model_buffer(self.h, which, C.byref(ptr), C.byref(nbytes)))
        return ptr.value, nbytes.value

    def buffer(self, which):
        ptr, nbytes = self.tensor(which)
        host = np.empty(nbytes, np.uint8)
        if nbytes:
            self.ctx._check(self.ctx.lib.cf_memcpy_d2h(self.ctx.h, host.ctypes.data_as(C.c_void_p), C.c_void_p(ptr), C.c_uint64(nbytes)))
        h, w = self.ctx.height, self.ctx.width
        if which in (11, 12):
            return host.view(np.float32).reshape(-1, SURFEL)
        if which == 13:
            return host.view(np.float32).reshape(h, w, 8)
        dt, ch = _BUF[which]
        a = host.view(dt)
        return a.reshape(h, w, ch) if ch > 1 else a.reshape(h, w)


class _DevView:

    def __init__(self, ptr):
        self._ptr = ptr
        self.is_cuda = True

    def is_contiguous(self):
        return True

    def data_ptr(self):
        return self._ptr
```

include/cofusion_hip.h:

```cpp
#ifndef COFUSION_HIP_H_
#define COFUSION_HIP_H_

#include <stdint.h>

#ifdef __cplusplus
extern "C" {
#endif

#define CF_OK 0
#define CF_EINVAL (-1)
#define CF_EHIP (-2)
#define CF_ENOMEM (-3)
#define CF_ESTATE (-4)

#define CF_NUM_PYRS 3
#define CF_SE3_WORDS 32
#define CF_SO3_WORDS 16
#define CF_FIX_ICP 32
#define CF_FIX_RGB_MAX 32
static inline int CF_FIX_RGB_BITS(float sigma)
{
    union { float f; uint32_t u; } v;
    int F;
    if (sigma == -1.0f || !(sigma >= 2.0f)) return 8;
// ... 68 lines not shown
int cf_transform_maps(cf_ctx *ctx, float *vmap, float *nmap, int cols, int rows, const float R[9], const float t[3]);
int cf_vertices_to_depth(cf_ctx *ctx, const float *vertex4, int cols, int rows, float cutoff, float *depth);
int cf_pyrdown_gauss_f32(cf_ctx *ctx, const float *src, int src_cols, int src_rows, float *dst);
int cf_pyrdown_gauss_u8(cf_ctx *ctx, const uint8_t *src, int src_cols, int src_rows, uint8_t *dst);
int cf_rgba_to_intensity(cf_ctx *ctx, const uint8_t *rgba, int cols, int rows, uint8_t *dst);
int cf_sobel(cf_ctx *ctx, const uint8_t *src, int cols, int rows, int16_t *dx, int16_t *dy);
int cf_project_cloud(cf_ctx *ctx, const float *depth, int cols, int rows, cf_cam intr_level, float *cloud3);

int cf_icp_step(cf_ctx *ctx, const float Rcurr[9], const float tcurr[3], const float *vmap_curr,
                const float *nmap_curr, const float Rprev_inv[9], const float tprev[3], cf_cam intr,
                const float *vmap_g_prev, const float *nmap_g_prev, float dist_thres, float angle_thres,
                int cols, int rows, float *A_host, float *b_host, float *residual_host, int64_t *sums_host,
                float *err_surface);
int cf_icp_step_band(cf_ctx *ctx, const float Rcurr[9], const float tcurr[3], const float *vmap_curr,
                     const float *nmap_curr, const float Rprev_inv[9], const float tprev[3], cf_cam intr,
                     const float *vmap_g_prev, const float *nmap_g_prev, float dist_thres, float angle_thres,
                     int cols, int rows, int row_begin, int row_end, float *A_host, float *b_host,
                     float *residual_host, int64_t *sums_host, float *err_surface);
int cf_rgb_residual(cf_ctx *ctx, float min_scale, const int16_t *dIdx, const int16_t *dIdy, const float *last_depth,
                    const float *next_depth, const uint8_t *last_image, const uint8_t *next_image,
                    cf_dataterm *corres, float max_depth_delta, const float kt[3], const float krkinv[9],
                    int cols, int rows, int *sigma_sum_host, int *count_host);
int cf_rgb_step(cf_ctx *ctx, const cf_dataterm *corres, float sigma, const float *cloud3, float fx, float fy,
                const int16_t *dIdx, const int16_t *dIdy, float sobel_scale, int cols, int rows, float *A_host,
                float *b_host, int64_t *sums_host);
int cf_so3_step(cf_ctx *ctx, const uint8_t *last_image, const uint8_t *next_image, const float image_basis[9],
                const float kinv[9], const float krlr[9], int cols, int rows, float *A_host, float *b_host,
                float *residual_host, int64_t *sums_host);

typedef struct {
    int rgb_only, pyramid, fast_odom, so3;
    float icp_weight;
} cf_track_opts;
typedef struct {
    float last_icp_error, last_icp_count, last_rgb_error, last_rgb_count, last_so3_error, last_so3_count;
    double lastA[36], lastb[6];
    int so3_iterations;
    int fault;
    int cull_box[4];
} cf_track_stats;

int cf_odom_create(cf_ctx *ctx, cf_odom **out);
void cf_odom_destroy(cf_odom *od);
int cf_odom_init_icp_model(cf_odom *od, const float *pred_vertex4, const float *pred_normal4, const float pose[16]);
int cf_odom_init_rgb_model(cf_odom *od, const uint8_t *pred_rgba);
int cf_odom_init_rgb(cf_odom *od, const uint8_t *rgba);
int cf_odom_init_first_rgb(cf_odom *od, const uint8_t *rgba);
int cf_odom_init_models_batch(cf_ctx *ctx, cf_odom *const *ods, int n, const float *const *pred_vertex4,
                              const float *const *pred_normal4, const uint8_t *const *pred_rgba, const float *const *poses ,
                              const uint8_t *frame_rgba);
int cf_odom_init_models_batch_frames(cf_ctx *ctx, cf_odom *const *ods, int n, const float *const *pred_vertex4,
                                     const float *const *pred_normal4, const uint8_t *const *pred_rgba, const float *const *poses ,
                                     const uint8_t *const *frame_rgba );
int cf_odom_init_models_batch_select(cf_ctx *ctx, cf_odom *const *ods, int n, const float *const *pred_vertex4,
                                     const float *const *pred_normal4, const uint8_t *const *pred_rgba,
                                     const float *const *alt_vertex4, const float *const *alt_normal4, const uint8_t *const *alt_rgba,
                                     const uint32_t *const *fill_counts, float ratio, const float *const *poses ,
                                     const uint8_t *const *frame_rgba );
int cf_odom_init_icp(cf_odom *od, const float *const depth_pyr[CF_NUM_PYRS], float depth_cutoff);
int cf_odom_get_incremental_transformation(cf_odom *od, float trans[3], float rot[9], const cf_track_opts *opts,
                                           float *icp_err_surface, cf_track_stats *stats);
int cf_odom_track_batch_async(cf_ctx *ctx, cf_odom *const *ods, int n, const float *const *poses_in ,
                              const cf_track_opts *opts, float *const *icp_err_surfaces );
int cf_odom_fetch_result(cf_odom *od, float trans[3], float rot[9], cf_track_stats *stats);
int cf_odom_get_covariance(const cf_track_stats *stats, double cov[36]);

typedef struct {
    cf_cam intr;
    int32_t width, height;
    int32_t icp, rgb, rgbOnly;
    float icpWeight;
    float Rprev[9], tprev[3], Rprev_inv[9], Rcurr[9], tcurr[3];
    double resultRt[16];
    float krkInv[9], kt[3];
    float lastRGBError;
    int32_t level_done, solves;
    float residual[2];
    float cull_z[2];
    float pose_inv[16];
    cf_track_stats stats;
} cf_gn_state;
typedef struct {
    int64_t icp_acc[64 * 32];
    int64_t rgb_acc[64 * 32];
    cf_gn_state state;
    cf_gn_state twin;
    uint32_t hot[48];
} cf_gn_system;
int cf_gn_solve_step(cf_ctx *ctx, int n, cf_gn_system *systems, int next_level, int last_of_level, int icp_fix);
int cf_odom_level0_visited(cf_odom *od, uint64_t *icp_pixels, uint64_t *residual_pixels);
int cf_odom_last_launch_shape(cf_odom *od, int icp_blocks[3], int residual_blocks[3], int *icp_blocks_err);
int cf_odom_set_culling(cf_odom *od, int on);
typedef int (*cf_collective_fn)(void *user, int op, void *dev_buf, uint64_t words, void *hip_stream);
int cf_set_collective(cf_ctx *ctx, cf_collective_fn fn, void *user);
int cf_odom_set_band(cf_odom *od, int row_begin, int row_end, int add_counts);
#define CF_RCCL_ID_BYTES 128
int cf_rccl_unique_id(void *id128);
int cf_rccl_init(cf_ctx *ctx, const void *id128, int rank, int world);
int cf_rccl_allreduce(cf_ctx *ctx, void *dev_buf, uint64_t words, int op, void *hip_stream);
int cf_rccl_broadcast(cf_ctx *ctx, void *dev_buf, uint64_t bytes, int root, void *hip_stream);
int cf_rccl_info(const cf_ctx *ctx, int *rank, int *world, int *rccl_version);
int cf_rccl_destroy(cf_ctx *ctx);
int cf_odom_bind_frame_maps(cf_odom *od, const float *const vmaps[CF_NUM_PYRS], const float *const nmaps[CF_NUM_PYRS]);
int cf_odom_share_frame_maps(cf_odom *od, cf_odom *owner);
int cf_odom_buffer(cf_odom *od, int which, int level, void **dptr, uint64_t *bytes);
int cf_depth_pyramid(cf_ctx *ctx, const float *depth_filtered, int cols, int rows, float *l1, float *l2);

int cf_bilateral(cf_ctx *ctx, const float *depth, int cols, int rows, float maxD, float *out);

int cf_model_create(cf_ctx *ctx, int max_surfels, cf_model **out);
void cf_model_destroy(cf_model *m);
int cf_model_initialise(cf_model *m, const uint8_t *rgba, const float *depth_raw, const float *depth_filtered, int time,
                        float maxDepth);
int cf_model_count(cf_model *m, uint32_t *count);
int cf_model_predict_indices(cf_model *m, const float pose[16], int time, float maxDepth, int timeDelta);
int cf_model_index_keys(cf_model *m, const float pose[16], int time, float maxDepth, int timeDelta, uint32_t surfel_begin,
                        uint32_t surfel_end, uint64_t *keys_dev);
int cf_model_index_resolve(cf_model *m, const float pose[16], uint64_t *keys_dev);
int cf_model_predict_indices_sharded(cf_model *m, const float pose[16], int time, float maxDepth, int timeDelta, int shard, int nshards);
int cf_model_combined_predict(cf_model *m, const float pose[16], float maxDepth, float confThreshold, int time, int maxTime,
                              int timeDelta);
int cf_model_prefetch_fill_ratio(cf_model *m);
int cf_model_perform_fill_in(cf_model *m, const uint8_t *rgba, const float *depth_filtered, int passthrough_geom,
                             int passthrough_rgb);
int cf_model_requires_fill_in(cf_model *m, float ratio, int *out);
int cf_model_fill_ratio_device(cf_model *m, const uint32_t **counts_dev);
int cf_model_fuse(cf_model *m, const float pose[16], int time, const uint8_t *rgba, const uint8_t *mask, const float *depth_raw,
                  const float *depth_filtered, float maxDepth, float weighting, int maskID);
int cf_model_clean(cf_model *m, const float pose[16], int time, float confThreshold, float outlierCoeff, int timeDelta,
                   const float *depth_filtered, const uint8_t *mask, int maskID, uint32_t *count_out);
typedef struct {
    cf_model *model;
    const float *pose;
    const uint8_t *rgba, *mask;
    const float *depth_raw, *depth_filtered;
    int do_fuse;
    int time;
    float fuse_max_depth;
    float weighting;
    int mask_id;
    float conf_threshold;
    int fill_in, passthrough_geom, passthrough_rgb;
} cf_model_pass;
int cf_models_frame_passes(cf_ctx *ctx, const cf_model_pass *items, int n, float depth_cutoff, float outlier_coeff, int time_delta);
typedef struct {
    cf_model *model;
    const cf_odom *odom;
    int time;
} cf_model_preindex;
int cf_models_preindex(cf_ctx *ctx, const cf_model_preindex *items, int n, float depth_cutoff, int time_delta);
int cf_model_download_map(cf_model *m, float *host_surfels, uint32_t capacity, uint32_t *count);
int cf_model_upload_map(cf_model *m, const float *host_surfels, uint32_t count);
int cf_model_buffer(cf_model *m, int which, void **dptr, uint64_t *bytes);
typedef struct { uint32_t projected, occluded, seen_through, agree, agree_on_label, covered; } cf_redetect_counts;
typedef struct {
    cf_model *model;
    float pose[16];
    float conf_threshold;
} cf_redetect_candidate;
typedef struct {
    const float *depth;
    const uint8_t *label;
    int cols, rows;
    cf_cam cam;
    int new_label;
    float depth_cutoff, depth_tol;
} cf_redetect_frame;
int cf_redetect_score(cf_ctx *ctx, const cf_redetect_candidate *candidates, int n, const cf_redetect_frame *frame, cf_redetect_counts *counts ,
                      uint32_t *label_pixels);
int cf_redetect_timing(cf_ctx *ctx, int on, float *last_ms);
int cf_relabel(cf_ctx *ctx, uint8_t *label_dev, uint64_t n, int from, int to);
float cf_fusion_weight(const float pose[16], const float lastPose[16], float weightMultiplier);

typedef struct cf_segmenter cf_segmenter;
int cf_seg_create(cf_ctx *ctx, cf_segmenter **out);
void cf_seg_destroy(cf_segmenter *s);
int cf_seg_slic(cf_segmenter *s, const uint8_t *rgba);
int cf_seg_crf(cf_segmenter *s, const float *unary_host, int L, const float *feat_smooth_host, const float *feat_app_host,
               float w_smooth, float w_app, int iterations, float *Q_host);
typedef struct {
    float unaryWeightError, unaryKError, unaryThresholdNew;
    float weightAppearance, weightSmoothness;
    float scaleFeaturesRGB, scaleFeaturesDepth, scaleFeaturesPos;
    float minRelSizeNew, maxRelSizeNew;
    int crfIterations;
} cf_seg_params;
#define CF_SEG_MAX_ENTRIES 256
typedef struct {
    uint32_t id, superPixelCount;
    float avgConfidence, depthMean, depthStd;
    int32_t top, right, bottom, left;
} cf_seg_model;
typedef struct {
    int32_t has_new_label, n_models;
    float depth_range;
    cf_seg_model model[CF_SEG_MAX_ENTRIES];
} cf_seg_result;
int cf_seg_sums(cf_segmenter *s, const float *depth, int n_models, const float *const *icp_err, const float *const *vertconf4,
                int64_t **sums_dev, uint64_t *sums_words);
int cf_seg_infer(cf_segmenter *s, const cf_seg_params *params, const uint8_t *rgba, int n_models, const uint32_t *model_ids,
                 uint32_t next_model_id, int allow_new, uint8_t *full_dev);
int cf_seg_fetch(cf_segmenter *s, cf_seg_result *out, uint8_t *low_map_host);
int cf_seg_early(cf_segmenter *s, const float *depth, const uint8_t *rgba, int n_models, const float *const *vertconf4,
                 const cf_seg_params *params);
typedef struct cf_seg_job {
    cf_segmenter *seg;
    const float *depth;
    int32_t n_models;
    const float *const *icp_err;
    const float *const *vertconf4;
    const uint8_t *rgba;
    const uint32_t *model_ids;
    uint32_t next_model_id;
    int32_t allow_new;
    uint8_t *full_dev;
} cf_seg_job;
int cf_seg_run_batch(cf_ctx *ctx, const cf_seg_params *params, const cf_seg_job *jobs, int n_jobs);
int cf_seg_publish_poses(cf_segmenter *s, int n_models, cf_odom *const *trackers);
int cf_seg_fetch_poses(cf_segmenter *s, int n_models, int64_t *words_host);
int cf_seg_labels(cf_segmenter *s, void **dptr, uint64_t *bytes);
int cf_seg_buffer(cf_segmenter *s, int which, void **dptr, uint64_t *bytes);
typedef struct cf_seg_mask_job {
    cf_segmenter *seg;
    const uint8_t *mask_dev;
    const float *depth_dev;
    int32_t n_models;
    const uint32_t *model_ids;
    uint32_t next_model_id;
    int32_t allow_new;
    const uint8_t *mapping;
    uint8_t *full_dev;
} cf_seg_mask_job;
int cf_seg_create_masks(cf_ctx *ctx, cf_segmenter **out);
int cf_seg_masks(const cf_seg_mask_job *job);
int cf_seg_masks_batch(cf_ctx *ctx, const cf_seg_mask_job *jobs, int n_jobs);
int cf_seg_new_mask_value(cf_segmenter *s, int *value);

int cf_set_gn_mode(cf_ctx *ctx, int mode);
int cf_set_icp_launch(cf_ctx *ctx, int threads, int pixels_per_thread);
#define CF_ICP_ARITH_PRODUCT 0
#define CF_ICP_ARITH_GRAM 1
#define CF_ICP_ARITH_REFERENCE 2
int cf_set_icp_arith(cf_ctx *ctx, int mode);
int cf_get_icp_arith(cf_ctx *ctx);

typedef struct cf_renderer cf_renderer;
#define CF_RENDER_MAX_ITEMS 256
#define CF_RENDER_MAX_COLOUR 8
#define CF_RENDER_UNSTABLE 1
#define CF_RENDER_WINDOW 2
#define CF_RENDER_PHONG 4
#define CF_RENDER_GREY 0
#define CF_RENDER_NORMALS 1
#define CF_RENDER_COLOUR 2
#define CF_RENDER_TIMES 3
#define CF_RENDER_LABEL 4
#define CF_RENDER_ITEM_MODE (-1)
#define CF_RENDER_RGBA 0
#define CF_RENDER_DEPTH 1
#define CF_RENDER_LABELS 2
typedef struct {
    float pose[16];
    float fx, fy, cx, cy;
    int width, height;
    float near_z, far_z;
    int flags;
    int tick, time_delta;
} cf_render_view;
typedef struct {
    const float *surfels;
    uint32_t count;
    float pose[16];
    float conf_threshold;
    int model_id;
    int colour_mode;
} cf_render_item;
typedef struct {
    void *dst;
    int kind;
    int mode;
} cf_render_output;
int cf_render_create(cf_ctx *ctx, int max_w, int max_h, cf_renderer **out);
void cf_render_destroy(cf_renderer *r);
int cf_render(cf_renderer *r, const cf_render_view *view, const cf_render_item *items, int n_items, const cf_render_output *outputs,
              int n_outputs);
int cf_render_palette(uint8_t *rgb768);

#define CF_FERNS_MAX 2048
typedef struct cf_ferns cf_ferns;
typedef struct {
    int32_t x, y;
    int32_t r, g, b;
    int32_t d;
} cf_fern;
typedef struct {
    int n_ferns;
    int capacity;
    int max_depth_mm;
    float photo_threshold;
} cf_ferns_config;
typedef struct {
    int accepted;
    int keyframe;
    float dissimilarity;
    float overlap;
    float pose[16];
// ... 157 lines not shown
```

Measured before the change: 930.2.

## Cull index-resolve wavefronts outside the projected screen extent of each model

Result: faster. 944.2, median of 6 (+1.5%).

```diff
diff --git a/co_fusion_amd/csrc/cabi_model.hip b/co_fusion_amd/csrc/cabi_model.hip
--- a/co_fusion_amd/csrc/cabi_model.hip
+++ b/co_fusion_amd/csrc/cabi_model.hip
@@ -52,6 +52,31 @@
     void drop_preindex() { preindex_od = nullptr; preindex_time = -1; }
     float* rays = nullptr;
     float inv_fx = 0, inv_fy = 0;
+    unsigned* d_ext = nullptr;
+    int ext_k = 0;
+    bool ext_unknown = true;
+    void extents_unknown() { ext_unknown = true; }
+};
+static int next_extent(cf_model* m, bool on, uint32_t nb, hipStream_t s, unsigned** ext, int* ext_slot)
+{
+    *ext = nullptr; *ext_slot = 0;
+    if (2ull * nb >= (unsigned long long)m->ctx->cfg.width * m->ctx->cfg.height) on = false;
+    if (!on) { m->ext_unknown = true; return CF_OK; }
+    const bool full = m->ext_unknown;
+    if (full) HIPCHK(m->ctx, hipMemsetAsync(m->d_ext, 0, 12 * sizeof(unsigned), s));
+    *ext = m->d_ext; *ext_slot = m->ext_k | (full ? 4 : 0);
+    m->ext_k = (m->ext_k + 1) % 3;
+    m->ext_unknown = false;
+    return CF_OK;
+}
+static bool extent_culling_on(const cf_ctx* ctx)
+{
+    static const bool env_on = getenv("CF_NO_EXTENT_CULL") == nullptr;
+    return env_on && ctx->extent_cull && !ctx->collective && !ctx->rccl;
+}
+struct ExtentGuard {
+    std::vector<cf_model*> models; bool done = false;
+    ~ExtentGuard() { if (!done) for (cf_model* m : models) if (m) m->extents_unknown(); }
 };
 
 using cf::inv44f;
@@ -110,6 +135,7 @@
     if (int r = dmalloc(ctx, &m->tcy, (size_t)H)) return r;
     if (int r = dmalloc(ctx, &m->rays, N * 4)) return r;
     if (int r = dmalloc(ctx, &m->t_inv_dev, 16)) return r;
+    if (int r = dmalloc(ctx, &m->d_ext, 12)) return r;
     launch_splat_rays(ctx->cur(), ctx_cam(ctx), W, H, m->rays);
     HIPCHK(ctx, hipHostMalloc(reinterpret_cast<void**>(&m->h_counts), sizeof(unsigned) * 4, hipHostMallocCoherent));
     HIPCHK(ctx, hipEventCreateWithFlags(&m->count_event, hipEventDisableTiming));
@@ -131,7 +157,7 @@
     void* ptrs[] = {m->buf[0], m->buf[1], m->staged, m->flags, m->block_sums, m->d_count, m->d_nfresh, m->d_tmp2, m->records,
                     m->fresh, m->new_flags, m->owner, m->fb_rec, m->fb_raw, m->fb_filt, m->keys, m->index, m->vertConf,
                     m->colorTime, m->normRad, m->splat_image, m->splat_vertex, m->splat_normal, m->splat_time, m->fill_vertex,
-                    m->fill_normal, m->fill_image, m->tcx, m->tcy, m->rays, m->t_inv_dev, m->clean_rec};
+                    m->fill_normal, m->fill_image, m->tcx, m->tcy, m->rays, m->t_inv_dev, m->clean_rec, m->d_ext};
     for (void* p : ptrs) (void)hipFree(p);
     (void)hipHostFree(m->h_counts);
     if (m->count_event) (void)hipEventDestroy(m->count_event);
@@ -187,6 +213,7 @@
 {
     if (!m || !rgba || !depth_raw || !depth_filt) return CF_EINVAL;
     m->drop_preindex();
+    m->extents_unknown();
     cf_ctx* ctx = m->ctx; hipStream_t s = ctx->cur();
     const int W = ctx->cfg.width, H = ctx->cfg.height; const long long N = (long long)W * H;
     if ((uint32_t)N > m->max_surfels) return CF_ENOMEM;
@@ -209,6 +236,7 @@
 {
     if (!m || !pose) return CF_EINVAL;
     m->drop_preindex();
+    m->extents_unknown();
     cf_ctx* ctx = m->ctx;
     float t_inv[16];
     inv44f(pose, t_inv);
@@ -225,6 +253,7 @@
 {
     if (!m || !pose || !keys_dev || surfel_begin > surfel_end) return CF_EINVAL;
     m->drop_preindex();
+    m->extents_unknown();
     cf_ctx* ctx = m->ctx;
     const int W = ctx->cfg.width, H = ctx->cfg.height;
     float t_inv[16];
@@ -241,6 +270,7 @@
 {
     if (!m || !pose || !keys_dev) return CF_EINVAL;
     m->drop_preindex();
+    m->extents_unknown();
     cf_ctx* ctx = m->ctx;
     float t_inv[16];
     inv44f(pose, t_inv);
@@ -331,6 +361,7 @@
 {
     if (!m || !pose || !rgba || !mask || !depth_raw || !depth_filt) return CF_EINVAL;
     m->drop_preindex();
+    m->extents_unknown();
     cf_ctx* ctx = m->ctx; hipStream_t s = ctx->cur();
     const int W = ctx->cfg.width, H = ctx->cfg.height; const long long N = (long long)W * H;
     SurfelFuseArgs a;
@@ -358,6 +389,7 @@
 {
     if (!m || !pose || !depth_filt || !mask) return CF_EINVAL;
     m->drop_preindex();
+    m->extents_unknown();
     cf_ctx* ctx = m->ctx; hipStream_t s = ctx->cur();
     const int W = ctx->cfg.width, H = ctx->cfg.height;
     uint32_t nb = 0;
@@ -384,9 +416,13 @@
     hipStream_t s = ctx->cur();
     const int W = ctx->cfg.width, H = ctx->cfg.height;
     std::vector<IndexPassArgs> a((size_t)n);
+    for (int k = 0; k < n; k++)
+        if (!items[k].model || !items[k].odom || items[k].model->ctx != ctx || items[k].odom->ctx != ctx) return CF_EINVAL;
+    ExtentGuard guard;
+    for (int k = 0; k < n; k++) guard.models.push_back(items[k].model);
+    const bool cull = extent_culling_on(ctx);
     for (int k = 0; k < n; k++) {
         cf_model* m = items[k].model; const cf_odom* od = items[k].odom;
-        if (!m || !od || m->ctx != ctx || od->ctx != ctx) return CF_EINVAL;
         uint32_t nb = 0;
         if (int r = count_bound(m, &nb)) return r;
         const float* pinv = reinterpret_cast<const float*>(reinterpret_cast<const char*>(od->d_state) + offsetof(cf::OdomDev, pose_inv));
@@ -394,6 +430,7 @@
         p.surfels = m->buf[m->target]; p.count = m->d_count; p.id_begin = 0; p.id_end = nb; p.maxDepth = depth_cutoff; p.time = items[k].time;
         p.timeDelta = time_delta; p.keys = m->keys; p.index = m->index; p.vertConf = m->vertConf; p.colorTime = m->colorTime; p.normRad = m->normRad;
         p.t_inv_dev = pinv;
+        if (int r = next_extent(m, cull, nb, s, &p.ext, &p.ext_slot)) return r;
     }
     launch_index_keys_batch(s, a.data(), n, ctx_cam(ctx), W, H);
     launch_index_resolve_batch(s, a.data(), n, ctx_cam(ctx), W, H);
@@ -402,6 +439,7 @@
         cf_model* m = items[k].model;
         m->preindex_od = items[k].odom; m->preindex_time = items[k].time; m->preindex_cutoff = depth_cutoff; m->preindex_delta = time_delta; m->preindex_nb = a[k].id_end;
     }
+    guard.done = true;
     return CF_OK;
 }
 static bool preindexed_with(const cf_model* m, const float pose[16], int time, float depth_cutoff, int time_delta, uint32_t nb)
@@ -437,6 +475,9 @@
         }
     }
     for (int k = 0; k < n; k++) { uint32_t nb = 0; if (int r = count_bound(items[k].model, &nb)) return r; }
+    ExtentGuard guard;
+    for (int k = 0; k < n; k++) guard.models.push_back(items[k].model);
+    const bool cull = extent_culling_on(ctx);
     int surf_ev = -1;
     if (ctx->prof.enabled > 0 && (ctx->surf_calls_seen++ % (unsigned)ctx->prof.enabled) == 0 && ctx->surf_used + 2 <= cf_ctx::kSurfEvents) {
         for (int e = ctx->surf_used; e < ctx->surf_used + 2; e++)
@@ -458,6 +499,7 @@
             p.time = it.time; p.timeDelta = time_delta; p.keys = m->keys; p.index = m->index; p.vertConf = m->vertConf; p.colorTime = m->colorTime;
             p.normRad = m->normRad;
             if (feeds_clean && clean_rec_on) { p.clean_rec = m->clean_rec; p.clean_depth = it.depth_filtered; }
+            if (int r = next_extent(m, cull, nb, s, &p.ext, &p.ext_slot)) return r;
         }
         return CF_OK;
     };
@@ -564,6 +606,7 @@
         for (int k : fusing) items[k].model->count_wait = ctx->batch_event;
     }
     for (int k = 0; k < n; k++) items[k].model->drop_preindex();
+    guard.done = true;
     return CF_OK;
 }
 
@@ -584,6 +627,7 @@
 {
     if (!m || (!host_surfels && count) || count > m->max_surfels) return CF_EINVAL;
     m->drop_preindex();
+    m->extents_unknown();
     cf_ctx* ctx = m->ctx;
     if (count) HIPCHK(ctx, hipMemcpyAsync(m->buf[m->target], host_surfels, (size_t)count * 48, hipMemcpyHostToDevice, ctx->cur()));
     launch_set_count(ctx->cur(), m->d_count, count);
@@ -618,9 +662,23 @@
             p = m->fresh; b = (size_t)nf * 48; break;
         }
         case 13: p = m->clean_rec; b = N * 32; break;
+        case 14: p = m->keys; b = N * 8; break;
         default: return CF_EINVAL;
     }
     *dptr = p; if (bytes) *bytes = b;
+    return CF_OK;
+}
+
+int cf_set_extent_culling(cf_ctx* ctx, int on)
+{
+    if (!ctx) return CF_EINVAL;
+    ctx->extent_cull = on != 0;
+    return CF_OK;
+}
+int cf_model_extents_unknown(cf_model* m)
+{
+    if (!m) return CF_EINVAL;
+    m->extents_unknown();
     return CF_OK;
 }
 
diff --git a/co_fusion_amd/csrc/cf_host.h b/co_fusion_amd/csrc/cf_host.h
--- a/co_fusion_amd/csrc/cf_host.h
+++ b/co_fusion_amd/csrc/cf_host.h
@@ -38,6 +38,7 @@
     cf::OdomDev* h_state_pool = nullptr;
     bool slot_used[kStateSlots]{};
     hipEvent_t batch_event = nullptr;
+    bool extent_cull = true;
     static constexpr int kLanes = 8;
     hipStream_t lanes[kLanes]{};
     hipEvent_t lane_done[kLanes]{};
diff --git a/co_fusion_amd/csrc/cf_kernels.h b/co_fusion_amd/csrc/cf_kernels.h
--- a/co_fusion_amd/csrc/cf_kernels.h
+++ b/co_fusion_amd/csrc/cf_kernels.h
@@ -285,6 +285,8 @@
     const float* t_inv_dev;
     float* clean_rec;
     const float* clean_depth;
+    unsigned* ext;
+    int ext_slot;
 };
 __host__ __device__ inline void inv44f(const float a[16], float o[16])
 {
diff --git a/co_fusion_amd/csrc/surfel.hip b/co_fusion_amd/csrc/surfel.hip
--- a/co_fusion_amd/csrc/surfel.hip
+++ b/co_fusion_amd/csrc/surfel.hip
@@ -83,8 +83,8 @@
 
 static constexpr int kScanItems = 2048;
 struct ScanArgs {
-    const float4* rec; const unsigned* flags; long long n; unsigned* block_sums; unsigned* total; unsigned add_to_total; float4* out;
-    unsigned* total_host; int zero_flags;
+    const float4* rec; const unsigned* flags; long long n; unsigned* block_sums; unsigned* total; unsigned add_to_total; int zero_flags;
+    float4* out; unsigned* total_host;
 };
 __device__ __forceinline__ void scan_load_flags(const unsigned* __restrict__ flags, long long i0, long long n, unsigned (&f)[8])
 {
@@ -196,7 +196,7 @@
         int blocks[kSurfBatch], any = 0;
         for (int k = 0; k < nb; k++) {
             const ScanPassArgs& h = items[base + k];
-            B.m[k] = ScanArgs{reinterpret_cast<const float4*>(h.rec), h.flags, h.n, h.block_sums, h.total, h.add_to_total, reinterpret_cast<float4*>(h.out), h.total_host, h.zero_flags};
+            B.m[k] = ScanArgs{reinterpret_cast<const float4*>(h.rec), h.flags, h.n, h.block_sums, h.total, h.add_to_total, h.zero_flags, reinterpret_cast<float4*>(h.out), h.total_host};
             blocks[k] = (int)((B.m[k].n + kScanItems - 1) / kScanItems);
             any += blocks[k];
             if (blocks[k] == 0) set_count2_kernel<<<1, 1, 0, s>>>(B.m[k].total, B.m[k].total_host, B.m[k].add_to_total);
@@ -246,6 +246,33 @@
     out[k * 3 + 2] = filt[k * 3 + 2];
 }
 
+extern "C" __device__ unsigned int __ockl_wfred_max_u32(unsigned int);
+__device__ __forceinline__ unsigned extent_peek(const unsigned* e) { return __hip_atomic_load(&e[threadIdx.x & 3], __ATOMIC_RELAXED, __HIP_MEMORY_SCOPE_AGENT); }
+__device__ __forceinline__ void extent_extend(unsigned* __restrict__ e, unsigned peeked, bool ok, int x_lo, int y_lo, int x_hi, int y_hi)
+{
+    const unsigned k0 = __ockl_wfred_max_u32(ok ? ~(unsigned)x_lo : 0u), k1 = __ockl_wfred_max_u32(ok ? ~(unsigned)y_lo : 0u);
+    const unsigned k2 = __ockl_wfred_max_u32(ok ? (unsigned)x_hi + 1u : 0u), k3 = __ockl_wfred_max_u32(ok ? (unsigned)y_hi + 1u : 0u);
+    const int lane = threadIdx.x & 63;
+    if (lane < 4) {
+        const unsigned key = lane == 0 ? k0 : lane == 1 ? k1 : lane == 2 ? k2 : k3;
+        if (key > peeked) atomicMax(&e[lane], key);
+    }
+}
+__device__ __forceinline__ bool extent_meets(const unsigned* __restrict__ e, int x0, int x1, int y0, int y1)
+{
+    const unsigned nx = e[0], ny = e[1], mx = e[2], my = e[3];
+    return (unsigned)x0 < mx && (unsigned)y0 < my && (unsigned)x1 >= ~nx && (unsigned)y1 >= ~ny;
+}
+__device__ __forceinline__ bool extent_culled(unsigned* __restrict__ ext, int ext_slot, int bid, int q0, int cols, int n_texels)
+{
+    const int slot = ext_slot & 3, next = slot == 2 ? 0 : slot + 1, prev = slot == 0 ? 2 : slot - 1;
+    if (bid == 0 && threadIdx.x < 4) ext[4 * next + threadIdx.x] = 0u;
+    if (ext_slot & 4) return false;
+    const int q1 = min(q0 + 63, n_texels - 1), y0 = q0 / cols, y1 = q1 / cols;
+    const int x0 = y0 == y1 ? q0 - y0 * cols : 0, x1 = y0 == y1 ? q1 - y0 * cols : cols - 1;
+    return !extent_meets(ext + 4 * slot, x0, x1, y0, y1) && !extent_meets(ext + 4 * prev, x0, x1, y0, y1);
+}
+
 __device__ __forceinline__ bool index_project(const float4 pc, const float4 ct, const Mat4& t_inv, cf_cam cam, int cols, int rows,
                                               float maxDepth, int time, int timeDelta, f3& ph, int& q)
 {
@@ -255,9 +282,11 @@
 
 struct IndexArgs {
     const float4* surfels; const unsigned* count; Mat4 t_inv; float maxDepth; int time, timeDelta; unsigned id_begin, id_end;
+    int ext_slot;
     unsigned long long* keys; unsigned* index; float4* vertConf; float4* colorTime; float4* normRad;
     const float* t_inv_dev;
     float4* clean_rec; const float* clean_depth;
+    unsigned* ext;
 };
 __device__ __forceinline__ Mat4 index_matrix(const IndexArgs& a)
 {
@@ -275,11 +304,18 @@
     const IndexArgs& a = B.m[vb.model];
     const float4* __restrict__ surfels = a.surfels;
     const unsigned id = a.id_begin + vb.bid * kB + threadIdx.x;
-    if (id >= *a.count || id >= a.id_end) return;
-    f3 ph; int q;
-    const Mat4 T = index_matrix(a);
-    if (!index_project(surfels[id * 3], surfels[id * 3 + 1], T, g.cam, g.cols, g.rows, a.maxDepth, a.time, a.timeDelta, ph, q)) return;
-    atomicMin(&a.keys[q], zkey(ph.z, id));
+    unsigned* const slot = a.ext ? a.ext + 4 * (a.ext_slot & 3) : nullptr;
+    const unsigned peeked = slot ? extent_peek(slot) : 0u;
+    bool ok = id < *a.count && id < a.id_end;
+    f3 ph; int q = 0;
+    if (ok) {
+        const Mat4 T = index_matrix(a);
+        ok = index_project(surfels[id * 3], surfels[id * 3 + 1], T, g.cam, g.cols, g.rows, a.maxDepth, a.time, a.timeDelta, ph, q);
+    }
+    if (ok) atomicMin(&a.keys[q], zkey(ph.z, id));
+    if (!slot || __ballot(ok) == 0) return;
+    const int y = q / g.cols, x = q - y * g.cols;
+    extent_extend(slot, peeked, ok, x, y, x, y);
 }
 __global__ void __launch_bounds__(kB) index_splat_kernel(const Batch<IndexArgs> B, const FrameGeom g) { index_splat_body(B, g, (int)blockIdx.x); }
 
@@ -290,6 +326,16 @@
     const float4* __restrict__ surfels = a.surfels; unsigned long long* __restrict__ keys = a.keys; unsigned* __restrict__ index = a.index;
     float4* __restrict__ vertConf = a.vertConf; float4* __restrict__ colorTime = a.colorTime; float4* __restrict__ normRad = a.normRad;
     const int q = vb.bid * kB + threadIdx.x;
+    if (a.ext) {
+        const int q0 = __builtin_amdgcn_readfirstlane(q & ~63);
+        if (q0 >= g.cols * g.rows) return;
+        if (extent_culled(a.ext, a.ext_slot, vb.bid, q0, g.cols, g.cols * g.rows)) {
+            if (a.clean_rec && q < g.cols * g.rows) {
+                a.clean_rec[2 * q] = make_float4(0, 0, 0, 0); a.clean_rec[2 * q + 1] = make_float4(0, 0, __uint_as_float(0u), a.clean_depth[q]);
+            }
+            return;
+        }
+    }
     if (q >= g.cols * g.rows) return;
     const unsigned long long k = keys[q];
     keys[q] = kEmptyKey;
@@ -921,8 +967,8 @@
 static IndexArgs index_args(const IndexPassArgs& h)
 {
     return IndexArgs{reinterpret_cast<const float4*>(h.surfels), h.count, mat4_from(h.t_inv), h.maxDepth, h.time, h.timeDelta, h.id_begin, h.id_end,
-                     h.keys, h.index, reinterpret_cast<float4*>(h.vertConf), reinterpret_cast<float4*>(h.colorTime), reinterpret_cast<float4*>(h.normRad),
-                     h.t_inv_dev, reinterpret_cast<float4*>(h.clean_rec), h.clean_depth};
+                     h.ext_slot, h.keys, h.index, reinterpret_cast<float4*>(h.vertConf), reinterpret_cast<float4*>(h.colorTime),
+                     reinterpret_cast<float4*>(h.normRad), h.t_inv_dev, reinterpret_cast<float4*>(h.clean_rec), h.clean_depth, h.ext};
 }
 void launch_index_keys_batch(hipStream_t s, const IndexPassArgs* items, int n_items, cf_cam cam, int cols, int rows)
 {
@@ -1082,7 +1128,7 @@
                             reinterpret_cast<float4*>(up[k].out)};
         ub[k] = up[k].count_bound > 0 ? gridFor(up[k].count_bound) : 0;
         const ScanPassArgs& h = sc[k];
-        S.m[k] = ScanArgs{reinterpret_cast<const float4*>(h.rec), h.flags, h.n, h.block_sums, h.total, h.add_to_total, reinterpret_cast<float4*>(h.out), h.total_host, h.zero_flags};
+        S.m[k] = ScanArgs{reinterpret_cast<const float4*>(h.rec), h.flags, h.n, h.block_sums, h.total, h.add_to_total, h.zero_flags, reinterpret_cast<float4*>(h.out), h.total_host};
         sb[k] = (int)((h.n + kScanItems - 1) / kScanItems);
         if (sb[k] == 0) return false;
         I.m[k] = index_args(ix[k]);
diff --git a/co_fusion_amd/facade.py b/co_fusion_amd/facade.py
--- a/co_fusion_amd/facade.py
+++ b/co_fusion_amd/facade.py
@@ -404,6 +404,9 @@
     def set_gn_mode(self, mode):
         assert self.abi.cf_set_gn_mode(self._ctx(), int(mode)) == 0
 
+    def set_extent_culling(self, on=True):
+        assert self.abi.cf_set_extent_culling(self._ctx(), int(bool(on))) == 0
+
     def model_download(self, index):
         n = self.model_info(index)["count"]
         out = np.zeros((max(n, 1), 12), np.float32)
diff --git a/co_fusion_amd/host/CoFusion.cpp b/co_fusion_amd/host/CoFusion.cpp
--- a/co_fusion_amd/host/CoFusion.cpp
+++ b/co_fusion_amd/host/CoFusion.cpp
@@ -1287,6 +1287,7 @@
     re.depth = depthFiltered_dev; re.conf_threshold = g.getConfidenceThreshold(); re.tick = tick;
     struct Restore { int& t; int a; ~Restore() { t += a; } } restore{tick, clockAhead};
     check(ctx, cf_deform_apply(deform, map, count, &re), "cf_deform_apply");
+    check(ctx, cf_model_extents_unknown(g.handle()), "cf_model_extents_unknown");
     if (keyframes > 0) {
         float* poses = nullptr; int32_t* times = nullptr;
         check(ctx, cf_ferns_keyframe_buffers(ferns, &poses, &times), "cf_ferns_keyframe_buffers");
diff --git a/co_fusion_amd/lib.py b/co_fusion_amd/lib.py
--- a/co_fusion_amd/lib.py
+++ b/co_fusion_amd/lib.py
@@ -19,6 +19,7 @@
     "cf_bilateral", "cf_model_create", "cf_model_destroy", "cf_model_initialise", "cf_model_count",
     "cf_model_predict_indices", "cf_model_index_keys", "cf_model_index_resolve", "cf_model_combined_predict", "cf_model_prefetch_fill_ratio", "cf_model_perform_fill_in", "cf_model_requires_fill_in",
     "cf_model_fuse", "cf_model_clean", "cf_models_frame_passes", "cf_models_preindex", "cf_model_download_map", "cf_model_upload_map", "cf_model_buffer",
+    "cf_set_extent_culling", "cf_model_extents_unknown",
     "cf_redetect_score", "cf_redetect_timing", "cf_relabel",
     "cf_fusion_weight", "cf_seg_create", "cf_seg_destroy", "cf_seg_slic", "cf_seg_crf", "cf_seg_sums", "cf_seg_infer", "cf_seg_early", "cf_seg_run_batch", "cf_seg_fetch", "cf_seg_publish_poses", "cf_seg_fetch_poses",
     "cf_seg_labels", "cf_seg_buffer", "cf_seg_create_masks", "cf_seg_masks", "cf_seg_masks_batch", "cf_seg_new_mask_value",
diff --git a/co_fusion_amd/model.py b/co_fusion_amd/model.py
--- a/co_fusion_amd/model.py
+++ b/co_fusion_amd/model.py
@@ -49,6 +49,10 @@
     for a, (m, od, time) in zip(arr, items):
         a.model, a.odom, a.time = m.h, od.h, int(time)
     ctx._check(ctx.lib.cf_models_preindex(ctx.h, arr, n, C.c_float(depth_cutoff), int(TIME_DELTA if time_delta is None else time_delta)))
+
+
+def set_extent_culling(ctx: Context, on=True):
+    ctx._check(ctx.lib.cf_set_extent_culling(ctx.h, int(bool(on))))
 
 
 _BUF = {0: (np.uint32, 1), 1: (np.float32, 4), 2: (np.float32, 4), 3: (np.float32, 4), 4: (np.uint8, 4), 5: (np.float32, 4),
@@ -153,6 +157,9 @@
         s = np.ascontiguousarray(surfels, np.float32).reshape(-1, SURFEL)
         self.ctx._check(self.ctx.lib.cf_model_upload_map(self.h, s.ctypes.data_as(C.c_void_p), s.shape[0]))
 
+    def extents_unknown(self):
+        self.ctx._check(self.ctx.lib.cf_model_extents_unknown(self.h))
+
     def tensor(self, which):
         ptr = C.c_void_p(); nbytes = C.c_uint64()
         self.ctx._check(self.ctx.lib.cf_model_buffer(self.h, which, C.byref(ptr), C.byref(nbytes)))
@@ -168,6 +175,8 @@
             return host.view(np.float32).reshape(-1, SURFEL)
         if which == 13:
             return host.view(np.float32).reshape(h, w, 8)
+        if which == 14:
+            return host.view(np.uint64).reshape(h, w)
         dt, ch = _BUF[which]
         a = host.view(dt)
         return a.reshape(h, w, ch) if ch > 1 else a.reshape(h, w)
diff --git a/include/cofusion_hip.h b/include/cofusion_hip.h
--- a/include/cofusion_hip.h
+++ b/include/cofusion_hip.h
@@ -244,6 +244,8 @@
 int cf_model_download_map(cf_model *m, float *host_surfels, uint32_t capacity, uint32_t *count);
 int cf_model_upload_map(cf_model *m, const float *host_surfels, uint32_t count);
 int cf_model_buffer(cf_model *m, int which, void **dptr, uint64_t *bytes);
+int cf_set_extent_culling(cf_ctx *ctx, int on);
+int cf_model_extents_unknown(cf_model *m);
 typedef struct { uint32_t projected, occluded, seen_through, agree, agree_on_label, covered; } cf_redetect_counts;
 typedef struct {
     cf_model *model;
```
